# zhang-xuan1314/ABC-Net

Hardware: NVIDIA B200
Metric: images_per_sec_unet_fwd_decode (higher is better)
Workload: dtype bf16

## Files before the change

abcnet_b200/_lib.py:

```python
from __future__ import annotations

import ctypes as C
import os

_HERE = os.path.dirname(os.path.abspath(__file__))
LIB_PATH = os.path.join(_HERE, "libabcnet_b200.so")

EXPORTS = (
    "abc_last_error", "abc_version", "abc_device_ok", "abc_sm_count", "abc_launch_count",
    "abc_conv3x3_c1", "abc_conv3x3_c1_u8", "abc_conv3x3_cn", "abc_conv3x3_cn_wgrad", "abc_conv3x3_stem", "abc_conv_igemm", "abc_conv_wpack_bytes", "abc_decode_peaks",
    "abc_loss_partials", "abc_loss_backward", "abc_loss_partials_p8",
    "abc_bn_stats", "abc_bn_finalize", "abc_bn_act", "abc_bn_act_backward", "abc_nchw_to_p8", "abc_channel_sum",
    "abc_nchw_to_p8_ex", "abc_deinterleave2", "abc_conv_wgrad", "abc_conv3x3_c1_wgrad", "abc_conv3x3_c1_raw",
    "abc_heads_fused", "abc_heads_fused_pack_sizes", "abc_gather_pack", "abc_adam_step", "abc_adam_chunk_elems", "abc_assemble_molblocks", "abc_gather_patches", "abc_rasterise_targets",
    "abc_unet_wpack_bytes", "abc_unet_workspace_bytes", "abc_unet_create", "abc_unet_forward_infer", "abc_unet_destroy", "abc_unet_pack_host",
)


class AbcConvDesc(C.Structure):
    _fields_ = [
        ("in_", C.c_void_p), ("N", C.c_int), ("H", C.c_int), ("W", C.c_int),
        ("in_planes", C.c_int), ("in_plane_off", C.c_int), ("cin", C.c_int),
        ("wpack", C.c_void_p), ("bias", C.c_void_p),
        ("cout", C.c_int), ("n_tile", C.c_int), ("ntaps", C.c_int),
        ("tap_dy", C.c_int * 9), ("tap_dx", C.c_int * 9),
        ("act", C.c_int), ("out_mode", C.c_int),
        ("out", C.c_void_p), ("out_planes", C.c_int), ("out_plane_off", C.c_int),
        ("out_H", C.c_int), ("out_W", C.c_int),
        ("out_sy", C.c_int), ("out_oy", C.c_int), ("out_sx", C.c_int), ("out_ox", C.c_int),
        ("pool_out", C.c_void_p), ("pool_planes", C.c_int), ("pool_plane_off", C.c_int),
        ("k_segments", C.c_int), ("seg_tap0", C.c_int * 4), ("seg_ntaps", C.c_int * 4),
        ("row_fold", C.c_int), ("cta_pair", C.c_int), ("swap_mn", C.c_int),
        ("stat_sum", C.c_void_p), ("stat_sq", C.c_void_p), ("subpixel", C.c_int), ("k_chunk", C.c_int), ("act_fp16", C.c_int),
    ]


class AbcUNetConfig(C.Structure):
    _fields_ = [("in_channels", C.c_int), ("n_heads", C.c_int), ("heads", C.c_int * 16), ("crop_first", C.c_int), ("act_fp16", C.c_int)]


class AbcNamedTensor(C.Structure):
    _fields_ = [("name", C.c_char_p), ("data", C.c_void_p), ("numel", C.c_int64)]


class AbcAtomRec(C.Structure):
    _fields_ = [("x", C.c_uint16), ("y", C.c_uint16), ("type", C.c_uint8), ("charge", C.c_uint8),
                ("hs", C.c_uint8), ("pad", C.c_uint8)]


class AbcBondRec(C.Structure):
    _fields_ = [("x", C.c_uint16), ("y", C.c_uint16), ("omega", C.c_uint8), ("type", C.c_uint8),
                ("pad", C.c_uint16), ("rho", C.c_float)]


class AbcDecodeDesc(C.Structure):
    _fields_ = [
        ("maps", C.c_void_p * 8), ("N", C.c_int), ("H", C.c_int), ("W", C.c_int),
        ("c_type", C.c_int), ("c_charge", C.c_int), ("c_hs", C.c_int), ("n_omega", C.c_int), ("n_btype", C.c_int),
        ("thr", C.c_float), ("omega_mode", C.c_int),
        ("atoms", C.c_void_p), ("atom_cap", C.c_int),
        ("bonds", C.c_void_p), ("bond_cap", C.c_int),
        ("counts", C.c_void_p), ("p8f_mask", C.c_int), ("centre_prob", C.c_int), ("thr_omega", C.c_float),
        ("peak_pix", C.c_void_p), ("peak_cnt", C.c_void_p), ("peak_cap", C.c_int), ("sparse_mode", C.c_int),
    ]


class AbcTargetsDesc(C.Structure):
    _fields_ = [
        ("N", C.c_int), ("H", C.c_int), ("W", C.c_int), ("n_omega", C.c_int), ("n_btype", C.c_int), ("c_type", C.c_int),
        ("c_charge", C.c_int), ("c_hs", C.c_int),
        ("atoms", C.c_void_p), ("atom_off", C.c_void_p), ("bonds", C.c_void_p), ("bond_rho", C.c_void_p), ("bond_off", C.c_void_p),
        ("atom_target", C.c_void_p), ("atom_type", C.c_void_p), ("atom_charge", C.c_void_p), ("atom_hs", C.c_void_p),
        ("bond_target", C.c_void_p), ("bond_type", C.c_void_p), ("bond_rho_map", C.c_void_p), ("bond_omega", C.c_void_p),
        ("f64", C.c_int), ("zero_first", C.c_int),
    ]


class AbcHeadsFusedDesc(C.Structure):
    _fields_ = [
        ("in_", C.c_void_p), ("N", C.c_int), ("H", C.c_int), ("W", C.c_int), ("in_planes", C.c_int), ("in_plane_off", C.c_int),
        ("w1pack", C.c_void_p), ("bias1", C.c_void_p), ("n_heads", C.c_int), ("cout", C.c_int * 16),
        ("w2pack", C.c_void_p), ("w2pack_bytes", C.c_int64), ("bias2", C.c_void_p), ("bias2_len", C.c_int),
        ("out", C.c_void_p * 16), ("out_mode", C.c_int * 16), ("out_planes", C.c_int * 16), ("item_slot", C.c_int * 6),
        ("act_fp16", C.c_int),
    ]


class AbcBnActDesc(C.Structure):
    _fields_ = [
        ("z", C.c_void_p), ("z_planes", C.c_int), ("z_plane_off", C.c_int),
        ("out", C.c_void_p), ("out_planes", C.c_int), ("out_plane_off", C.c_int),
        ("pool", C.c_void_p), ("pool_planes", C.c_int), ("pool_plane_off", C.c_int),
        ("N", C.c_int), ("H", C.c_int), ("W", C.c_int), ("C", C.c_int),
        ("scale", C.c_void_p), ("shift", C.c_void_p),
        ("act", C.c_int), ("drop_p", C.c_float), ("seed", C.c_uint64), ("seed_dev", C.c_void_p), ("drop_mask", C.c_void_p),
    ]


class AbcBnActBwdDesc(C.Structure):
    _fields_ = [
        ("z", C.c_void_p), ("z_planes", C.c_int), ("z_plane_off", C.c_int),
        ("dA", C.c_void_p), ("dA_planes", C.c_int), ("dA_plane_off", C.c_int),
        ("dP", C.c_void_p), ("dP_planes", C.c_int), ("dP_plane_off", C.c_int),
        ("dz", C.c_void_p), ("dz_planes", C.c_int), ("dz_plane_off", C.c_int),
        ("N", C.c_int), ("H", C.c_int), ("W", C.c_int), ("C", C.c_int),
        ("scale", C.c_void_p), ("shift", C.c_void_p), ("mean", C.c_void_p), ("invstd", C.c_void_p),
        ("act", C.c_int), ("drop_p", C.c_float), ("seed", C.c_uint64),
        ("s1", C.c_void_p), ("s2", C.c_void_p), ("seed_dev", C.c_void_p), ("gscale", C.c_void_p), ("drop_mask", C.c_void_p),
    ]


class AbcWgradDesc(C.Structure):
    _fields_ = [
        ("dz", C.c_void_p), ("dz_planes", C.c_int), ("dz_plane_off", C.c_int), ("cout", C.c_int),
        ("in_", C.c_void_p), ("in_planes", C.c_int), ("in_plane_off", C.c_int), ("cin", C.c_int),
        ("N", C.c_int), ("H", C.c_int), ("W", C.c_int),
        ("ntaps", C.c_int), ("tap_dy", C.c_int * 9), ("tap_dx", C.c_int * 9),
        ("dw", C.c_void_p), ("row_boxes", C.c_int),
    ]


class AbcLossDesc(C.Structure):
    _fields_ = [
        ("logits", C.c_void_p * 8), ("targets", C.c_void_p * 8), ("tgt_f64", C.c_int),
        ("N", C.c_int), ("H", C.c_int), ("W", C.c_int),
        ("c_type", C.c_int), ("c_charge", C.c_int), ("c_hs", C.c_int), ("n_omega", C.c_int), ("n_btype", C.c_int),
        ("type_weights", C.c_void_p), ("sums", C.c_void_p), ("scale", C.c_void_p),
        ("dlogits", C.c_void_p * 8),
    ]


class AbcLossP8Out(C.Structure):
    _fields_ = [("dz", C.c_void_p * 8), ("planes", C.c_int * 8), ("dbias", C.c_void_p * 8)]


assert C.sizeof(AbcAtomRec) == 8 and C.sizeof(AbcBondRec) == 12


def _load():
    if not os.path.exists(LIB_PATH):
        raise ImportError(
            f"{LIB_PATH} not found: the abcnet_b200 CUDA library has not been built "
            "(run __graft_entry__.build() or `make -C abcnet_b200/csrc`). There is no CPU fallback.")
    lib = C.CDLL(LIB_PATH)
    lib.abc_last_error.restype = C.c_char_p
    lib.abc_launch_count.restype = C.c_int64
    lib.abc_conv_wpack_bytes.restype = C.c_int64
    lib.abc_conv_wpack_bytes.argtypes = [C.c_int] * 4
    lib.abc_conv3x3_c1.argtypes = [C.c_void_p, C.c_void_p, C.c_void_p, C.c_void_p, C.c_int, C.c_int, C.c_int,
                                   C.c_int, C.c_int, C.c_void_p]
    lib.abc_conv3x3_c1_u8.argtypes = lib.abc_conv3x3_c1.argtypes
    lib.abc_conv3x3_cn.argtypes = [C.c_void_p, C.c_int, C.c_void_p, C.c_void_p, C.c_void_p, C.c_int, C.c_int, C.c_int,
                                   C.c_int, C.c_int, C.c_int, C.c_void_p]
    lib.abc_conv3x3_stem.argtypes = [C.c_void_p, C.c_int, C.c_int, C.c_void_p, C.c_void_p, C.c_void_p, C.c_int, C.c_int, C.c_int,
                                     C.c_int, C.c_int, C.c_int, C.c_void_p]
    lib.abc_conv3x3_cn_wgrad.argtypes = [C.c_void_p, C.c_int, C.c_void_p, C.c_int, C.c_int, C.c_int, C.c_int, C.c_int,
                                         C.c_void_p, C.c_void_p]
    lib.abc_conv_igemm.argtypes = [C.POINTER(AbcConvDesc), C.c_void_p]
    lib.abc_decode_peaks.argtypes = [C.POINTER(AbcDecodeDesc), C.c_void_p]
    lib.abc_loss_partials.argtypes = [C.POINTER(AbcLossDesc), C.c_void_p]
    lib.abc_loss_backward.argtypes = [C.POINTER(AbcLossDesc), C.c_void_p]
    lib.abc_loss_partials_p8.argtypes = [C.POINTER(AbcLossDesc), C.POINTER(AbcLossP8Out), C.c_void_p]
    vp, ci = C.c_void_p, C.c_int
    lib.abc_bn_stats.argtypes = [vp, ci, ci, ci, ci, ci, ci, vp, vp, vp]
    lib.abc_channel_sum.argtypes = lib.abc_bn_stats.argtypes
    lib.abc_bn_finalize.argtypes = [vp, vp, ci, C.c_double, vp, vp, C.c_float, C.c_float, vp, vp, vp, vp, vp, vp, vp]
    lib.abc_bn_act.argtypes = [C.POINTER(AbcBnActDesc), vp]
    lib.abc_bn_act_backward.argtypes = [C.POINTER(AbcBnActBwdDesc), vp]
    lib.abc_nchw_to_p8.argtypes = [vp, vp, ci, ci, ci, ci, vp]
    lib.abc_nchw_to_p8_ex.argtypes = [vp, vp, ci, ci, ci, ci, ci, vp, vp, vp]
    lib.abc_deinterleave2.argtypes = [vp, ci, ci, ci, vp, ci, ci, ci, vp]
    lib.abc_conv_wgrad.argtypes = [C.POINTER(AbcWgradDesc), vp]
    lib.abc_conv3x3_c1_wgrad.argtypes = [vp, ci, vp, ci, ci, ci, ci, ci, vp, vp]
    lib.abc_conv3x3_c1_raw.argtypes = [vp, ci, vp, vp, vp, ci, ci, ci, ci, ci, vp]
    lib.abc_heads_fused.argtypes = [C.POINTER(AbcHeadsFusedDesc), vp]
    lib.abc_heads_fused_pack_sizes.argtypes = [ci, C.POINTER(C.c_int), C.POINTER(C.c_int64), C.POINTER(C.c_int)]
    lib.abc_gather_pack.argtypes = [vp, vp, vp, C.c_int64, ci, vp]
    lib.abc_adam_step.argtypes = [vp, vp, vp, vp, vp, vp, ci, vp, vp, vp]
    lib.abc_rasterise_targets.argtypes = [C.POINTER(AbcTargetsDesc), vp]
    lib.abc_gather_patches.argtypes = [vp, ci, ci, ci, ci, vp, vp, ci, vp, vp]
    lib.abc_unet_wpack_bytes.restype = C.c_int64
    lib.abc_unet_wpack_bytes.argtypes = [C.POINTER(AbcUNetConfig)]
    lib.abc_unet_workspace_bytes.restype = C.c_int64
    lib.abc_unet_workspace_bytes.argtypes = [C.POINTER(AbcUNetConfig), ci, ci, ci]
    lib.abc_unet_create.argtypes = [C.POINTER(AbcUNetConfig), C.POINTER(AbcNamedTensor), ci, vp, C.c_int64, vp, C.POINTER(vp)]
    lib.abc_unet_forward_infer.argtypes = [vp, vp, ci, ci, ci, ci, vp, C.c_int64, C.POINTER(vp), ci, vp]
    lib.abc_unet_destroy.argtypes = [vp]
    lib.abc_unet_pack_host.argtypes = [C.POINTER(AbcUNetConfig), C.POINTER(AbcNamedTensor), ci, vp, C.c_int64, C.POINTER(C.c_int64)]
    lib.abc_assemble_molblocks.argtypes = [vp, ci, vp, ci, vp, ci, vp, vp, ci, ci, vp, C.c_int64, vp]
    return lib


lib = _load()


def check(rc: int, what: str = "abcnet_b200") -> None:
    if rc != 0:
        msg = lib.abc_last_error()
        raise RuntimeError(f"{what} failed with status {rc}: {msg.decode() if msg else ''}")


def require_device() -> None:
    if not lib.abc_device_ok():
        msg = lib.abc_last_error()
        raise RuntimeError("abcnet_b200 needs an sm_100 (B200) CUDA device and has no CPU fallback: "
                           + (msg.decode() if msg else ""))


def current_stream_ptr() -> int:
    import torch
    return torch.cuda.current_stream().cuda_stream


def launch_count() -> int:
    return int(lib.abc_launch_count())
```

abcnet_b200/csrc/conv_first.cu:

```cuda
#include <cstdlib>
#include <cuda_bf16.h>

#include "common.cuh"
#include "p8_device.cuh"

namespace abc {

template <typename T>
__global__ void __launch_bounds__(256) conv3x3_c1_kernel(const T* __restrict__ img, const float* __restrict__ w,
                                                         const float* __restrict__ b, uint4* __restrict__ out, int H, int W,
                                                         int out_planes, int out_plane_off, int relu) {
  __shared__ float ws[16 * 9 + 16];
  const int tid = threadIdx.y * 32 + threadIdx.x;
  if (tid < 144) ws[tid] = w[tid];
  if (tid < 16) ws[144 + tid] = b[tid];
  __syncthreads();
  const int x = blockIdx.x * 32 + threadIdx.x;
  const int y = blockIdx.y * 8 + threadIdx.y;
  const int n = blockIdx.z;
  if (x >= W || y >= H) return;
  const T* im = img + static_cast<size_t>(n) * H * W;
  float t[9];
#pragma unroll
  for (int dy = 0; dy < 3; ++dy)
#pragma unroll
    for (int dx = 0; dx < 3; ++dx) {
      const int yy = y + dy - 1, xx = x + dx - 1;
      t[dy * 3 + dx] = (yy >= 0 && yy < H && xx >= 0 && xx < W) ? static_cast<float>(__ldg(im + static_cast<size_t>(yy) * W + xx)) : 0.f;
    }
  float v[16];
#pragma unroll
  for (int co = 0; co < 16; ++co) {
    float a = ws[144 + co];
#pragma unroll
    for (int k = 0; k < 9; ++k) a = fmaf(t[k], ws[co * 9 + k], a);
    v[co] = (relu & 1) ? fmaxf(a, 0.f) : a;
  }
#pragma unroll
  for (int pl = 0; pl < 2; ++pl)
    out[((static_cast<size_t>(n) * out_planes + out_plane_off + pl) * H + y) * W + x] = pack8_act16(v + pl * 8, (relu & 2) != 0);
}

constexpr int kC1Rows = 16;

__device__ __forceinline__ uint4 c1_pack8(const float* a, int flags) { return pack8_act16(a, (flags & 2) != 0); }

template <typename T>
__device__ __noinline__ void c1_generic_pixel(const T* __restrict__ im, int y, int x, int H, int W, const float* ws, int relu,
                                              uint4* o0, uint4* o1) {
  float t[9];
#pragma unroll
  for (int k = 0; k < 9; ++k) {
    const int yy = y + k / 3 - 1, xx = x + k % 3 - 1;
    t[k] = (yy >= 0 && yy < H && xx >= 0 && xx < W) ? static_cast<float>(__ldg(im + static_cast<size_t>(yy) * W + xx)) : 0.f;
  }
#pragma unroll
  for (int pl = 0; pl < 2; ++pl) {
    float v[8];
#pragma unroll
    for (int c8 = 0; c8 < 8; ++c8) {
      const int co = pl * 8 + c8;
      float a = ws[144 + co];
#pragma unroll
      for (int k = 0; k < 9; ++k) a = fmaf(t[k], ws[k * 16 + co], a);
      v[c8] = (relu & 1) ? fmaxf(a, 0.f) : a;
    }
    *(pl ? o1 : o0) = c1_pack8(v, relu);
  }
}

template <typename T>
__global__ void __launch_bounds__(256, 4) conv3x3_c1_rows_kernel(const T* __restrict__ img, const float* __restrict__ w,
                                                              const float* __restrict__ b, uint4* __restrict__ out, int N, int H, int W,
                                                              int out_planes, int out_plane_off, int relu) {
  __shared__ __align__(16) float ws[9 * 16 + 16];
  __shared__ __align__(16) uint4 lut[512][2];
  const int tid = threadIdx.x;
  if (tid < 144) ws[(tid % 9) * 16 + tid / 9] = w[tid];
  if (tid < 16) ws[144 + tid] = b[tid];
  __syncthreads();
#pragma unroll 1
  for (int e = tid; e < 512; e += 256) {
#pragma unroll 1
    for (int pl = 0; pl < 2; ++pl) {
      float v[8];
#pragma unroll
      for (int c8 = 0; c8 < 8; ++c8) {
        const int co = pl * 8 + c8;
        float a = ws[144 + co];
#pragma unroll
        for (int k = 0; k < 9; ++k) a = fmaf(((e >> k) & 1) ? 1.f : 0.f, ws[k * 16 + co], a);
        v[c8] = (relu & 1) ? fmaxf(a, 0.f) : a;
      }
      lut[e][pl] = c1_pack8(v, relu);
    }
  }
  __syncthreads();
  const int lane = tid & 31, warp = tid >> 5;
  const int tiles_x = (W + 127) >> 7, strips = (H + kC1Rows - 1) / kC1Rows;
  const long long items = static_cast<long long>(N) * strips * tiles_x;
  const size_t plane = static_cast<size_t>(H) * W;
  for (long long it = static_cast<long long>(blockIdx.x) * 8 + warp; it < items; it += static_cast<long long>(gridDim.x) * 8) {
    const int n = static_cast<int>(it / (strips * tiles_x));
    const int rem = static_cast<int>(it - static_cast<long long>(n) * (strips * tiles_x));
    const int x0 = (rem % tiles_x) << 7, y0 = (rem / tiles_x) * kC1Rows;
    const int y1 = min(y0 + kC1Rows, H);
    const T* im = img + static_cast<size_t>(n) * plane;
    uint4* o_img = out + (static_cast<size_t>(n) * out_planes + out_plane_off) * plane;
    const int xe = lane == 0 ? x0 - 1 : x0 + 128;
    const bool edge_ok = lane < 2 && xe >= 0 && xe < W;
    uint32_t m[3][4], e[3];
    bool nb[3];
    auto load_row = [&](int yy, uint32_t (&mm)[4], uint32_t& ee, bool& nbin) {
      float v[4], ve = 0.f;
      const bool in = yy >= 0 && yy < H;
      const T* row = im + static_cast<size_t>(in ? yy : 0) * W;
#pragma unroll
      for (int k = 0; k < 4; ++k) {
        const int x = x0 + 32 * k + lane;
        v[k] = (in && x < W) ? static_cast<float>(__ldg(row + x)) : 0.f;
      }
      if (in && edge_ok) ve = static_cast<float>(__ldg(row + xe));
      bool bad = (ve != 0.f) && (ve != 1.f);
#pragma unroll
      for (int k = 0; k < 4; ++k) {
        mm[k] = __ballot_sync(0xffffffffu, v[k] != 0.f);
        bad = bad || ((v[k] != 0.f) && (v[k] != 1.f));
      }
      ee = __ballot_sync(0xffffffffu, ve != 0.f);
      nbin = __any_sync(0xffffffffu, bad);
    };
    load_row(y0 - 1, m[0], e[0], nb[0]);
    load_row(y0, m[1], e[1], nb[1]);
    for (int y = y0; y < y1; ++y) {
      load_row(y + 1, m[2], e[2], nb[2]);
      uint4* o0 = o_img + static_cast<size_t>(y) * W;
      uint4* o1 = o0 + plane;
      if (!(nb[0] || nb[1] || nb[2])) {
#pragma unroll
        for (int k = 0; k < 4; ++k) {
          uint32_t pat = 0;
#pragma unroll
          for (int r = 0; r < 3; ++r) {
            const uint32_t lo = k == 0 ? (e[r] & 1u) : (m[r][k - 1] >> 31);
            const uint32_t hi = k == 3 ? ((e[r] >> 1) & 1u) : (m[r][k + 1] & 1u);
            const uint64_t wide = (static_cast<uint64_t>(hi) << 33) | (static_cast<uint64_t>(m[r][k]) << 1) | lo;
            pat |= (static_cast<uint32_t>(wide >> lane) & 7u) << (3 * r);
          }
          const int x = x0 + 32 * k + lane;
          if (x < W) {
            o0[x] = lut[pat][0];
            o1[x] = lut[pat][1];
          }
        }
      } else {
#pragma unroll 1
        for (int k = 0; k < 4; ++k) {
          const int x = x0 + 32 * k + lane;
          if (x < W) c1_generic_pixel<T>(im, y, x, H, W, ws, relu, o0 + x, o1 + x);
        }
      }
#pragma unroll
      for (int k = 0; k < 4; ++k) {
        m[0][k] = m[1][k];
        m[1][k] = m[2][k];
      }
      e[0] = e[1]; e[1] = e[2];
      nb[0] = nb[1]; nb[1] = nb[2];
    }
  }
}

__global__ void __launch_bounds__(256) conv3x3_cn_kernel(const float* __restrict__ img, int cin, const float* __restrict__ w,
                                                         const float* __restrict__ b, uint4* __restrict__ out, int H, int W,
                                                         int out_planes, int out_plane_off, int relu) {
  __shared__ float ws[16 * 8 * 9 + 16];
  const int tid = threadIdx.y * 32 + threadIdx.x;
  for (int i = tid; i < 16 * cin * 9; i += 256) ws[i] = w[i];
  if (tid < 16) ws[16 * 8 * 9 + tid] = b[tid];
  __syncthreads();
  const int x = blockIdx.x * 32 + threadIdx.x;
  const int y = blockIdx.y * 8 + threadIdx.y;
  const int n = blockIdx.z;
  if (x >= W || y >= H) return;
  float v[16];
#pragma unroll
  for (int co = 0; co < 16; ++co) v[co] = ws[16 * 8 * 9 + co];
  for (int ci = 0; ci < cin; ++ci) {
    const float* im = img + (static_cast<size_t>(n) * cin + ci) * H * W;
    float t[9];
#pragma unroll
    for (int dy = 0; dy < 3; ++dy)
#pragma unroll
      for (int dx = 0; dx < 3; ++dx) {
        const int yy = y + dy - 1, xx = x + dx - 1;
        t[dy * 3 + dx] = (yy >= 0 && yy < H && xx >= 0 && xx < W) ? __ldg(im + static_cast<size_t>(yy) * W + xx) : 0.f;
      }
#pragma unroll
    for (int co = 0; co < 16; ++co) {
      float a = v[co];
#pragma unroll
      for (int k = 0; k < 9; ++k) a = fmaf(t[k], ws[(co * cin + ci) * 9 + k], a);
      v[co] = a;
    }
  }
  if (relu & 1) {
#pragma unroll
    for (int co = 0; co < 16; ++co) v[co] = fmaxf(v[co], 0.f);
  }
#pragma unroll
  for (int pl = 0; pl < 2; ++pl)
    out[((static_cast<size_t>(n) * out_planes + out_plane_off + pl) * H + y) * W + x] = pack8_act16(v + pl * 8, (relu & 2) != 0);
}

}

extern "C" int abc_conv3x3_cn(const float* img, int cin, const float* w, const float* b, void* out, int N, int H, int W,
                              int out_planes, int out_plane_off, int relu, void* stream) {
  using namespace abc;
  if (int rc = device_check()) return rc;
  ABC_REQUIRE(img && w && b && out, "abc_conv3x3_cn: null pointer");
  ABC_REQUIRE(cin >= 1 && cin <= 8, "abc_conv3x3_cn: cin=%d must be in 1..8", cin);
  ABC_REQUIRE(N > 0 && H > 0 && W > 0 && N <= 65535, "abc_conv3x3_cn: bad geometry N=%d H=%d W=%d", N, H, W);
  ABC_REQUIRE(out_plane_off >= 0 && out_plane_off + 2 <= out_planes, "abc_conv3x3_cn: output plane range");
  ABC_REQUIRE((reinterpret_cast<uintptr_t>(out) & 15) == 0, "abc_conv3x3_cn: output must be 16-byte aligned");
  dim3 grid((W + 31) / 32, (H + 7) / 8, N);
  conv3x3_cn_kernel<<<grid, dim3(32, 8), 0, static_cast<cudaStream_t>(stream)>>>(img, cin, w, b, static_cast<uint4*>(out), H, W,
                                                                                  out_planes, out_plane_off, relu);
  return launch_check("conv3x3_cn_kernel");
}

template <typename T>
static int conv3x3_c1_launch(const T* img, const float* w, const float* b, void* out, int N, int H, int W, int out_planes,
                             int out_plane_off, void* stream, int relu = 1) {
  using namespace abc;
  if (int rc = device_check()) return rc;
  ABC_REQUIRE(img && w && b && out, "abc_conv3x3_c1: null pointer");
  ABC_REQUIRE(N > 0 && H > 0 && W > 0 && N <= 65535, "abc_conv3x3_c1: bad geometry N=%d H=%d W=%d", N, H, W);
  ABC_REQUIRE(out_plane_off >= 0 && out_plane_off + 2 <= out_planes, "abc_conv3x3_c1: output plane range");
  ABC_REQUIRE((reinterpret_cast<uintptr_t>(out) & 15) == 0, "abc_conv3x3_c1: output must be 16-byte aligned");
  dim3 block(32, 8);
  static const bool simple = getenv("ABCNET_C1_SIMPLE") != nullptr;
  if (!simple) {
    const long long items = static_cast<long long>((W + 127) / 128) * ((H + kC1Rows - 1) / kC1Rows) * N;
    int sms = sm_count();
    if (sms <= 0) sms = 148;
    const long long want = (items + 7) / 8;
    const int gx = static_cast<int>(want < 4LL * sms ? want : 4LL * sms);
    conv3x3_c1_rows_kernel<T><<<gx, 256, 0, static_cast<cudaStream_t>(stream)>>>(img, w, b, static_cast<uint4*>(out), N, H, W,
                                                                                 out_planes, out_plane_off, relu);
    return launch_check("conv3x3_c1_rows_kernel");
  }
  dim3 grid((W + 31) / 32, (H + 7) / 8, N);
  conv3x3_c1_kernel<T><<<grid, block, 0, static_cast<cudaStream_t>(stream)>>>(img, w, b, static_cast<uint4*>(out), H, W,
                                                                               out_planes, out_plane_off, relu);
  return launch_check("conv3x3_c1_kernel");
}

extern "C" int abc_conv3x3_c1(const float* img, const float* w, const float* b, void* out, int N, int H, int W,
                              int out_planes, int out_plane_off, void* stream) {
  return conv3x3_c1_launch<float>(img, w, b, out, N, H, W, out_planes, out_plane_off, stream);
}

extern "C" int abc_conv3x3_c1_u8(const uint8_t* img, const float* w, const float* b, void* out, int N, int H, int W,
                                 int out_planes, int out_plane_off, void* stream) {
  return conv3x3_c1_launch<uint8_t>(img, w, b, out, N, H, W, out_planes, out_plane_off, stream);
}

extern "C" int abc_conv3x3_c1_raw(const void* img, int img_is_u8, const float* w, const float* b, void* out, int N, int H, int W,
                                  int out_planes, int out_plane_off, void* stream) {
  if (img_is_u8)
    return conv3x3_c1_launch<uint8_t>(static_cast<const uint8_t*>(img), w, b, out, N, H, W, out_planes, out_plane_off, stream, 0);
  return conv3x3_c1_launch<float>(static_cast<const float*>(img), w, b, out, N, H, W, out_planes, out_plane_off, stream, 0);
}


extern "C" int abc_conv3x3_stem(const void* img, int img_is_u8, int cin, const float* w, const float* b, void* out, int N, int H, int W,
                                int out_planes, int out_plane_off, int flags, void* stream) {
  ABC_REQUIRE(flags >= 0 && flags <= 3, "abc_conv3x3_stem: flags=%d (bit 0 ReLU, bit 1 fp16 output)", flags);
  if (cin != 1) {
    ABC_REQUIRE(!img_is_u8, "abc_conv3x3_stem: uint8 images are the 1-channel binarised format");
    return abc_conv3x3_cn(static_cast<const float*>(img), cin, w, b, out, N, H, W, out_planes, out_plane_off, flags, stream);
  }
  if (img_is_u8)
    return conv3x3_c1_launch<uint8_t>(static_cast<const uint8_t*>(img), w, b, out, N, H, W, out_planes, out_plane_off, stream, flags);
  return conv3x3_c1_launch<float>(static_cast<const float*>(img), w, b, out, N, H, W, out_planes, out_plane_off, stream, flags);
}
```

abcnet_b200/csrc/conv_igemm_sm100.cu:

```cuda
#include <cstdlib>
#include <cuda.h>
#include <cuda_bf16.h>

#include "common.cuh"
#include "p8_device.cuh"
#include "ptx_sm100.cuh"

namespace abc {

constexpr int kMaxNA = 8;
constexpr int kMaxAcc = 8;
constexpr int kMaxNB = 16;
constexpr uint32_t kHeaderBytes = 2048;
constexpr uint32_t kSmemBudget = 232448;
constexpr int kThreads = 384;
constexpr int kTmemCols = 512;
constexpr uint32_t kSwapRowBytes = 80;
constexpr uint32_t kSwapWarpBytes = 16 * kSwapRowBytes;
constexpr uint32_t kSwapStageBytes = 8 * kSwapWarpBytes;

struct ConvKParams {
  int N, H, W, tiles_x, tiles_y, groups_x, num_groups;
  int in_plane_off, kp, nkc, ntaps, halo, n_tile, resident_b, na, nb, mt, nacc, acc_cols;
  int chunks_per_seg, blocks_per_ntile;
  int seg_tap0[4], seg_ntaps[4];
  uint32_t a_stage_bytes, a_tile_bytes, a_plane_bytes, a_row_bytes, b_block_bytes;
  uint32_t tap_off[18];
  int dbg;
  int fold;
  int tile_rows;
  uint32_t smem_a_off, smem_b_off;
  const uint8_t* wpack;
  const float* bias;
  int cout, act, out_mode;
  void* out;
  int out_planes, out_plane_off, out_H, out_W, out_sy, out_oy, out_sx, out_ox;
  void* pool_out;
  int pool_planes, pool_plane_off;
  int subpixel;
  int fp16;
  double* stat_sum;
  double* stat_sq;
};

__device__ __forceinline__ float apply_act(float v, int act) {
  if (act == 1) return fmaxf(v, 0.f);
  if (act == 2) return v > 0.f ? v : 0.01f * v;
  return v;
}

__device__ __forceinline__ uint4 pack8_bf16(const float* v) {
  __nv_bfloat162 a = __floats2bfloat162_rn(v[0], v[1]);
  __nv_bfloat162 b = __floats2bfloat162_rn(v[2], v[3]);
  __nv_bfloat162 c = __floats2bfloat162_rn(v[4], v[5]);
  __nv_bfloat162 d = __floats2bfloat162_rn(v[6], v[7]);
  uint4 r;
  r.x = *reinterpret_cast<uint32_t*>(&a);
  r.y = *reinterpret_cast<uint32_t*>(&b);
  r.z = *reinterpret_cast<uint32_t*>(&c);
  r.w = *reinterpret_cast<uint32_t*>(&d);
  return r;
}

__device__ __forceinline__ uint32_t pool_max_bf16x2(uint32_t a, bool f16) {
  uint32_t b = __shfl_xor_sync(0xffffffffu, a, 1);
  a = max2_act16(a, b, f16);
  b = __shfl_xor_sync(0xffffffffu, a, 8);
  return max2_act16(a, b, f16);
}

__device__ __forceinline__ uint4 hmax_bf16x8(uint4 a, uint4 b, bool f16) {
  return make_uint4(max2_act16(a.x, b.x, f16), max2_act16(a.y, b.y, f16), max2_act16(a.z, b.z, f16), max2_act16(a.w, b.w, f16));
}

__device__ __forceinline__ uint4 pool_hmax_x(uint4 q, bool f16) {
  uint4 o;
  o.x = __shfl_xor_sync(0xffffffffu, q.x, 1);
  o.y = __shfl_xor_sync(0xffffffffu, q.y, 1);
  o.z = __shfl_xor_sync(0xffffffffu, q.z, 1);
  o.w = __shfl_xor_sync(0xffffffffu, q.w, 1);
  return hmax_bf16x8(q, o, f16);
}

__device__ __forceinline__ uint4 pool_max_bf16x8(uint4 q, bool f16) {
  q.x = pool_max_bf16x2(q.x, f16);
  q.y = pool_max_bf16x2(q.y, f16);
  q.z = pool_max_bf16x2(q.z, f16);
  q.w = pool_max_bf16x2(q.w, f16);
  return q;
}

template <int KSTEPS, bool RESIDENT, bool CG2, bool SWAP = false, bool STATS = false>
__global__ void __launch_bounds__(kThreads, 1)
conv_igemm_kernel(const __grid_constant__ CUtensorMap tmap, const ConvKParams p) {
  static_assert(!(CG2 && RESIDENT), "the CTA-pair variant streams its weights");
  static_assert(!(CG2 && SWAP), "operand swap is a single-CTA mode");
  static_assert(!(STATS && (SWAP || CG2)), "STATS is the non-swap, single-CTA variant");
  extern __shared__ __align__(1024) uint8_t smem[];
  const uint32_t sbase = smem_u32(smem);
  const int warp = static_cast<int>(warp_id_uniform());
  const int lane = threadIdx.x & 31;
  const uint32_t cta_rank = CG2 ? cluster_ctarank() : 0u;
  const bool leader = cta_rank == 0;

  const uint32_t bar_a_full = sbase;
  const uint32_t bar_a_empty = sbase + 8 * kMaxNA;
  const uint32_t bar_b_full = sbase + 8 * (2 * kMaxNA);
  const uint32_t bar_b_empty = bar_b_full + 8 * kMaxNB;
  const uint32_t bar_acc_full = bar_b_empty + 8 * kMaxNB;
  const uint32_t bar_acc_empty = bar_acc_full + 8 * kMaxAcc;
  static_assert(8 * (2 * kMaxNA + 2 * kMaxNB + 2 * kMaxAcc) <= 768, "barrier slots overflow the header");
  uint32_t* tmem_slot = reinterpret_cast<uint32_t*>(smem + 768);
  float* bias_s = reinterpret_cast<float*>(smem + 1024);

  if (threadIdx.x == 0) {
    const uint32_t full_count = (CG2 && leader && !(p.dbg & 1)) ? 2 : 1;
    for (int i = 0; i < kMaxNA; ++i) {
      mbar_init(bar_a_full + 8 * i, full_count);
      mbar_init(bar_a_empty + 8 * i, 1);
    }
    for (int i = 0; i < kMaxNB; ++i) {
      mbar_init(bar_b_full + 8 * i, full_count);
      mbar_init(bar_b_empty + 8 * i, 1);
    }
    for (int i = 0; i < kMaxAcc; ++i) {
      mbar_init(bar_acc_full + 8 * i, 1);
      mbar_init(bar_acc_empty + 8 * i, CG2 ? 16 : 8);
    }
    fence_mbar_init();
    tma_prefetch_desc(&tmap);
  }
  if (CG2) cluster_sync_all();
  if (warp == 2) {
    if (CG2) tmem_alloc_pair<kTmemCols>(smem_u32(tmem_slot));
    else tmem_alloc<kTmemCols>(smem_u32(tmem_slot));
  }
  for (int i = threadIdx.x; i < p.n_tile; i += kThreads) bias_s[i] = p.bias[blockIdx.y * p.n_tile + i];
  uint32_t* utab = reinterpret_cast<uint32_t*>(smem + 800);
  uint32_t* utab2 = reinterpret_cast<uint32_t*>(smem + 928);
  if (threadIdx.x < ((p.mt * p.n_tile) >> 4)) {
    const int col = threadIdx.x << 4;
    const int ti = col / p.n_tile;
    const int ul = (col - ti * p.n_tile) >> 4;
    const int b16 = ul / p.fold;
    utab[threadIdx.x] = static_cast<uint32_t>(ti) | (ul << 8) | (b16 << 16) | ((ul - b16 * p.fold) << 24);
    if (p.subpixel > 0 && threadIdx.x < 16) {
      const int c0 = blockIdx.y * p.n_tile + (b16 << 4);
      const int ph = c0 / p.subpixel, chn = c0 - ph * p.subpixel;
      utab2[threadIdx.x] = (static_cast<uint32_t>(chn >> 3) << 16) | static_cast<uint32_t>((ph >> 1) * p.out_W + (ph & 1));
    }
  }
  tc_fence_before();
  if (CG2) cluster_sync_all();
  else __syncthreads();
  tc_fence_after();
  const uint32_t tmem_base = *reinterpret_cast<volatile uint32_t*>(tmem_slot);
  const int g_first = CG2 ? static_cast<int>(blockIdx.x & ~1u) : static_cast<int>(blockIdx.x);

  const int groups_per_img = p.groups_x * p.tiles_y;
  const uint32_t a_region = sbase + p.smem_a_off;
  const uint32_t b_region = sbase + p.smem_b_off;
  const int blocks_per_ntile = p.blocks_per_ntile;

  if (warp == 0) {
    int stage = 0;
    uint32_t phase = 0;
    for (int gp = g_first; gp < p.num_groups; gp += gridDim.x) {
      const int g = CG2 ? min(gp + static_cast<int>(cta_rank), p.num_groups - 1) : gp;
      const int n = g / groups_per_img;
      const int rem = g - n * groups_per_img;
      const int ty = rem / p.groups_x;
      const int tx0 = (rem - ty * p.groups_x) * p.mt;
      const int c1 = ty * p.tile_rows - p.halo;
      for (int kc = 0; kc < p.nkc; ++kc) {
        mbar_wait(bar_a_empty + 8 * stage, phase ^ 1);
        if (elect_one()) {
          mbar_arrive_expect_tx(bar_a_full + 8 * stage, p.a_stage_bytes);
          for (int i = 0; i < p.mt; ++i)
            tma_load_4d(a_region + stage * p.a_stage_bytes + i * p.a_tile_bytes, &tmap, bar_a_full + 8 * stage,
                        ((tx0 + i) * 8 - p.halo) * 8, c1, p.in_plane_off + kc * p.kp, n);
        }
        __syncwarp();
        if (++stage == p.na) {
          stage = 0;
          phase ^= 1;
        }
      }
    }
  } else if (warp == 3) {
    const size_t b_src_stride = CG2 ? 2 * static_cast<size_t>(p.b_block_bytes) : p.b_block_bytes;
    const uint8_t* wsrc = p.wpack + static_cast<size_t>(blockIdx.y) * blocks_per_ntile * b_src_stride +
                          (CG2 ? cta_rank * p.b_block_bytes : 0u);
    if (RESIDENT) {
      if (blockIdx.x < p.num_groups && elect_one()) {
        mbar_arrive_expect_tx(bar_b_full, static_cast<uint32_t>(blocks_per_ntile) * p.b_block_bytes);
        for (int blk = 0; blk < blocks_per_ntile; ++blk)
          bulk_load_1d(b_region + blk * p.b_block_bytes, wsrc + static_cast<size_t>(blk) * p.b_block_bytes,
                       p.b_block_bytes, bar_b_full);
      }
      __syncwarp();
    } else {
      int stage = 0;
      uint32_t phase = 0;
      for (int g = g_first; g < p.num_groups; g += gridDim.x) {
        for (int blk = 0; blk < blocks_per_ntile; ++blk) {
          mbar_wait(bar_b_empty + 8 * stage, phase ^ 1);
          if (elect_one()) {
            mbar_arrive_expect_tx(bar_b_full + 8 * stage, p.b_block_bytes);
            bulk_load_1d(b_region + stage * p.b_block_bytes, wsrc + static_cast<size_t>(blk) * b_src_stride,
                         p.b_block_bytes, bar_b_full + 8 * stage);
          }
          __syncwarp();
          if (++stage == p.nb) {
            stage = 0;
            phase ^= 1;
          }
        }
      }
    }
  } else if (warp == 1 && CG2 && !leader) {
    int a_stage = 0, b_stage = 0;
    uint32_t a_phase = 0, b_phase = 0;
    for (int g = g_first; g < p.num_groups; g += gridDim.x) {
      for (int kc = 0; kc < p.nkc; ++kc) {
        mbar_wait(bar_a_full + 8 * a_stage, a_phase);
        if (!(p.dbg & 1) && elect_one()) mbar_arrive_cluster(mapa_cluster(bar_a_full + 8 * a_stage, 0));
        __syncwarp();
        if (++a_stage == p.na) {
          a_stage = 0;
          a_phase ^= 1;
        }
        for (int t = 0; t < p.ntaps; ++t) {
          mbar_wait(bar_b_full + 8 * b_stage, b_phase);
          if (!(p.dbg & 1) && elect_one()) mbar_arrive_cluster(mapa_cluster(bar_b_full + 8 * b_stage, 0));
          __syncwarp();
          if (++b_stage == p.nb) {
            b_stage = 0;
            b_phase ^= 1;
          }
        }
      }
    }
  } else if (warp == 1) {
    const bool f16 = p.fp16 != 0;
    const uint32_t idesc = SWAP ? umma_idesc_16(128, 256, 0, 0, f16) : umma_idesc_16(CG2 ? 256 : 128, p.n_tile, 0, 0, f16);
    const int b_rows = CG2 ? p.n_tile >> 1 : p.n_tile;
    auto mma = [&](uint32_t d, uint32_t a_lo, uint32_t a_hi_, uint32_t b_lo, uint32_t b_hi_, uint32_t acc_) {
      if (CG2) umma_bf16_lohi_pair(d, a_lo, a_hi_, b_lo, b_hi_, idesc, acc_);
      else if (SWAP) umma_bf16_lohi(d, b_lo, b_hi_, a_lo, a_hi_, idesc, acc_);
      else umma_bf16_lohi(d, a_lo, a_hi_, b_lo, b_hi_, idesc, acc_);
    };
    auto commit = [&](uint32_t bar) {
      if (CG2) umma_commit_pair(bar);
      else umma_commit(bar);
    };
    const uint64_t a_hi64 = umma_desc_hi(p.a_plane_bytes, p.a_row_bytes * p.fold);
    const uint64_t b_hi64 = CG2 ? umma_desc_hi_sw128() : umma_desc_hi(b_rows * 16, 128);
    const uint32_t a_hi = static_cast<uint32_t>(a_hi64 >> 32), b_hi = static_cast<uint32_t>(b_hi64 >> 32);
    const uint32_t a_lo0 = static_cast<uint32_t>(a_hi64) | (a_region >> 4);
    const uint32_t b_lo0 = static_cast<uint32_t>(b_hi64) | (b_region >> 4);
    const uint32_t a_kstep = (2 * p.a_plane_bytes) >> 4, b_kstep = CG2 ? 2u : (2 * b_rows * 16) >> 4;
    const uint32_t a_tile16 = p.a_tile_bytes >> 4, a_stage16 = p.a_stage_bytes >> 4, b_block16 = p.b_block_bytes >> 4;
    int a_stage = 0, b_stage = 0, acc = 0;
    uint32_t a_phase = 0, b_phase = 0, acc_phase = 0;
    if (RESIDENT && blockIdx.x < p.num_groups) {
      mbar_wait(bar_b_full, 0);
      tc_fence_after();
    }
    if (p.chunks_per_seg == p.nkc) {
      uint32_t tap16[18];
#pragma unroll
      for (int t = 0; t < 18; ++t) tap16[t] = p.tap_off[t] >> 4;
      const int ntaps = p.ntaps, nkc = p.nkc, mt = p.mt, n_tile = p.n_tile, na = p.na, nb = p.nb, nacc = p.nacc;
      const uint32_t acc_cols = p.acc_cols;
      for (int g = g_first; g < p.num_groups; g += gridDim.x) {
        mbar_wait(bar_acc_empty + 8 * acc, acc_phase ^ 1);
        tc_fence_after();
        const uint32_t tmem_d = tmem_base + acc * acc_cols;
        uint32_t b_res = b_lo0;
        for (int kc = 0; kc < nkc; ++kc) {
          mbar_wait(bar_a_full + 8 * a_stage, a_phase);
          tc_fence_after();
          const uint32_t a_base = a_lo0 + a_stage * a_stage16;
#pragma unroll
          for (int t = 0; t < 18; ++t) {
            if (t < ntaps) {
              uint32_t b_base;
              if (RESIDENT) {
                b_base = b_res;
                b_res += b_block16;
              } else {
                mbar_wait(bar_b_full + 8 * b_stage, b_phase);
                tc_fence_after();
                b_base = b_lo0 + b_stage * b_block16;
              }
              const uint32_t a_tap = a_base + tap16[t];
              const uint32_t acc0 = (kc | t) != 0 ? 1u : 0u;
              if (elect_one()) {
                uint32_t d_col = tmem_d, a_t = a_tap;
                for (int i = 0; i < mt; ++i, d_col += n_tile, a_t += a_tile16) {
#pragma unroll
                  for (int j = 0; j < KSTEPS; ++j)
                    mma(d_col, a_t + j * a_kstep, a_hi, b_base + j * b_kstep, b_hi, j != 0 ? 1u : acc0);
                }
                if (!RESIDENT) commit(bar_b_empty + 8 * b_stage);
              }
              __syncwarp();
              if (!RESIDENT) {
                if (++b_stage == nb) {
                  b_stage = 0;
                  b_phase ^= 1;
                }
              }
            }
          }
          if (elect_one()) commit(bar_a_empty + 8 * a_stage);
          __syncwarp();
          if (++a_stage == na) {
            a_stage = 0;
            a_phase ^= 1;
          }
        }
        if (elect_one()) commit(bar_acc_full + 8 * acc);
        __syncwarp();
        if (++acc == nacc) {
          acc = 0;
          acc_phase ^= 1;
        }
      }
    } else
    for (int g = blockIdx.x; g < p.num_groups; g += gridDim.x) {
      mbar_wait(bar_acc_empty + 8 * acc, acc_phase ^ 1);
      tc_fence_after();
      const uint32_t tmem_d = tmem_base + acc * p.acc_cols;
      int blk = 0;
      for (int kc = 0; kc < p.nkc; ++kc) {
        mbar_wait(bar_a_full + 8 * a_stage, a_phase);
        tc_fence_after();
        const uint32_t a_base = a_lo0 + a_stage * a_stage16;
        const int seg = kc / p.chunks_per_seg;
        const int t_begin = p.seg_tap0[seg], t_end = t_begin + p.seg_ntaps[seg];
        for (int t = t_begin; t < t_end; ++t, ++blk) {
          uint32_t b_base;
          if (RESIDENT) {
            b_base = b_lo0 + blk * b_block16;
          } else {
            mbar_wait(bar_b_full + 8 * b_stage, b_phase);
            tc_fence_after();
            b_base = b_lo0 + b_stage * b_block16;
          }
          const uint32_t a_tap = a_base + (p.tap_off[t] >> 4);
          const uint32_t acc0 = (kc | (t - t_begin)) != 0 ? 1u : 0u;
          if (elect_one()) {
#pragma unroll 2
            for (int i = 0; i < p.mt; ++i) {
#pragma unroll
              for (int j = 0; j < KSTEPS; ++j)
                umma_bf16_lohi(tmem_d + i * p.n_tile, a_tap + i * a_tile16 + j * a_kstep, a_hi, b_base + j * b_kstep, b_hi,
                               idesc, j != 0 ? 1u : acc0);
            }
            if (!RESIDENT) umma_commit(bar_b_empty + 8 * b_stage);
          }
          __syncwarp();
          if (!RESIDENT) {
            if (++b_stage == p.nb) {
              b_stage = 0;
              b_phase ^= 1;
            }
          }
        }
        if (elect_one()) umma_commit(bar_a_empty + 8 * a_stage);
        __syncwarp();
        if (++a_stage == p.na) {
          a_stage = 0;
          a_phase ^= 1;
        }
      }
      if (elect_one()) umma_commit(bar_acc_full + 8 * acc);
      __syncwarp();
      if (++acc == p.nacc) {
        acc = 0;
        acc_phase ^= 1;
      }
    }
  } else if (warp >= 4 && SWAP) {
    const int q = warp & 3;
    const int eh = (warp - 4) >> 2;
    const int n0 = blockIdx.y * p.n_tile;
    const float bias = bias_s[q * 32 + lane];
    const float slope = p.act == 1 ? 0.f : (p.act == 2 ? 0.01f : 1.f);
    const int g8 = lane >> 3, i8 = lane & 7;
    const int J = p.fold, cpj = 128 / J;
    const int m0 = q * 32 + g8 * 8;
    const int fj = m0 / cpj, ch0 = m0 - fj * cpj;
    uint8_t* stage = smem + kHeaderBytes + (warp - 4) * kSwapWarpBytes;
    unsigned short* st_w = reinterpret_cast<unsigned short*>(stage) + lane;
    const bool f16 = p.fp16 != 0;
    const uint4* st_r = reinterpret_cast<const uint4*>(stage + i8 * kSwapRowBytes + g8 * 16);
    const bool plane_ok = (n0 + ch0) < p.cout;
    const size_t out_plane_px = static_cast<size_t>(p.out_H) * p.out_W;
    const bool do_stats = p.stat_sum != nullptr;
    const int m_own = q * 32 + lane;
    const int fj_own = m_own / cpj;
    float st_s = 0.f, st_q = 0.f;
    int acc = 0;
    uint32_t acc_phase = 0;
    for (int g = g_first; g < p.num_groups; g += gridDim.x) {
      const int n = g / groups_per_img;
      const int rem = g - n * groups_per_img;
      const int ty = rem / p.groups_x;
      const int tx = rem - ty * p.groups_x;
      const int x = tx * 8 + i8;
      const int y0 = (ty * 32 + eh * 16) * J + fj;
      uint4* obase = reinterpret_cast<uint4*>(p.out) +
                     (static_cast<size_t>(n) * p.out_planes + p.out_plane_off + ((n0 + ch0) >> 3)) * out_plane_px +
                     static_cast<size_t>(p.out_oy) * p.out_W + (x * p.out_sx + p.out_ox);
      const bool col_ok = plane_ok && x < p.W;
      const uint32_t tbase = tmem_base + acc * p.acc_cols + (static_cast<uint32_t>(q * 32) << 16) + eh * 128;
      const int x_left = p.W - tx * 8;
      const uint32_t xmask8 = x_left >= 8 ? 0xffu : ((1u << (x_left > 0 ? x_left : 0)) - 1u);
      const int yo0 = (ty * 32 + eh * 16) * J + fj_own;
      mbar_wait(bar_acc_full + 8 * acc, acc_phase);
      tc_fence_after();
      auto process = [&](uint32_t (&raw)[16], int it) {
        uint32_t vmask = 0;
        if (do_stats)
          vmask = ((yo0 + (it * 2) * J) < p.H ? xmask8 : 0u) | ((yo0 + (it * 2 + 1) * J) < p.H ? (xmask8 << 8) : 0u);
#pragma unroll
        for (int i = 0; i < 16; ++i) {
          const float t = __uint_as_float(raw[i]) + bias;
          const unsigned short hv = to_act16(fmaxf(t, t * slope), f16);
          st_w[i * (kSwapRowBytes / 2)] = hv;
          if (do_stats && ((vmask >> i) & 1u)) {
            const float r = __uint_as_float(static_cast<uint32_t>(hv) << 16);
            st_s += r;
            st_q = fmaf(r, r, st_q);
          }
        }
        __syncwarp();
#pragma unroll
        for (int rr = 0; rr < 2; ++rr) {
          const uint4 val = st_r[rr * (8 * kSwapRowBytes / 16)];
          const int y = y0 + (it * 2 + rr) * J;
          if (col_ok && y < p.H) obase[static_cast<size_t>(y * p.out_sy) * p.out_W] = val;
        }
        __syncwarp();
      };
      uint32_t raw_a[16], raw_b[16];
      tmem_ld16(tbase, raw_a);
#pragma unroll 1
      for (int it = 0; it < 8; it += 2) {
        tmem_ld_wait();
        tmem_ld16(tbase + (it + 1) * 16, raw_b);
        process(raw_a, it);
        tmem_ld_wait();
        if (it + 2 < 8) tmem_ld16(tbase + (it + 2) * 16, raw_a);
        process(raw_b, it + 1);
      }
      tc_fence_before();
      __syncwarp();
      if (lane == 0) mbar_arrive(bar_acc_empty + 8 * acc);
      if (++acc == p.nacc) {
        acc = 0;
        acc_phase ^= 1;
      }
    }
    if (do_stats) {
      const int ch = n0 + (m_own - fj_own * cpj);
      if (ch < p.cout) {
        atomicAdd(p.stat_sum + ch, static_cast<double>(st_s));
        atomicAdd(p.stat_sq + ch, static_cast<double>(st_q));
      }
    }
  } else if (warp >= 4) {
    const int q = warp & 3;
    const int eh = (warp - 4) >> 2;
    const int m = q * 32 + lane;
    const int r = m >> 3, c = m & 7;
    const int n0 = blockIdx.y * p.n_tile;
    const int units = (p.mt * p.n_tile) >> 4;
    const int nchunks = (units + 1) >> 1;
    const float slope = p.act == 1 ? 0.f : (p.act == 2 ? 0.01f : 1.f);
    const bool f16 = p.fp16 != 0;
    const float4* bias4 = reinterpret_cast<const float4*>(bias_s);
    const size_t out_plane_px = static_cast<size_t>(p.out_H) * p.out_W;
    const int ph = p.H >> 1, pw = p.W >> 1;
    const size_t pool_plane_px = static_cast<size_t>(ph) * pw;
    int acc = 0;
    uint32_t acc_phase = 0;
    float sacc[STATS ? 16 : 1], qacc[STATS ? 16 : 1];
#pragma unroll
    for (int i = 0; i < (STATS ? 16 : 1); ++i) sacc[i] = qacc[i] = 0.f;
    const uint32_t acc_empty_base = CG2 ? mapa_cluster(bar_acc_empty, 0) : bar_acc_empty;
    for (int gp = g_first; gp < p.num_groups; gp += gridDim.x) {
      const int g = CG2 ? min(gp + static_cast<int>(cta_rank), p.num_groups - 1) : gp;
      const bool g_valid = !CG2 || (gp + static_cast<int>(cta_rank) < p.num_groups);
      const int n = g / groups_per_img;
      const int rem = g - n * groups_per_img;
      const int ty = rem / p.groups_x;
      const int tx0 = (rem - ty * p.groups_x) * p.mt;
      const int ybase = (ty * 16 + r) * p.fold;
      const int xbase = tx0 * 8 + c;
      const size_t out_px0 = static_cast<size_t>(ybase * p.out_sy + p.out_oy) * p.out_W + (xbase * p.out_sx + p.out_ox);
      const size_t out_pl0 = static_cast<size_t>(n) * p.out_planes + p.out_plane_off + (n0 >> 3);
      const size_t pool_px0 = static_cast<size_t>(ybase >> 1) * pw + (xbase >> 1);
      const size_t pool_pl0 = static_cast<size_t>(n) * p.pool_planes + p.pool_plane_off + (n0 >> 3);
      const uint32_t tbase = tmem_base + acc * p.acc_cols + (static_cast<uint32_t>(q * 32) << 16);
      mbar_wait(bar_acc_full + 8 * acc, acc_phase);
      tc_fence_after();

      auto load = [&](uint32_t (&raw)[2][16], int ch) {
        tmem_ld16(tbase + ch * 32, raw[0]);
        if (2 * ch + 1 < units) tmem_ld16(tbase + ch * 32 + 16, raw[1]);
      };
      auto process = [&](uint32_t (&raw)[2][16], int ch) {
        uint4 keep0 = make_uint4(0, 0, 0, 0), keep1 = keep0;
#pragma unroll
        for (int half = 0; half < 2; ++half) {
          const int u = 2 * ch + half;
          if (u >= units) break;
          const uint32_t info = utab[u];
          const int ti = info & 0xff, bu = (info >> 8) & 0xff, b16 = (info >> 16) & 0xff, j = info >> 24;
          if (tx0 + ti >= p.tiles_x) continue;
          const int ch0 = n0 + (b16 << 4);
          const int y = ybase + j;
          const int x = xbase + ti * 8;
          const bool valid = (y < p.H) && (x < p.W) && (ch0 < p.cout) && g_valid;
          const bool two = (ch0 + 8) < p.cout;
          float v[16];
#pragma unroll
          for (int i = 0; i < 4; ++i) {
            const float4 bb = bias4[bu * 4 + i];
            float t0 = __uint_as_float(raw[half][4 * i + 0]) + bb.x, t1 = __uint_as_float(raw[half][4 * i + 1]) + bb.y;
            float t2 = __uint_as_float(raw[half][4 * i + 2]) + bb.z, t3 = __uint_as_float(raw[half][4 * i + 3]) + bb.w;
            v[4 * i + 0] = fmaxf(t0, t0 * slope);
            v[4 * i + 1] = fmaxf(t1, t1 * slope);
            v[4 * i + 2] = fmaxf(t2, t2 * slope);
            v[4 * i + 3] = fmaxf(t3, t3 * slope);
          }
          if (p.out_mode == 0) {
            uint4 q0 = pack8_act16(v, f16), q1 = pack8_act16(v + 8, f16);
            if constexpr (STATS) {
              if (valid) {
                float r[16];
                unpack8u(q0, r);
                unpack8u(q1, r + 8);
#pragma unroll
                for (int i = 0; i < 16; ++i) {
                  sacc[i] += r[i];
                  qacc[i] = fmaf(r[i], r[i], qacc[i]);
                }
              }
            }
            if (p.out != nullptr && valid) {
              uint4* o;
              if (p.subpixel > 0) {
                const uint32_t t2 = utab2[u];
                o = reinterpret_cast<uint4*>(p.out) +
                    (static_cast<size_t>(n) * p.out_planes + p.out_plane_off + (t2 >> 16)) * out_plane_px + out_px0 + (t2 & 0xffffu) +
                    ti * 8 * p.out_sx;
              } else {
                o = reinterpret_cast<uint4*>(p.out) + (out_pl0 + 2 * b16) * out_plane_px + out_px0 +
                    static_cast<size_t>(j * p.out_sy) * p.out_W + ti * 8 * p.out_sx;
              }
              o[0] = q0;
              if (two) o[out_plane_px] = q1;
            }
            if (p.pool_out != nullptr) {
              bool write;
              if (p.fold == 1) {
                q0 = pool_max_bf16x8(q0, f16);
                q1 = pool_max_bf16x8(q1, f16);
                write = !(c & 1) && !(r & 1);
              } else {
                if (half == 0) {
                  keep0 = q0;
                  keep1 = q1;
                  continue;
                }
                q0 = pool_hmax_x(hmax_bf16x8(q0, keep0, f16), f16);
                q1 = pool_hmax_x(hmax_bf16x8(q1, keep1, f16), f16);
                write = !(c & 1);
              }
              if (valid && write) {
                uint4* o = reinterpret_cast<uint4*>(p.pool_out) + (pool_pl0 + 2 * b16) * pool_plane_px + pool_px0 +
                           static_cast<size_t>(j >> 1) * pw + ti * 4;
                o[0] = q0;
                if (two) o[pool_plane_px] = q1;
              }
            }
          } else if (p.out_mode == 2) {
            if (valid) {
              float4* o = reinterpret_cast<float4*>(p.out) + 2 * ((out_pl0 + 2 * b16) * out_plane_px + out_px0 + ti * 8 * p.out_sx);
              o[0] = make_float4(v[0], v[1], v[2], v[3]);
              o[1] = make_float4(v[4], v[5], v[6], v[7]);
              if (two) {
                o += 2 * out_plane_px;
                o[0] = make_float4(v[8], v[9], v[10], v[11]);
                o[1] = make_float4(v[12], v[13], v[14], v[15]);
              }
            }
          } else if (valid) {
            float* o = reinterpret_cast<float*>(p.out) + (static_cast<size_t>(n) * p.cout + ch0) * out_plane_px + out_px0 +
                       ti * 8 * p.out_sx;
#pragma unroll
            for (int i = 0; i < 16; ++i)
              if (ch0 + i < p.cout) o[i * out_plane_px] = v[i];
          }
        }
      };

      uint32_t raw_a[2][16], raw_b[2][16];
      int ch = eh;
      if (ch < nchunks) {
        load(raw_a, ch);
        while (true) {
          tmem_ld_wait();
          if (ch + 2 < nchunks) load(raw_b, ch + 2);
          process(raw_a, ch);
          ch += 2;
          if (ch >= nchunks) break;
          tmem_ld_wait();
          if (ch + 2 < nchunks) load(raw_a, ch + 2);
          process(raw_b, ch);
          ch += 2;
          if (ch >= nchunks) break;
        }
      }
      tc_fence_before();
      __syncwarp();
      if (lane == 0) {
        if (CG2) mbar_arrive_cluster(acc_empty_base + 8 * acc);
        else mbar_arrive(bar_acc_empty + 8 * acc);
      }
      if (++acc == p.nacc) {
        acc = 0;
        acc_phase ^= 1;
      }
    }
    if constexpr (STATS) {
#pragma unroll
      for (int i = 0; i < 16; ++i) {
        float a = sacc[i], b = qacc[i];
#pragma unroll
        for (int o = 16; o > 0; o >>= 1) {
          a += __shfl_xor_sync(0xffffffffu, a, o);
          b += __shfl_xor_sync(0xffffffffu, b, o);
        }
        if (lane == 0 && n0 + i < p.cout) {
          atomicAdd(p.stat_sum + n0 + i, static_cast<double>(a));
          atomicAdd(p.stat_sq + n0 + i, static_cast<double>(b));
        }
      }
    }
  }

  tc_fence_before();
  if (CG2) cluster_sync_all();
  else __syncthreads();
  if (warp == 2) {
    tc_fence_after();
    if (CG2) tmem_dealloc_pair<kTmemCols>(tmem_base);
    else tmem_dealloc<kTmemCols>(tmem_base);
  }
}

typedef CUresult (*EncodeTiledFn)(CUtensorMap*, CUtensorMapDataType, cuuint32_t, void*, const cuuint64_t*,
                                  const cuuint64_t*, const cuuint32_t*, const cuuint32_t*, CUtensorMapInterleave,
                                  CUtensorMapSwizzle, CUtensorMapL2promotion, CUtensorMapFloatOOBfill);

static EncodeTiledFn get_encode_fn() { return reinterpret_cast<EncodeTiledFn>(tensor_map_encode_fn()); }

static int conv_kc(int cin) { return cin < 64 ? cin : 64; }

struct ConvEnv {
  int pair_dbg, mt256, mt, nacc;
  ConvEnv() {
    auto num = [](const char* name, int dflt) { const char* e = getenv(name); return e ? atoi(e) : dflt; };
    pair_dbg = num("ABCNET_PAIR_DBG", 0);
    mt256 = num("ABCNET_MT256", 0);
    mt = num("ABCNET_MT", 0);
    nacc = num("ABCNET_NACC", 0);
  }
};
static const ConvEnv& conv_env() {
  static const ConvEnv e;
  return e;
}

}

extern "C" int64_t abc_conv_wpack_bytes(int cin, int cout, int ntaps, int n_tile) {
  if (cin <= 0 || cin % 16 || n_tile < 16 || n_tile > 256 || n_tile % 16 || ntaps < 1 || ntaps > 18 || cout < 1) return -1;
  const int n_tiles = (cout + n_tile - 1) / n_tile;
  return static_cast<int64_t>(n_tiles) * n_tile * cin * ntaps * 2;
}

extern "C" int abc_conv_igemm(const AbcConvDesc* d, void* stream_) {
  using namespace abc;
  if (int rc = device_check()) return rc;
  ABC_REQUIRE(d != nullptr, "abc_conv_igemm: null descriptor");
  ABC_REQUIRE(d->in && d->wpack && d->bias, "abc_conv_igemm: null input / weights / bias");
  ABC_REQUIRE(d->out || d->pool_out, "abc_conv_igemm: no output buffer");
  ABC_REQUIRE(d->N > 0 && d->H > 0 && d->W > 0, "abc_conv_igemm: bad geometry N=%d H=%d W=%d", d->N, d->H, d->W);
  ABC_REQUIRE(d->cin >= 16 && d->cin % 16 == 0 && (d->cin <= 64 || d->cin % 64 == 0),
              "abc_conv_igemm: cin=%d must be 16, 32, 48, 64 or a multiple of 64", d->cin);
  ABC_REQUIRE(d->in_plane_off >= 0 && d->in_plane_off + d->cin / 8 <= d->in_planes, "abc_conv_igemm: input plane range");
  ABC_REQUIRE(d->n_tile >= 16 && d->n_tile <= 256 && d->n_tile % 16 == 0, "abc_conv_igemm: n_tile=%d", d->n_tile);
  ABC_REQUIRE(d->ntaps >= 1 && d->ntaps <= 9, "abc_conv_igemm: ntaps=%d", d->ntaps);
  ABC_REQUIRE(d->cout >= 1, "abc_conv_igemm: cout=%d", d->cout);
  ABC_REQUIRE(d->out_mode >= 0 && d->out_mode <= 2, "abc_conv_igemm: out_mode=%d", d->out_mode);
  ABC_REQUIRE((reinterpret_cast<uintptr_t>(d->in) & 15) == 0 && (reinterpret_cast<uintptr_t>(d->wpack) & 15) == 0,
              "abc_conv_igemm: input / weights must be 16-byte aligned");
  const int fold = d->row_fold > 1 ? d->row_fold : 1;
  if (fold > 1) {
    ABC_REQUIRE(fold == 2 || fold == 4, "abc_conv_igemm: row_fold=%d must be 1, 2 or 4", fold);
    ABC_REQUIRE(d->ntaps == 9 && d->k_segments <= 1, "abc_conv_igemm: row_fold needs the plain 3x3 tap set");
    ABC_REQUIRE(d->cout % 16 == 0 && d->n_tile == fold * d->cout, "abc_conv_igemm: row_fold needs n_tile == row_fold * cout (cout %% 16 == 0)");
    ABC_REQUIRE(d->out_mode == 0 && d->out_sy == 1 && d->out_sx == 1 && d->out_oy == 0 && d->out_ox == 0,
                "abc_conv_igemm: row_fold supports plain P8 outputs only");
  }
  const bool swap = d->swap_mn != 0;
  if (swap) {
    ABC_REQUIRE(d->n_tile == 128 && (fold == 1 || fold == 2 || fold == 4) && d->k_segments <= 1 && !d->cta_pair,
                "abc_conv_igemm: swap_mn needs n_tile == 128 and no k_segments / cta_pair");
    ABC_REQUIRE(d->out_mode == 0 && d->out != nullptr && d->pool_out == nullptr,
                "abc_conv_igemm: swap_mn supports plain P8 outputs only (no pool_out)");
  }
  int halo = 0;
  for (int t = 0; t < d->ntaps; ++t) {
    ABC_REQUIRE(d->tap_dy[t] >= -1 && d->tap_dy[t] <= 1 && d->tap_dx[t] >= -1 && d->tap_dx[t] <= 1,
                "abc_conv_igemm: tap %d offset out of [-1,1]", t);
    if (d->tap_dy[t] || d->tap_dx[t]) halo = 1;
  }
  if (d->out_mode == 0) {
    ABC_REQUIRE(d->cout % 8 == 0, "abc_conv_igemm: P8 output needs cout %% 8 == 0 (got %d)", d->cout);
    const int out_ch = d->subpixel > 0 ? d->subpixel : d->cout;
    if (d->out) ABC_REQUIRE(d->out_plane_off >= 0 && d->out_plane_off + out_ch / 8 <= d->out_planes, "abc_conv_igemm: output plane range");
  } else {
    ABC_REQUIRE(d->out != nullptr && d->pool_out == nullptr, "abc_conv_igemm: fp32 output modes need out and no pool_out");
    if (d->out_mode == 2)
      ABC_REQUIRE(d->out_plane_off >= 0 && d->out_plane_off + (d->cout + 7) / 8 <= d->out_planes,
                  "abc_conv_igemm: planar fp32 output plane range");
  }
  const int subpixel = d->subpixel > 0 ? d->subpixel : 0;
  if (subpixel) {
    ABC_REQUIRE(d->out_mode == 0 && d->out != nullptr && d->pool_out == nullptr && !swap && fold == 1 && !d->cta_pair,
                "abc_conv_igemm: subpixel needs a plain P8 output without pool / swap / fold / pair");
    ABC_REQUIRE(subpixel % 16 == 0 && d->cout == 4 * subpixel && d->out_sy == 2 && d->out_sx == 2,
                "abc_conv_igemm: subpixel needs cout == 4 * subpixel (multiple of 16) and out_sy == out_sx == 2");
    ABC_REQUIRE(d->n_tile / 16 <= 16 && d->out_W < 32768 && d->out_plane_off + subpixel / 8 <= d->out_planes,
                "abc_conv_igemm: subpixel: n_tile <= 256, out_W < 32768, plane range");
    ABC_REQUIRE((d->H - 1) * 2 + d->out_oy + 1 < d->out_H && (d->W - 1) * 2 + d->out_ox + 1 < d->out_W,
                "abc_conv_igemm: subpixel output mapping exceeds out_H x out_W");
  }
  if (d->out) {
    ABC_REQUIRE(d->out_sy >= 1 && d->out_sx >= 1 && d->out_oy >= 0 && d->out_ox >= 0 &&
                    (d->H - 1) * d->out_sy + d->out_oy < d->out_H && (d->W - 1) * d->out_sx + d->out_ox < d->out_W,
                "abc_conv_igemm: output mapping exceeds out_H x out_W");
  }
  if (d->pool_out) {
    ABC_REQUIRE(d->H % 2 == 0 && d->W % 2 == 0, "abc_conv_igemm: fused max-pool needs even H, W");
    ABC_REQUIRE(d->pool_plane_off >= 0 && d->pool_plane_off + d->cout / 8 <= d->pool_planes, "abc_conv_igemm: pool plane range");
  }

  ConvKParams p{};
  p.N = d->N; p.H = d->H; p.W = d->W;
  p.tiles_x = (d->W + 7) / 8;
  p.fold = fold;
  const ConvEnv& env = conv_env();
  p.dbg = env.pair_dbg;
  p.tile_rows = swap ? 32 * fold : 16 * fold;
  p.tiles_y = (d->H + p.tile_rows - 1) / p.tile_rows;
  p.in_plane_off = d->in_plane_off;
  const int kc = d->k_chunk > 0 ? d->k_chunk : conv_kc(d->cin);
  ABC_REQUIRE((kc == 16 || kc == 32 || kc == 48 || kc == 64) && kc <= d->cin && d->cin % kc == 0 && !(d->cta_pair && kc != 64),
              "abc_conv_igemm: k_chunk=%d must be 16, 32 or 64 and divide cin=%d", kc, d->cin);
  p.kp = kc / 8;
  p.nkc = d->cin / kc;
  p.ntaps = fold > 1 ? 3 * (fold + 2) : d->ntaps;
  p.halo = halo;
  p.n_tile = d->n_tile;
  const int rows = p.tile_rows + 2 * halo, cols = 8 + 2 * halo;
  p.a_row_bytes = cols * 16;
  p.a_plane_bytes = rows * p.a_row_bytes;
  p.a_tile_bytes = p.kp * p.a_plane_bytes;
  p.b_block_bytes = static_cast<uint32_t>(d->n_tile) * kc * 2;
  if (fold > 1) {
    for (int t = 0; t < p.ntaps; ++t) p.tap_off[t] = static_cast<uint32_t>(((t / 3) * cols + (t % 3)) * 16);
  } else {
    for (int t = 0; t < d->ntaps; ++t)
      p.tap_off[t] = static_cast<uint32_t>(((d->tap_dy[t] + halo) * cols + (d->tap_dx[t] + halo)) * 16);
  }
  ABC_REQUIRE((p.a_tile_bytes & 127u) == 0, "abc_conv_igemm: internal: A tile not a 128-byte multiple");
  const int nseg = d->k_segments > 1 ? d->k_segments : 1;
  ABC_REQUIRE(nseg <= 4 && p.nkc % nseg == 0, "abc_conv_igemm: k_segments=%d must divide the %d K chunks (<= 4)", nseg, p.nkc);
  p.chunks_per_seg = p.nkc / nseg;
  p.blocks_per_ntile = 0;
  for (int sgi = 0; sgi < nseg; ++sgi) {
    p.seg_tap0[sgi] = nseg > 1 ? d->seg_tap0[sgi] : 0;
    p.seg_ntaps[sgi] = nseg > 1 ? d->seg_ntaps[sgi] : p.ntaps;
    ABC_REQUIRE(p.seg_tap0[sgi] >= 0 && p.seg_ntaps[sgi] >= 1 && p.seg_tap0[sgi] + p.seg_ntaps[sgi] <= p.ntaps,
                "abc_conv_igemm: segment %d tap range", sgi);
    p.blocks_per_ntile += p.chunks_per_seg * p.seg_ntaps[sgi];
  }
  const bool want_pair = d->cta_pair != 0;
  if (want_pair) {
    ABC_REQUIRE(fold == 1 && nseg == 1 && kc == 64 && d->n_tile % 32 == 0,
                "abc_conv_igemm: cta_pair needs cin %% 64 == 0, n_tile %% 32 == 0, no row folding / K segments");
    p.b_block_bytes /= 2;
  }
  const uint32_t total_b = want_pair ? (1u << 30) : static_cast<uint32_t>(p.blocks_per_ntile) * p.b_block_bytes;
  p.smem_a_off = kHeaderBytes + (swap ? kSwapStageBytes : 0u);
  const uint32_t hdr = p.smem_a_off;
  int mt_max = swap ? 1 : 256 / d->n_tile;
  if (d->n_tile == 256 && env.mt256 > 0) mt_max = env.mt256 >= 2 ? 2 : 1;
  if (mt_max > 8) mt_max = 8;
  if (mt_max > p.tiles_x) mt_max = p.tiles_x;
  if (env.mt >= 1 && env.mt < mt_max) mt_max = env.mt;
  uint32_t smem_bytes = 0;
  p.mt = 0;
  for (int mt = mt_max; mt >= 1 && !p.mt; --mt) {
    const uint32_t a_stage = mt * p.a_tile_bytes;
    if (total_b < (1u << 20) && hdr + 2 * a_stage + total_b <= kSmemBudget) {
      p.mt = mt; p.resident_b = 1; p.nb = 1;
      int na = static_cast<int>((kSmemBudget - hdr - total_b) / a_stage);
      p.na = na > kMaxNA ? kMaxNA : na;
      p.a_stage_bytes = a_stage;
      p.smem_b_off = hdr + p.na * a_stage;
      smem_bytes = p.smem_b_off + total_b;
    }
  }
  for (int mt = mt_max; mt >= 1 && !p.mt; --mt) {
    const uint32_t a_stage = mt * p.a_tile_bytes;
    if (hdr + 2 * a_stage + (swap && fold > 1 ? 3 : 4) * p.b_block_bytes <= kSmemBudget) {
      p.mt = mt; p.resident_b = 0; p.na = 2;
      if (hdr + 3 * a_stage + 6 * p.b_block_bytes <= kSmemBudget) p.na = 3;
      p.a_stage_bytes = a_stage;
      p.smem_b_off = hdr + p.na * a_stage;
      if (want_pair) p.smem_b_off = (p.smem_b_off + 1023u) & ~1023u;
      int nb = static_cast<int>((kSmemBudget - p.smem_b_off) / p.b_block_bytes);
      p.nb = nb > kMaxNB ? kMaxNB : nb;
      smem_bytes = p.smem_b_off + p.nb * p.b_block_bytes;
    }
  }
  ABC_REQUIRE(p.mt >= 1, "abc_conv_igemm: cin=%d n_tile=%d does not fit in shared memory", d->cin, d->n_tile);
  p.acc_cols = swap ? 256 : p.mt * d->n_tile;
  p.nacc = kTmemCols / p.acc_cols;
  if (p.nacc > kMaxAcc) p.nacc = kMaxAcc;
  if (env.nacc >= 2 && env.nacc < p.nacc) p.nacc = env.nacc;
  p.groups_x = (p.tiles_x + p.mt - 1) / p.mt;
  const int64_t groups = static_cast<int64_t>(d->N) * p.groups_x * p.tiles_y;
  ABC_REQUIRE(groups < (1ll << 31), "abc_conv_igemm: too many tiles");
  p.num_groups = static_cast<int>(groups);
  if (smem_bytes < 120 * 1024) smem_bytes = 120 * 1024;
  p.wpack = static_cast<const uint8_t*>(d->wpack);
  p.bias = d->bias;
  p.cout = d->cout; p.act = d->act; p.out_mode = d->out_mode;
  p.out = d->out;
  p.out_planes = d->out_planes; p.out_plane_off = d->out_plane_off;
  p.out_H = d->out_H; p.out_W = d->out_W;
  p.out_sy = d->out_sy; p.out_oy = d->out_oy; p.out_sx = d->out_sx; p.out_ox = d->out_ox;
  p.pool_out = d->pool_out; p.pool_planes = d->pool_planes; p.pool_plane_off = d->pool_plane_off;
  p.subpixel = subpixel;
  p.fp16 = d->act_fp16 ? 1 : 0;
  ABC_REQUIRE(!(p.fp16 && (want_pair || d->stat_sum)), "abc_conv_igemm: act_fp16 is an inference mode (no cta_pair, no fused statistics)");
  cudaStream_t st_ = static_cast<cudaStream_t>(stream_);
  const bool stats = d->stat_sum != nullptr || d->stat_sq != nullptr;
  if (stats) {
    ABC_REQUIRE(d->stat_sum && d->stat_sq, "abc_conv_igemm: stat_sum and stat_sq go together");
    ABC_REQUIRE(d->out_mode == 0 && d->out != nullptr && d->pool_out == nullptr && !want_pair,
                "abc_conv_igemm: fused statistics need a plain P8 output");
    ABC_REQUIRE(swap || (fold == 4 && d->cout == 16 && d->n_tile == 64 && d->cin == 16),
                "abc_conv_igemm: fused statistics are built for operand-swap launches and the row-folded 16 -> 16 layers "
                "(use abc_bn_stats otherwise)");
    ABC_CUDA(cudaMemsetAsync(d->stat_sum, 0, d->cout * sizeof(double), st_));
    ABC_CUDA(cudaMemsetAsync(d->stat_sq, 0, d->cout * sizeof(double), st_));
    p.stat_sum = d->stat_sum;
    p.stat_sq = d->stat_sq;
  }

  EncodeTiledFn encode = get_encode_fn();
  if (!encode) {
    set_error("cuTensorMapEncodeTiled driver entry point not available");
    return ABC_ERR_NO_DEVICE;
  }
  CUtensorMap tmap;
  const cuuint64_t gdim[4] = {static_cast<cuuint64_t>(d->W) * 8, static_cast<cuuint64_t>(d->H),
                              static_cast<cuuint64_t>(d->in_planes), static_cast<cuuint64_t>(d->N)};
  const cuuint64_t gstride[3] = {static_cast<cuuint64_t>(d->W) * 16, static_cast<cuuint64_t>(d->W) * d->H * 16,
                                 static_cast<cuuint64_t>(d->W) * d->H * 16 * d->in_planes};
  const cuuint32_t box[4] = {static_cast<cuuint32_t>(cols * 8), static_cast<cuuint32_t>(rows),
                             static_cast<cuuint32_t>(p.kp), 1};
  const cuuint32_t estr[4] = {1, 1, 1, 1};
  CUresult cr = encode(&tmap, CU_TENSOR_MAP_DATA_TYPE_BFLOAT16, 4, const_cast<void*>(d->in), gdim, gstride, box, estr,
                       CU_TENSOR_MAP_INTERLEAVE_NONE, CU_TENSOR_MAP_SWIZZLE_NONE, CU_TENSOR_MAP_L2_PROMOTION_L2_256B,
                       CU_TENSOR_MAP_FLOAT_OOB_FILL_NONE);
  if (cr != CUDA_SUCCESS) {
    set_error("cuTensorMapEncodeTiled failed with CUresult %d (W=%d H=%d planes=%d N=%d box=%ux%ux%u)", static_cast<int>(cr),
              d->W, d->H, d->in_planes, d->N, box[0], box[1], box[2]);
    return ABC_ERR_CUDA;
  }

  typedef void (*KernelFn)(const CUtensorMap, const ConvKParams);
  KernelFn kernels[2][5] = {{nullptr, conv_igemm_kernel<1, false, false>, conv_igemm_kernel<2, false, false>,
                             conv_igemm_kernel<3, false, false>, conv_igemm_kernel<4, false, false>},
                            {nullptr, conv_igemm_kernel<1, true, false>, conv_igemm_kernel<2, true, false>,
                             conv_igemm_kernel<3, true, false>, conv_igemm_kernel<4, true, false>}};
  KernelFn swap_kernels[2][5] = {{nullptr, conv_igemm_kernel<1, false, false, true>, conv_igemm_kernel<2, false, false, true>,
                                  conv_igemm_kernel<3, false, false, true>, conv_igemm_kernel<4, false, false, true>},
                                 {nullptr, conv_igemm_kernel<1, true, false, true>, conv_igemm_kernel<2, true, false, true>,
                                  conv_igemm_kernel<3, true, false, true>, conv_igemm_kernel<4, true, false, true>}};
  KernelFn pair_kernel = conv_igemm_kernel<4, false, true>;
  KernelFn stats_kernel = conv_igemm_kernel<1, true, false, false, true>;
  static PerDeviceOnce attr_once;
  ABC_CUDA(attr_once.run([&]() -> cudaError_t {
    for (int r = 0; r < 2; ++r)
      for (int k = 1; k <= 4; ++k) {
        if (cudaError_t e = cudaFuncSetAttribute(kernels[r][k], cudaFuncAttributeMaxDynamicSharedMemorySize, kSmemBudget)) return e;
        if (cudaError_t e = cudaFuncSetAttribute(swap_kernels[r][k], cudaFuncAttributeMaxDynamicSharedMemorySize, kSmemBudget)) return e;
      }
    if (cudaError_t e = cudaFuncSetAttribute(stats_kernel, cudaFuncAttributeMaxDynamicSharedMemorySize, kSmemBudget)) return e;
    return cudaFuncSetAttribute(pair_kernel, cudaFuncAttributeMaxDynamicSharedMemorySize, kSmemBudget);
  }));
  const int ksteps = p.kp / 2;
  ABC_REQUIRE(ksteps >= 1 && ksteps <= 4, "abc_conv_igemm: internal: ksteps=%d", ksteps);
  const int n_tiles = (d->cout + d->n_tile - 1) / d->n_tile;
  int sms = sm_count();
  if (sms <= 0) sms = 148;
  int gx = sms / n_tiles;
  if (gx < 1) gx = 1;
  if (want_pair) {
    ABC_REQUIRE(!p.resident_b && ksteps == 4, "abc_conv_igemm: internal: cta_pair with resident weights");
    const int need = (p.num_groups + 1) & ~1;
    gx &= ~1;
    if (gx > need) gx = need;
    if (gx < 2) gx = 2;
    cudaLaunchConfig_t cfg = {};
    cfg.gridDim = dim3(gx, n_tiles, 1);
    cfg.blockDim = dim3(kThreads, 1, 1);
    cfg.dynamicSmemBytes = smem_bytes;
    cfg.stream = static_cast<cudaStream_t>(stream_);
    cudaLaunchAttribute attr[1];
    attr[0].id = cudaLaunchAttributeClusterDimension;
    attr[0].val.clusterDim.x = 2;
    attr[0].val.clusterDim.y = 1;
    attr[0].val.clusterDim.z = 1;
    cfg.attrs = attr;
    cfg.numAttrs = 1;
    ABC_CUDA(cudaLaunchKernelEx(&cfg, pair_kernel, tmap, p));
    return launch_check("conv_igemm_kernel<pair>");
  }
  if (gx > p.num_groups) gx = p.num_groups;
  dim3 grid(gx, n_tiles, 1);
  KernelFn fn = (swap ? swap_kernels : kernels)[p.resident_b ? 1 : 0][ksteps];
  if (stats && !swap) {
    ABC_REQUIRE(p.resident_b && ksteps == 1, "abc_conv_igemm: internal: fused statistics variant");
    fn = stats_kernel;
  }
  fn<<<grid, kThreads, smem_bytes, st_>>>(tmap, p);
  return launch_check(swap ? "conv_igemm_kernel<swap>" : "conv_igemm_kernel");
}
```

abcnet_b200/csrc/ptx_sm100.cuh:

```cuda
#pragma once
#include <cstdint>
#include <cuda_runtime.h>

namespace abc {

__device__ __forceinline__ uint32_t smem_u32(const void* p) {
  return static_cast<uint32_t>(__cvta_generic_to_shared(p));
}

__device__ __forceinline__ uint32_t warp_id_uniform() { return __shfl_sync(0xffffffffu, threadIdx.x >> 5, 0); }
__device__ __forceinline__ bool elect_one() {
  uint32_t pred;
  asm volatile(
      "{\n\t.reg .b32 rx;\n\t.reg .pred px;\n\t"
      "elect.sync rx|px, 0xffffffff;\n\t"
      "selp.u32 %0, 1, 0, px;\n\t}"
      : "=r"(pred));
  return pred != 0;
}

__device__ __forceinline__ void mbar_init(uint32_t bar, uint32_t count) {
  asm volatile("mbarrier.init.shared::cta.b64 [%0], %1;" ::"r"(bar), "r"(count) : "memory");
}
__device__ __forceinline__ void fence_mbar_init() {
  asm volatile("fence.mbarrier_init.release.cluster;" ::: "memory");
}
__device__ __forceinline__ void fence_proxy_async() {
  asm volatile("fence.proxy.async.shared::cta;" ::: "memory");
}
__device__ __forceinline__ void mbar_arrive(uint32_t bar) {
  asm volatile("{\n\t.reg .b64 st;\n\tmbarrier.arrive.shared::cta.b64 st, [%0];\n\t}" ::"r"(bar) : "memory");
}
__device__ __forceinline__ void mbar_arrive_expect_tx(uint32_t bar, uint32_t bytes) {
  asm volatile("{\n\t.reg .b64 st;\n\tmbarrier.arrive.expect_tx.shared::cta.b64 st, [%0], %1;\n\t}" ::"r"(bar),
               "r"(bytes)
               : "memory");
}
__device__ __forceinline__ bool mbar_try_wait(uint32_t bar, uint32_t parity) {
  uint32_t ok;
  asm volatile(
      "{\n\t.reg .pred p;\n\t"
      "mbarrier.try_wait.parity.shared::cta.b64 p, [%1], %2;\n\t"
      "selp.u32 %0, 1, 0, p;\n\t}"
      : "=r"(ok)
      : "r"(bar), "r"(parity)
      : "memory");
  return ok != 0;
}
__device__ __forceinline__ void mbar_wait(uint32_t bar, uint32_t parity) {
  uint32_t spins = 0;
  while (!mbar_try_wait(bar, parity)) {
    if (++spins > (1u << 24)) {
      printf("abcnet: mbarrier timeout (block %d,%d thread %d bar 0x%x parity %u)\n", blockIdx.x, blockIdx.y,
             threadIdx.x, bar, parity);
      __trap();
    }
  }
}

__device__ __forceinline__ void tma_prefetch_desc(const void* desc) {
  asm volatile("prefetch.tensormap [%0];" ::"l"(reinterpret_cast<uint64_t>(desc)) : "memory");
}
__device__ __forceinline__ void tma_load_4d(uint32_t dst, const void* desc, uint32_t bar, int c0, int c1, int c2,
                                            int c3) {
  asm volatile(
      "cp.async.bulk.tensor.4d.shared::cluster.global.mbarrier::complete_tx::bytes [%0], [%1, {%3, %4, %5, %6}], [%2];"
      ::"r"(dst), "l"(reinterpret_cast<uint64_t>(desc)), "r"(bar), "r"(c0), "r"(c1), "r"(c2), "r"(c3)
      : "memory");
}
__device__ __forceinline__ void bulk_load_1d(uint32_t dst, const void* src, uint32_t bytes, uint32_t bar) {
  asm volatile("cp.async.bulk.shared::cluster.global.mbarrier::complete_tx::bytes [%0], [%1], %2, [%3];" ::"r"(dst),
               "l"(reinterpret_cast<uint64_t>(src)), "r"(bytes), "r"(bar)
               : "memory");
}

template <int kCols>
__device__ __forceinline__ void tmem_alloc(uint32_t smem_dst) {
  const uint32_t ncols = kCols;
  asm volatile("tcgen05.alloc.cta_group::1.sync.aligned.shared::cta.b32 [%0], %1;" ::"r"(smem_dst), "r"(ncols)
               : "memory");
  asm volatile("tcgen05.relinquish_alloc_permit.cta_group::1.sync.aligned;" ::: "memory");
}
template <int kCols>
__device__ __forceinline__ void tmem_dealloc(uint32_t taddr) {
  const uint32_t ncols = kCols;
  asm volatile("tcgen05.dealloc.cta_group::1.sync.aligned.b32 %0, %1;" ::"r"(taddr), "r"(ncols) : "memory");
}
__device__ __forceinline__ void tc_fence_before() { asm volatile("tcgen05.fence::before_thread_sync;" ::: "memory"); }
__device__ __forceinline__ void tc_fence_after() { asm volatile("tcgen05.fence::after_thread_sync;" ::: "memory"); }

__device__ __forceinline__ void umma_bf16(uint32_t tmem_d, uint64_t adesc, uint64_t bdesc, uint32_t idesc,
                                          uint32_t accumulate) {
  asm volatile(
      "{\n\t.reg .pred p;\n\tsetp.ne.b32 p, %4, 0;\n\t"
      "tcgen05.mma.cta_group::1.kind::f16 [%0], %1, %2, %3, p;\n\t}"
      ::"r"(tmem_d), "l"(adesc), "l"(bdesc), "r"(idesc), "r"(accumulate)
      : "memory");
}
__device__ __forceinline__ void umma_bf16_lohi(uint32_t tmem_d, uint32_t a_lo, uint32_t a_hi, uint32_t b_lo, uint32_t b_hi,
                                               uint32_t idesc, uint32_t accumulate) {
  asm volatile(
      "{\n\t.reg .pred p;\n\t.reg .b64 da, db;\n\t"
      "mov.b64 da, {%1, %2};\n\tmov.b64 db, {%3, %4};\n\t"
      "setp.ne.b32 p, %6, 0;\n\t"
      "tcgen05.mma.cta_group::1.kind::f16 [%0], da, db, %5, p;\n\t}"
      ::"r"(tmem_d), "r"(a_lo), "r"(a_hi), "r"(b_lo), "r"(b_hi), "r"(idesc), "r"(accumulate)
      : "memory");
}
__device__ __forceinline__ void umma_16_ts(uint32_t tmem_d, uint32_t tmem_a, uint32_t b_lo, uint32_t b_hi, uint32_t idesc,
                                           uint32_t accumulate) {
  asm volatile(
      "{\n\t.reg .pred p;\n\t.reg .b64 db;\n\t"
      "mov.b64 db, {%2, %3};\n\t"
      "setp.ne.b32 p, %5, 0;\n\t"
      "tcgen05.mma.cta_group::1.kind::f16 [%0], [%1], db, %4, p;\n\t}"
      ::"r"(tmem_d), "r"(tmem_a), "r"(b_lo), "r"(b_hi), "r"(idesc), "r"(accumulate)
      : "memory");
}
__device__ __forceinline__ void umma_commit(uint32_t bar) {
  asm volatile("tcgen05.commit.cta_group::1.mbarrier::arrive::one.shared::cluster.b64 [%0];" ::"r"(bar) : "memory");
}
__device__ __forceinline__ void tmem_ld_wait() { asm volatile("tcgen05.wait::ld.sync.aligned;" ::: "memory"); }

__device__ __forceinline__ void tmem_ld16(uint32_t taddr, uint32_t (&r)[16]) {
  asm volatile(
      "tcgen05.ld.sync.aligned.32x32b.x16.b32 {%0,%1,%2,%3,%4,%5,%6,%7,%8,%9,%10,%11,%12,%13,%14,%15}, [%16];"
      : "=r"(r[0]), "=r"(r[1]), "=r"(r[2]), "=r"(r[3]), "=r"(r[4]), "=r"(r[5]), "=r"(r[6]), "=r"(r[7]), "=r"(r[8]),
        "=r"(r[9]), "=r"(r[10]), "=r"(r[11]), "=r"(r[12]), "=r"(r[13]), "=r"(r[14]), "=r"(r[15])
      : "r"(taddr)
      : "memory");
}
__device__ __forceinline__ void tmem_st16(uint32_t taddr, const uint32_t* r) {
  asm volatile(
      "tcgen05.st.sync.aligned.32x32b.x16.b32 [%0], {%1,%2,%3,%4,%5,%6,%7,%8,%9,%10,%11,%12,%13,%14,%15,%16};"
      ::"r"(taddr), "r"(r[0]), "r"(r[1]), "r"(r[2]), "r"(r[3]), "r"(r[4]), "r"(r[5]), "r"(r[6]), "r"(r[7]), "r"(r[8]),
        "r"(r[9]), "r"(r[10]), "r"(r[11]), "r"(r[12]), "r"(r[13]), "r"(r[14]), "r"(r[15])
      : "memory");
}
__device__ __forceinline__ void tmem_st_wait() { asm volatile("tcgen05.wait::st.sync.aligned;" ::: "memory"); }
__device__ __forceinline__ void named_bar_sync(uint32_t id, uint32_t threads) {
  asm volatile("bar.sync %0, %1;" ::"r"(id), "r"(threads) : "memory");
}

__device__ __forceinline__ uint32_t cluster_ctarank() {
  uint32_t r;
  asm volatile("mov.u32 %0, %%cluster_ctarank;" : "=r"(r));
  return r;
}
__device__ __forceinline__ void cluster_sync_all() {
  asm volatile("barrier.cluster.arrive.release.aligned;\n\tbarrier.cluster.wait.acquire.aligned;" ::: "memory");
}
__device__ __forceinline__ uint32_t mapa_cluster(uint32_t addr, uint32_t rank) {
  uint32_t r;
  asm volatile("mapa.shared::cluster.u32 %0, %1, %2;" : "=r"(r) : "r"(addr), "r"(rank));
  return r;
}
__device__ __forceinline__ void mbar_arrive_cluster(uint32_t cluster_addr) {
  asm volatile("mbarrier.arrive.release.cluster.shared::cluster.b64 _, [%0];" ::"r"(cluster_addr) : "memory");
}
template <int kCols>
__device__ __forceinline__ void tmem_alloc_pair(uint32_t smem_dst) {
  const uint32_t ncols = kCols;
  asm volatile("tcgen05.alloc.cta_group::2.sync.aligned.shared::cta.b32 [%0], %1;" ::"r"(smem_dst), "r"(ncols) : "memory");
  asm volatile("tcgen05.relinquish_alloc_permit.cta_group::2.sync.aligned;" ::: "memory");
}
template <int kCols>
__device__ __forceinline__ void tmem_dealloc_pair(uint32_t taddr) {
  const uint32_t ncols = kCols;
  asm volatile("tcgen05.dealloc.cta_group::2.sync.aligned.b32 %0, %1;" ::"r"(taddr), "r"(ncols) : "memory");
}
__device__ __forceinline__ void umma_bf16_lohi_pair(uint32_t tmem_d, uint32_t a_lo, uint32_t a_hi, uint32_t b_lo, uint32_t b_hi,
                                                    uint32_t idesc, uint32_t accumulate) {
  asm volatile(
      "{\n\t.reg .pred p;\n\t.reg .b64 da, db;\n\t"
      "mov.b64 da, {%1, %2};\n\tmov.b64 db, {%3, %4};\n\t"
      "setp.ne.b32 p, %6, 0;\n\t"
      "tcgen05.mma.cta_group::2.kind::f16 [%0], da, db, %5, p;\n\t}"
      ::"r"(tmem_d), "r"(a_lo), "r"(a_hi), "r"(b_lo), "r"(b_hi), "r"(idesc), "r"(accumulate)
      : "memory");
}
__device__ __forceinline__ void umma_commit_pair(uint32_t bar) {
  const uint16_t mask = 3;
  asm volatile("tcgen05.commit.cta_group::2.mbarrier::arrive::one.shared::cluster.multicast::cluster.b64 [%0], %1;" ::"r"(bar),
               "h"(mask)
               : "memory");
}

__device__ __forceinline__ uint64_t umma_desc_hi(uint32_t lbo_bytes, uint32_t sbo_bytes) {
  return (static_cast<uint64_t>((lbo_bytes >> 4) & 0x3FFF) << 16) | (static_cast<uint64_t>((sbo_bytes >> 4) & 0x3FFF) << 32) |
         (1ull << 46);
}
__device__ __forceinline__ uint64_t umma_desc(uint64_t hi, uint32_t smem_addr) {
  return hi | static_cast<uint64_t>((smem_addr >> 4) & 0x3FFF);
}
__device__ __forceinline__ uint64_t umma_desc_hi_sw128() {
  return (static_cast<uint64_t>(1024 >> 4) << 32) | (1ull << 46) | (2ull << 61);
}
__host__ __device__ constexpr uint32_t umma_idesc_bf16(int M, int N, int a_mn_major, int b_mn_major) {
  return (1u << 4) | (1u << 7) | (1u << 10) | (static_cast<uint32_t>(a_mn_major) << 15) |
         (static_cast<uint32_t>(b_mn_major) << 16) | (static_cast<uint32_t>(N >> 3) << 17) |
         (static_cast<uint32_t>(M >> 4) << 24);
}
__host__ __device__ constexpr uint32_t umma_idesc_16(int M, int N, int a_mn_major, int b_mn_major, bool fp16) {
  return umma_idesc_bf16(M, N, a_mn_major, b_mn_major) & ~(fp16 ? ((1u << 7) | (1u << 10)) : 0u);
}

}
```

abcnet_b200/csrc/unet_plan.cu:

```cuda
#include <cmath>
#include <cstring>
#include <map>
#include <string>
#include <vector>

#include <cuda_bf16.h>
#include <cuda_fp16.h>

#include "common.cuh"

namespace abc {

struct PackedConv {
  int64_t w_off = 0, b_off = 0;
  int cin = 0, cout = 0, n_tile = 0, ntaps = 0, fold = 1, fold_swap = 0, subpixel = 0;
  int tap_dy[9] = {0}, tap_dx[9] = {0};
};

struct UNetHandle {
  AbcUNetConfig cfg;
  const uint8_t* arena = nullptr;
  int64_t arena_bytes = 0;
  std::map<std::string, PackedConv> convs;
  int64_t stem_w_off = 0, stem_b_off = 0;
};

static const char* kDoubleConvs[] = {"inc1", "inc2", "down1.maxpool_conv.1", "down2.maxpool_conv.1", "inc3", "down3.maxpool_conv.1",
                                     "down4.maxpool_conv.1", "down5.maxpool_conv.1", "up1.conv", "up2.conv", "up3.conv", "dconv1", "dconv2"};
static const char* kShort[] = {"inc1", "inc2", "down1", "down2", "inc3", "down3", "down4", "down5", "up1.conv", "up2.conv", "up3.conv",
                               "dconv1", "dconv2"};
static const int kDcIn[] = {0, 16, 16, 32, 64, 64, 128, 256, 512, 256, 128, 128, 128};
static const int kDcOut[] = {16, 16, 32, 64, 64, 128, 256, 512, 256, 128, 128, 128, 128};

static bool is_pooled(const std::string& n) {
  return n == "inc2.3" || n == "down1.3" || n == "inc3.3" || n == "down3.3" || n == "down4.3";
}
static int default_n_tile(int cin, int cout) {
  const int c16 = (cout + 15) / 16 * 16;
  if (c16 <= 128) return c16;
  return (cout % 256 == 0 && cin >= 128) ? 256 : 128;
}
static int row_fold_for(int cin, int cout) {
  if (cout == 16 && cin <= 32) return 4;
  if (cout == 32 && cin <= 32) return 2;
  return 1;
}
static int swap_fold_for(int cin, int cout, bool plain) {
  if (!plain) return 0;
  const int J = cout == 64 ? 2 : (cout == 32 ? 4 : 0);
  if (J == 4 && cin > 32) return 0;
  return J;
}
static int head_conv2_n_tile(int h) {
  if (h <= 16) return 16;
  if (h <= 64) return 64;
  if (h <= 128) return 128;
  return ((h + 191) / 192 * 192 <= (h + 127) / 128 * 128) ? 192 : 128;
}
static void phase_taps(int parity, bool crop_first, int (&k)[2], int (&d)[2], int& n) {
  if (crop_first) {
    if (parity == 0) { n = 1; k[0] = 1; d[0] = 0; }
    else { n = 2; k[0] = 0; d[0] = 1; k[1] = 2; d[1] = 0; }
  } else {
    if (parity == 0) { n = 2; k[0] = 0; d[0] = 0; k[1] = 2; d[1] = -1; }
    else { n = 1; k[0] = 1; d[0] = 0; }
  }
}

struct Logical {
  int ntaps, rows, cin;
  std::vector<float> w;
  std::vector<float> bias;
  float& at(int t, int r, int c) { return w[(static_cast<size_t>(t) * rows + r) * cin + c]; }
};

static void append_pack(std::vector<uint8_t>& arena, PackedConv& pc, Logical& L, int n_tile, bool fp16) {
  const int kc = L.cin < 64 ? L.cin : 64;
  const int n_tiles = (L.rows + n_tile - 1) / n_tile;
  pc.n_tile = n_tile;
  pc.ntaps = L.ntaps;
  pc.cin = L.cin;
  while (arena.size() % 256) arena.push_back(0);
  pc.w_off = static_cast<int64_t>(arena.size());
  const size_t n_el = static_cast<size_t>(n_tiles) * n_tile * L.cin * L.ntaps;
  arena.resize(arena.size() + n_el * 2);
  uint16_t* dst = reinterpret_cast<uint16_t*>(arena.data() + pc.w_off);
  size_t o = 0;
  for (int nt = 0; nt < n_tiles; ++nt)
    for (int c = 0; c < L.cin / kc; ++c)
      for (int t = 0; t < L.ntaps; ++t)
        for (int p = 0; p < kc / 8; ++p)
          for (int r = 0; r < n_tile; ++r)
            for (int e = 0; e < 8; ++e) {
              const int row = nt * n_tile + r;
              const float v = row < L.rows ? L.at(t, row, c * kc + p * 8 + e) : 0.f;
              if (fp16) {
                const __half hv = __float2half_rn(v > 65504.f ? 65504.f : (v < -65504.f ? -65504.f : v));
                memcpy(&dst[o++], &hv, 2);
              } else {
                const __nv_bfloat16 bv = __float2bfloat16_rn(v);
                memcpy(&dst[o++], &bv, 2);
              }
            }
  while (arena.size() % 256) arena.push_back(0);
  pc.b_off = static_cast<int64_t>(arena.size());
  arena.resize(arena.size() + static_cast<size_t>(n_tiles) * n_tile * 4);
  float* b = reinterpret_cast<float*>(arena.data() + pc.b_off);
  for (int i = 0; i < n_tiles * n_tile; ++i) b[i] = i < L.rows ? L.bias[i] : 0.f;
}

struct Tensors {
  std::map<std::string, const AbcNamedTensor*> by_name;
  const float* get(const std::string& name, int64_t numel) const {
    auto it = by_name.find(name);
    if (it == by_name.end()) {
      set_error("abc_unet_create: tensor '%s' missing from the state_dict", name.c_str());
      return nullptr;
    }
    if (it->second->numel != numel || it->second->data == nullptr) {
      set_error("abc_unet_create: tensor '%s' has %lld elements, expected %lld", name.c_str(), static_cast<long long>(it->second->numel),
                static_cast<long long>(numel));
      return nullptr;
    }
    return it->second->data;
  }
};

static bool folded_conv(const Tensors& T, const std::string& conv, const std::string& bn, int cout, int cin, int k,
                        std::vector<float>& w, std::vector<float>& b) {
  const int64_t per = static_cast<int64_t>(cin) * k * k;
  const float* cw = T.get(conv + ".weight", cout * per);
  const float* cb = T.get(conv + ".bias", cout);
  const float* g = T.get(bn + ".weight", cout);
  const float* be = T.get(bn + ".bias", cout);
  const float* rm = T.get(bn + ".running_mean", cout);
  const float* rv = T.get(bn + ".running_var", cout);
  if (!cw || !cb || !g || !be || !rm || !rv) return false;
  w.resize(static_cast<size_t>(cout) * per);
  b.resize(cout);
  for (int co = 0; co < cout; ++co) {
    const float scale = g[co] / sqrtf(rv[co] + 1e-5f);
    for (int64_t i = 0; i < per; ++i) w[co * per + i] = cw[co * per + i] * scale;
    const float t = cb[co] - rm[co];
    b[co] = t * scale + be[co];
  }
  return true;
}

static void pack3x3(std::vector<uint8_t>& arena, PackedConv& pc, const std::vector<float>& w, const std::vector<float>& b, int cout, int cin,
                    bool plain_output, bool fp16) {
  const int js = swap_fold_for(cin, cout, plain_output);
  const int J = js ? js : row_fold_for(cin, cout);
  pc.cout = cout;
  pc.fold = J;
  pc.fold_swap = js ? 1 : 0;
  auto W = [&](int co, int ci, int dy, int dx) { return w[((static_cast<size_t>(co) * cin + ci) * 3 + (dy + 1)) * 3 + (dx + 1)]; };
  Logical L;
  L.cin = cin;
  if (J == 1) {
    L.ntaps = 9;
    L.rows = cout;
    L.w.assign(static_cast<size_t>(9) * cout * cin, 0.f);
    L.bias = b;
    for (int t = 0; t < 9; ++t) {
      pc.tap_dy[t] = t / 3 - 1;
      pc.tap_dx[t] = t % 3 - 1;
      for (int co = 0; co < cout; ++co)
        for (int ci = 0; ci < cin; ++ci) L.at(t, co, ci) = W(co, ci, t / 3 - 1, t % 3 - 1);
    }
    append_pack(arena, pc, L, default_n_tile(cin, cout), fp16);
    return;
  }
  L.ntaps = 3 * (J + 2);
  L.rows = J * cout;
  L.w.assign(static_cast<size_t>(L.ntaps) * L.rows * cin, 0.f);
  L.bias.resize(L.rows);
  for (int t = 0; t < 9; ++t) {
    pc.tap_dy[t] = t / 3 - 1;
    pc.tap_dx[t] = t % 3 - 1;
  }
  for (int r = 0; r < J + 2; ++r)
    for (int c = 0; c < 3; ++c)
      for (int j = 0; j < J; ++j) {
        const int dy = r - 1 - j;
        if (dy < -1 || dy > 1) continue;
        for (int co = 0; co < cout; ++co) {
          const int row = js ? j * cout + co : ((co / 16) * J + j) * 16 + (co % 16);
          for (int ci = 0; ci < cin; ++ci) L.at(r * 3 + c, row, ci) = W(co, ci, dy, c - 1);
        }
      }
  for (int j = 0; j < J; ++j)
    for (int co = 0; co < cout; ++co) L.bias[js ? j * cout + co : ((co / 16) * J + j) * 16 + (co % 16)] = b[co];
  append_pack(arena, pc, L, J * cout, fp16);
  pc.ntaps = 9;
}

static int64_t align256(int64_t v) { return (v + 255) & ~static_cast<int64_t>(255); }

struct Workspace {
  uint8_t* base;
  int64_t used = 0, cap;
  void* take(int64_t bytes) {
    void* p = base ? base + used : nullptr;
    used += align256(bytes);
    return p;
  }
};

static int64_t p8_bytes(int N, int C, int H, int W) { return static_cast<int64_t>(N) * (C / 8) * H * W * 16; }

}

using namespace abc;

static int check_cfg(const AbcUNetConfig* c) {
  ABC_REQUIRE(c != nullptr, "abc_unet: null configuration");
  ABC_REQUIRE(c->in_channels >= 1 && c->in_channels <= 8, "abc_unet: in_channels=%d must be in 1..8", c->in_channels);
  ABC_REQUIRE(c->n_heads >= 1 && c->n_heads <= 16, "abc_unet: n_heads=%d must be in 1..16", c->n_heads);
  for (int i = 0; i < c->n_heads; ++i) ABC_REQUIRE(c->heads[i] >= 1 && c->heads[i] <= 4096, "abc_unet: heads[%d]=%d", i, c->heads[i]);
  return ABC_OK;
}

static int64_t pack_bytes(int rows, int cin, int ntaps, int n_tile) {
  const int64_t n_tiles = (rows + n_tile - 1) / n_tile;
  return align256(n_tiles * n_tile * cin * ntaps * 2) + align256(n_tiles * n_tile * 4);
}

extern "C" int64_t abc_unet_wpack_bytes(const AbcUNetConfig* cfg) {
  if (check_cfg(cfg)) return -1;
  int64_t b = 0;
  for (int i = 0; i < 13; ++i) {
    const int cin0 = kDcIn[i] ? kDcIn[i] : cfg->in_channels, cout = kDcOut[i];
    for (int half = 0; half < 2; ++half) {
      const int cin = half ? cout : cin0;
      if (i == 0 && half == 0) {
        b += align256(static_cast<int64_t>(16) * cin * 9 * 4) + align256(64);
        continue;
      }
      const std::string name = std::string(kShort[i]) + (half ? ".3" : ".0");
      const int js = swap_fold_for(cin, cout, !is_pooled(name));
      const int J = js ? js : row_fold_for(cin, cout);
      b += J == 1 ? pack_bytes(cout, cin, 9, default_n_tile(cin, cout)) : pack_bytes(J * cout, cin, 3 * (J + 2), J * cout);
    }
  }
  const int up_cin[] = {512, 256, 128};
  for (int u = 0; u < 3; ++u) b += pack_bytes(4 * (up_cin[u] / 2), up_cin[u], 4, (up_cin[u] / 2) % 64 == 0 ? 256 : 128);
  b += pack_bytes(128 * cfg->n_heads, 128, 9, 256);
  for (int i = 0; i < cfg->n_heads; ++i) b += pack_bytes(cfg->heads[i], 128, 1, head_conv2_n_tile(cfg->heads[i]));
  return b + 256;
}

extern "C" int64_t abc_unet_workspace_bytes(const AbcUNetConfig* cfg, int N, int H, int W) {
  if (check_cfg(cfg)) return -1;
  if (N <= 0 || H <= 0 || W <= 0 || H % 32 || W % 32) {
    set_error("abc_unet_workspace_bytes: N=%d H=%d W=%d (H, W multiples of 32)", N, H, W);
    return -1;
  }
  int64_t b = 0;
  auto add = [&](int C, int s) { b += align256(p8_bytes(N, C, H / s, W / s)); };
  add(16, 1); add(16, 1); add(16, 2); add(32, 2); add(32, 4); add(64, 4); add(64, 4); add(128, 4); add(64, 8); add(128, 8); add(256, 8);
  add(128, 16); add(256, 16); add(512, 16); add(256, 32); add(512, 32); add(512, 32); add(256, 16); add(256, 16); add(128, 8); add(128, 8);
  add(128, 4); add(128, 4); add(128 * cfg->n_heads, 4);
  return b + 4096;
}

static int pack_all(const AbcUNetConfig* cfg, const AbcNamedTensor* tensors, int n_tensors, UNetHandle* h, std::vector<uint8_t>& arena) {
  Tensors T;
  for (int i = 0; i < n_tensors; ++i) {
    ABC_REQUIRE(tensors[i].name != nullptr, "abc_unet_create: tensor %d has no name", i);
    std::string nm = tensors[i].name;
    if (nm.rfind("module.", 0) == 0) nm = nm.substr(7);
    T.by_name[nm] = &tensors[i];
  }
  h->cfg = *cfg;
  const bool fp16 = cfg->act_fp16 != 0;
  arena.reserve(64 << 20);
  std::vector<float> w, b;
  auto fail = [&]() { return ABC_ERR_INVALID; };
  for (int i = 0; i < 13; ++i) {
    const int cin0 = kDcIn[i] ? kDcIn[i] : cfg->in_channels, cout = kDcOut[i];
    const std::string pre = std::string(kDoubleConvs[i]) + ".double_conv";
    for (int half = 0; half < 2; ++half) {
      const int cin = half ? cout : cin0;
      const std::string name = std::string(kShort[i]) + (half ? ".3" : ".0");
      if (!folded_conv(T, pre + (half ? ".3" : ".0"), pre + (half ? ".4" : ".1"), cout, cin, 3, w, b)) return fail();
      if (i == 0 && half == 0) {
        while (arena.size() % 256) arena.push_back(0);
        h->stem_w_off = static_cast<int64_t>(arena.size());
        arena.resize(arena.size() + w.size() * 4);
        memcpy(arena.data() + h->stem_w_off, w.data(), w.size() * 4);
        while (arena.size() % 256) arena.push_back(0);
        h->stem_b_off = static_cast<int64_t>(arena.size());
        arena.resize(arena.size() + 64);
        memcpy(arena.data() + h->stem_b_off, b.data(), 64);
        continue;
      }
      pack3x3(arena, h->convs[name], w, b, cout, cin, !is_pooled(name), fp16);
    }
  }
  const char* ups[] = {"up1", "up2", "up3"};
  const int up_cin[] = {512, 256, 128};
  for (int u = 0; u < 3; ++u) {
    const int cin = up_cin[u], cout = cin / 2;
    const float* uw = T.get(std::string(ups[u]) + ".up.weight", static_cast<int64_t>(cin) * cout * 9);
    const float* ub = T.get(std::string(ups[u]) + ".up.bias", cout);
    if (!uw || !ub) return fail();
    PackedConv& pc = h->convs[std::string(ups[u]) + ".up"];
    std::vector<std::pair<int, int>> offs;
    for (int dy = -1; dy <= 1; ++dy)
      for (int dx = -1; dx <= 1; ++dx) {
        bool used = false;
        for (int py = 0; py < 2 && !used; ++py)
          for (int px = 0; px < 2 && !used; ++px) {
            int ky[2], dyv[2], ny, kx[2], dxv[2], nx;
            phase_taps(py, cfg->crop_first != 0, ky, dyv, ny);
            phase_taps(px, cfg->crop_first != 0, kx, dxv, nx);
            for (int a = 0; a < ny; ++a)
              for (int c = 0; c < nx; ++c) used = used || (dyv[a] == dy && dxv[c] == dx);
          }
        if (used) offs.push_back({dy, dx});
      }
    Logical L;
    L.ntaps = static_cast<int>(offs.size());
    L.rows = 4 * cout;
    L.cin = cin;
    L.w.assign(static_cast<size_t>(L.ntaps) * L.rows * cin, 0.f);
    L.bias.resize(L.rows);
    for (int ph = 0; ph < 4; ++ph)
      for (int co = 0; co < cout; ++co) L.bias[ph * cout + co] = ub[co];
    for (int py = 0; py < 2; ++py)
      for (int px = 0; px < 2; ++px) {
        int ky[2], dyv[2], ny, kx[2], dxv[2], nx;
        phase_taps(py, cfg->crop_first != 0, ky, dyv, ny);
        phase_taps(px, cfg->crop_first != 0, kx, dxv, nx);
        for (int a = 0; a < ny; ++a)
          for (int c = 0; c < nx; ++c) {
            int t = 0;
            while (offs[t].first != dyv[a] || offs[t].second != dxv[c]) ++t;
            for (int co = 0; co < cout; ++co)
              for (int ci = 0; ci < cin; ++ci)
                L.at(t, (2 * py + px) * cout + co, ci) = uw[((static_cast<size_t>(ci) * cout + co) * 3 + ky[a]) * 3 + kx[c]];
          }
      }
    for (int t = 0; t < L.ntaps; ++t) {
      pc.tap_dy[t] = offs[t].first;
      pc.tap_dx[t] = offs[t].second;
    }
    pc.cout = 4 * cout;
    pc.subpixel = cout;
    append_pack(arena, pc, L, cout % 64 == 0 ? 256 : 128, fp16);
  }
  {
    const int nh = cfg->n_heads;
    Logical L;
    L.ntaps = 9;
    L.rows = 128 * nh;
    L.cin = 128;
    L.w.assign(static_cast<size_t>(9) * L.rows * 128, 0.f);
    L.bias.resize(L.rows);
    PackedConv& pc = h->convs["heads.conv1"];
    for (int i = 0; i < nh; ++i) {
      const std::string om = "out_modules." + std::to_string(i);
      if (!folded_conv(T, om + ".conv1", om + ".bn", 128, 128, 3, w, b)) return fail();
      for (int co = 0; co < 128; ++co) {
        L.bias[128 * i + co] = b[co];
        for (int ci = 0; ci < 128; ++ci)
          for (int t = 0; t < 9; ++t) L.at(t, 128 * i + co, ci) = w[(static_cast<size_t>(co) * 128 + ci) * 9 + t];
      }
    }
    for (int t = 0; t < 9; ++t) {
      pc.tap_dy[t] = t / 3 - 1;
      pc.tap_dx[t] = t % 3 - 1;
    }
    pc.cout = 128 * nh;
    append_pack(arena, pc, L, 256, fp16);
    for (int i = 0; i < nh; ++i) {
      const int hc = cfg->heads[i];
      const std::string om = "out_modules." + std::to_string(i);
      const float* w2 = T.get(om + ".conv2.weight", static_cast<int64_t>(hc) * 128);
      const float* b2 = T.get(om + ".conv2.bias", hc);
      if (!w2 || !b2) return fail();
      Logical L2;
      L2.ntaps = 1;
      L2.rows = hc;
      L2.cin = 128;
      L2.w.assign(w2, w2 + static_cast<size_t>(hc) * 128);
      L2.bias.assign(b2, b2 + hc);
      PackedConv& p2 = h->convs["heads." + std::to_string(i) + ".conv2"];
      p2.cout = hc;
      append_pack(arena, p2, L2, head_conv2_n_tile(hc), fp16);
    }
  }
  return ABC_OK;
}

extern "C" int abc_unet_create(const AbcUNetConfig* cfg, const AbcNamedTensor* tensors, int n_tensors, void* wpack_dev, int64_t wpack_bytes,
                               void* stream, AbcUNet** out) {
  if (int rc = check_cfg(cfg)) return rc;
  if (int rc = device_check()) return rc;
  ABC_REQUIRE(tensors && n_tensors > 0 && wpack_dev && out, "abc_unet_create: null argument");
  auto* h = new UNetHandle();
  std::vector<uint8_t> arena;
  if (int rc = pack_all(cfg, tensors, n_tensors, h, arena)) {
    delete h;
    return rc;
  }
  if (static_cast<int64_t>(arena.size()) > wpack_bytes) {
    set_error("abc_unet_create: packed weights need %lld bytes, wpack_bytes = %lld", static_cast<long long>(arena.size()),
              static_cast<long long>(wpack_bytes));
    delete h;
    return ABC_ERR_INVALID;
  }
  cudaStream_t st = static_cast<cudaStream_t>(stream);
  cudaError_t e = cudaMemcpyAsync(wpack_dev, arena.data(), arena.size(), cudaMemcpyHostToDevice, st);
  if (e == cudaSuccess) e = cudaStreamSynchronize(st);
  if (e != cudaSuccess) {
    set_error("abc_unet_create: weight upload failed: %s", cudaGetErrorString(e));
    delete h;
    return ABC_ERR_CUDA;
  }
  h->arena = static_cast<const uint8_t*>(wpack_dev);
  h->arena_bytes = static_cast<int64_t>(arena.size());
  *out = reinterpret_cast<AbcUNet*>(h);
  return ABC_OK;
}

extern "C" int abc_unet_pack_host(const AbcUNetConfig* cfg, const AbcNamedTensor* tensors, int n_tensors, void* out, int64_t out_bytes,
                                  int64_t* used) {
  if (int rc = check_cfg(cfg)) return rc;
  ABC_REQUIRE(tensors && n_tensors > 0 && out && used, "abc_unet_pack_host: null argument");
  UNetHandle h;
  std::vector<uint8_t> arena;
  if (int rc = pack_all(cfg, tensors, n_tensors, &h, arena)) return rc;
  *used = static_cast<int64_t>(arena.size());
  ABC_REQUIRE(*used <= out_bytes, "abc_unet_pack_host: %lld bytes needed, %lld given", static_cast<long long>(*used),
              static_cast<long long>(out_bytes));
  memcpy(out, arena.data(), arena.size());
  return ABC_OK;
}

extern "C" int abc_unet_destroy(AbcUNet* net) {
  delete reinterpret_cast<UNetHandle*>(net);
  return ABC_OK;
}

extern "C" int abc_unet_forward_infer(AbcUNet* net, const void* img, int img_is_u8, int N, int H, int W, void* workspace,
                                      int64_t workspace_bytes, void* const* out_ptrs, int logits_layout, void* stream) {
  if (int rc = device_check()) return rc;
  ABC_REQUIRE(net && img && workspace && out_ptrs, "abc_unet_forward_infer: null argument");
  auto* h = reinterpret_cast<UNetHandle*>(net);
  const AbcUNetConfig& cfg = h->cfg;
  ABC_REQUIRE(N > 0 && H > 0 && W > 0 && H % 32 == 0 && W % 32 == 0, "abc_unet_forward_infer: N=%d H=%d W=%d (H, W multiples of 32)", N, H, W);
  ABC_REQUIRE(logits_layout == 1 || logits_layout == 2, "abc_unet_forward_infer: logits_layout 1 (NCHW fp32) or 2 (planar-8 fp32)");
  ABC_REQUIRE(!(img_is_u8 && cfg.in_channels != 1), "abc_unet_forward_infer: uint8 images are the 1-channel binarised format");
  const int64_t need = abc_unet_workspace_bytes(&cfg, N, H, W);
  ABC_REQUIRE(workspace_bytes >= need, "abc_unet_forward_infer: workspace of %lld bytes, %lld needed", static_cast<long long>(workspace_bytes),
              static_cast<long long>(need));
  ABC_REQUIRE((reinterpret_cast<uintptr_t>(workspace) & 255) == 0, "abc_unet_forward_infer: workspace must be 256-byte aligned");
  Workspace ws{static_cast<uint8_t*>(workspace), 0, workspace_bytes};
  auto buf = [&](int C, int s) { return ws.take(p8_bytes(N, C, H / s, W / s)); };
  void *a = buf(16, 1), *b = buf(16, 1), *p1 = buf(16, 2), *d1 = buf(32, 2), *p2 = buf(32, 4), *e1 = buf(64, 4), *e2 = buf(64, 4);
  void *cat3 = buf(128, 4), *p3 = buf(64, 8), *f1 = buf(128, 8), *cat2 = buf(256, 8), *p4 = buf(128, 16), *g1 = buf(256, 16);
  void *cat1 = buf(512, 16), *p5 = buf(256, 32), *h1 = buf(512, 32), *h2 = buf(512, 32), *i1 = buf(256, 16), *i2 = buf(256, 16);
  void *j1 = buf(128, 8), *j2 = buf(128, 8), *k1 = buf(128, 4), *k2 = buf(128, 4), *hid = buf(128 * cfg.n_heads, 4);

  auto conv = [&](const char* name, const void* src, int in_planes, int hh, int ww, void* dst, int out_planes, int out_plane_off, int act,
                  void* pool, int pool_planes) -> int {
    auto it = h->convs.find(name);
    ABC_REQUIRE(it != h->convs.end(), "abc_unet_forward_infer: internal: no pack '%s'", name);
    const PackedConv& pc = it->second;
    AbcConvDesc d;
    memset(&d, 0, sizeof(d));
    d.in = src; d.N = N; d.H = hh; d.W = ww; d.in_planes = in_planes; d.in_plane_off = 0; d.cin = pc.cin;
    d.wpack = h->arena + pc.w_off;
    d.bias = reinterpret_cast<const float*>(h->arena + pc.b_off);
    d.cout = pc.cout; d.n_tile = pc.n_tile; d.ntaps = pc.ntaps;
    for (int t = 0; t < 9; ++t) { d.tap_dy[t] = pc.tap_dy[t]; d.tap_dx[t] = pc.tap_dx[t]; }
    d.act = act; d.out_mode = 0;
    d.out = dst; d.out_planes = out_planes; d.out_plane_off = out_plane_off;
    d.out_sy = d.out_sx = pc.subpixel ? 2 : 1;
    d.out_H = hh * d.out_sy; d.out_W = ww * d.out_sx;
    d.pool_out = pool; d.pool_planes = pool_planes;
    d.row_fold = pc.fold; d.subpixel = pc.subpixel;
    d.act_fp16 = cfg.act_fp16 ? 1 : 0;
    d.swap_mn = (!pc.subpixel && pc.n_tile == 128 && (pc.fold == 1 || pc.fold_swap) && dst != nullptr && pool == nullptr) ? 1 : 0;
    return abc_conv_igemm(&d, stream);
  };
#define RUN(call)               \
  do {                          \
    if (int rc_ = (call)) return rc_; \
  } while (0)

  const float* sw = reinterpret_cast<const float*>(h->arena + h->stem_w_off);
  const float* sb = reinterpret_cast<const float*>(h->arena + h->stem_b_off);
  RUN(abc_conv3x3_stem(img, img_is_u8 ? 1 : 0, cfg.in_channels, sw, sb, a, N, H, W, 2, 0, 1 | (cfg.act_fp16 ? 2 : 0), stream));
  RUN(conv("inc1.3", a, 2, H, W, b, 2, 0, 1, nullptr, 0));
  RUN(conv("inc2.0", b, 2, H, W, a, 2, 0, 1, nullptr, 0));
  RUN(conv("inc2.3", a, 2, H, W, nullptr, 0, 0, 1, p1, 2));
  RUN(conv("down1.0", p1, 2, H / 2, W / 2, d1, 4, 0, 1, nullptr, 0));
  RUN(conv("down1.3", d1, 4, H / 2, W / 2, nullptr, 0, 0, 1, p2, 4));
  RUN(conv("down2.0", p2, 4, H / 4, W / 4, e1, 8, 0, 1, nullptr, 0));
  RUN(conv("down2.3", e1, 8, H / 4, W / 4, e2, 8, 0, 1, nullptr, 0));
  RUN(conv("inc3.0", e2, 8, H / 4, W / 4, e1, 8, 0, 1, nullptr, 0));
  RUN(conv("inc3.3", e1, 8, H / 4, W / 4, cat3, 16, 0, 1, p3, 8));
  RUN(conv("down3.0", p3, 8, H / 8, W / 8, f1, 16, 0, 1, nullptr, 0));
  RUN(conv("down3.3", f1, 16, H / 8, W / 8, cat2, 32, 0, 1, p4, 16));
  RUN(conv("down4.0", p4, 16, H / 16, W / 16, g1, 32, 0, 1, nullptr, 0));
  RUN(conv("down4.3", g1, 32, H / 16, W / 16, cat1, 64, 0, 1, p5, 32));
  RUN(conv("down5.0", p5, 32, H / 32, W / 32, h1, 64, 0, 1, nullptr, 0));
  RUN(conv("down5.3", h1, 64, H / 32, W / 32, h2, 64, 0, 1, nullptr, 0));
  RUN(conv("up1.up", h2, 64, H / 32, W / 32, cat1, 64, 32, 0, nullptr, 0));
  RUN(conv("up1.conv.0", cat1, 64, H / 16, W / 16, i1, 32, 0, 1, nullptr, 0));
  RUN(conv("up1.conv.3", i1, 32, H / 16, W / 16, i2, 32, 0, 1, nullptr, 0));
  RUN(conv("up2.up", i2, 32, H / 16, W / 16, cat2, 32, 16, 0, nullptr, 0));
  RUN(conv("up2.conv.0", cat2, 32, H / 8, W / 8, j1, 16, 0, 1, nullptr, 0));
  RUN(conv("up2.conv.3", j1, 16, H / 8, W / 8, j2, 16, 0, 1, nullptr, 0));
  RUN(conv("up3.up", j2, 16, H / 8, W / 8, cat3, 16, 8, 0, nullptr, 0));
  RUN(conv("up3.conv.0", cat3, 16, H / 4, W / 4, k1, 16, 0, 1, nullptr, 0));
  RUN(conv("up3.conv.3", k1, 16, H / 4, W / 4, k2, 16, 0, 1, nullptr, 0));
  RUN(conv("dconv1.0", k2, 16, H / 4, W / 4, k1, 16, 0, 1, nullptr, 0));
  RUN(conv("dconv1.3", k1, 16, H / 4, W / 4, k2, 16, 0, 1, nullptr, 0));
  RUN(conv("dconv2.0", k2, 16, H / 4, W / 4, k1, 16, 0, 1, nullptr, 0));
  RUN(conv("dconv2.3", k1, 16, H / 4, W / 4, k2, 16, 0, 1, nullptr, 0));
  RUN(conv("heads.conv1", k2, 16, H / 4, W / 4, hid, 16 * cfg.n_heads, 0, 2, nullptr, 0));
  for (int i = 0; i < cfg.n_heads; ++i) {
    const PackedConv& pc = h->convs["heads." + std::to_string(i) + ".conv2"];
    ABC_REQUIRE(out_ptrs[i] != nullptr, "abc_unet_forward_infer: out_ptrs[%d] is null", i);
    AbcConvDesc d;
    memset(&d, 0, sizeof(d));
    d.in = hid; d.N = N; d.H = H / 4; d.W = W / 4; d.in_planes = 16 * cfg.n_heads; d.in_plane_off = 16 * i; d.cin = 128;
    d.wpack = h->arena + pc.w_off;
    d.bias = reinterpret_cast<const float*>(h->arena + pc.b_off);
    d.cout = pc.cout; d.n_tile = pc.n_tile; d.ntaps = 1;
    d.act = 0;
    d.out_mode = (logits_layout == 2 && pc.cout > 1) ? 2 : 1;
    d.out = out_ptrs[i]; d.out_planes = d.out_mode == 2 ? (pc.cout + 7) / 8 : 0; d.out_plane_off = 0;
    d.out_H = H / 4; d.out_W = W / 4; d.out_sy = d.out_sx = 1;
    d.row_fold = 1;
    d.act_fp16 = cfg.act_fp16 ? 1 : 0;
    RUN(abc_conv_igemm(&d, stream));
  }
#undef RUN
  return ABC_OK;
}
```

abcnet_b200/unet.py:

```python
from __future__ import annotations

import ctypes as C
import os
from collections import OrderedDict

import torch
import torch.nn as nn

from . import _lib
from ._lib import AbcConvDesc, AbcHeadsFusedDesc, check, lib

BN_EPS = 1e-5
_TAPS3 = [(ky - 1, kx - 1, ky, kx) for ky in range(3) for kx in range(3)]


def _bn(c):
    return nn.BatchNorm2d(c)


def _conv_bn_pair(cin, cout):
    holder = nn.Module()
    holder.double_conv = nn.Sequential(nn.Conv2d(cin, cout, 3, padding=1), _bn(cout), nn.ReLU(inplace=True),
                                       nn.Conv2d(cout, cout, 3, padding=1), _bn(cout), nn.ReLU(inplace=True))
    return holder


def _down(cin, cout):
    holder = nn.Module()
    holder.maxpool_conv = nn.Sequential(nn.MaxPool2d(2), _conv_bn_pair(cin, cout))
    return holder


def _up(cin, cout):
    holder = nn.Module()
    holder.up = nn.ConvTranspose2d(cin, cin // 2, kernel_size=3, stride=2)
    holder.conv = _conv_bn_pair(cin, cout)
    return holder


def _head(cin, cout):
    holder = nn.Module()
    holder.conv1 = nn.Conv2d(cin, cin, 3, padding=1)
    holder.bn = _bn(cin)
    holder.conv2 = nn.Conv2d(cin, cout, 1)
    return holder


def row_fold_for(cin, cout):
    if os.environ.get("ABCNET_NO_FOLD"):
        return 1
    if cout == 16 and cin <= 32:
        return 4
    if cout == 32 and cin <= 32:
        return 2
    return 1


def k_chunk_for(cin):
    if cin == 64 and os.environ.get("ABCNET_KC64"):
        return int(os.environ["ABCNET_KC64"])
    return min(cin, 64)


def use_cta_pair(cin, ntaps, n_tile):
    if os.environ.get("ABCNET_PAIR", "0") != "1":
        return False
    return cin % 64 == 0 and n_tile % 32 == 0 and cin * ntaps * n_tile * 2 > 160 * 1024


def swap_fold_for(cin, cout, plain_output=True):
    if os.environ.get("ABCNET_NO_SWAP") or os.environ.get("ABCNET_NO_FOLD") or os.environ.get("ABCNET_NO_SWAPFOLD") or not plain_output:
        return 0
    J = {64: 2, 32: 4}.get(cout, 0)
    if J == 4 and cin > 32:
        return 0
    return J


def use_swap(pk, out_mode, dst, pool):
    if os.environ.get("ABCNET_NO_SWAP"):
        return False
    return (pk.n_tile == 128 and (pk.fold == 1 or getattr(pk, "fold_swap", False)) and not pk.pair
            and not getattr(pk, "segments", None) and out_mode == 0 and dst is not None and pool is None)


def pair_pack(w_taps, n_tiles, n_tile):
    ntaps, _, cin = w_taps.shape
    w = w_taps.view(ntaps, n_tiles, 2, n_tile // 16, 8, cin // 64, 8, 8)
    r8 = torch.arange(8, device=w_taps.device).view(8, 1)
    pos = torch.arange(8, device=w_taps.device).view(1, 8)
    src = (pos ^ r8).view(1, 1, 1, 1, 8, 1, 8, 1).expand(ntaps, n_tiles, 2, n_tile // 16, 8, cin // 64, 8, 8)
    w = torch.gather(w, 6, src)
    return w.permute(1, 5, 0, 2, 3, 4, 6, 7)


def fold_rows_swap(w_taps, bias, taps, J):
    ntaps, cout, cin = w_taps.shape
    assert ntaps == 9 and J * cout == 128 and sorted(taps) == sorted((dy, dx) for dy in (-1, 0, 1) for dx in (-1, 0, 1))
    by_off = {t: w_taps[i] for i, t in enumerate(taps)}
    out = w_taps.new_zeros(3 * (J + 2), J, cout, cin)
    for r in range(J + 2):
        for c in range(3):
            for j in range(J):
                dy = r - 1 - j
                if -1 <= dy <= 1:
                    out[r * 3 + c, j] = by_off[(dy, c - 1)]
    return out.view(3 * (J + 2), J * cout, cin), bias.view(1, cout).expand(J, cout).reshape(-1)


def fold_rows(w_taps, bias, taps, J):
    ntaps, cout, cin = w_taps.shape
    assert ntaps == 9 and cout % 16 == 0 and sorted(taps) == sorted((dy, dx) for dy in (-1, 0, 1) for dx in (-1, 0, 1))
    by_off = {t: w_taps[i] for i, t in enumerate(taps)}
    out = w_taps.new_zeros(3 * (J + 2), cout // 16, J, 16, cin)
    for r in range(J + 2):
        for c in range(3):
            for j in range(J):
                dy = r - 1 - j
                if -1 <= dy <= 1:
                    out[r * 3 + c, :, j] = by_off[(dy, c - 1)].view(cout // 16, 16, cin)
    b = bias.view(cout // 16, 1, 16).expand(cout // 16, J, 16).reshape(-1)
    return out.view(3 * (J + 2), J * cout, cin), b


class _Packed:

    def __init__(self, w_taps, bias, taps, n_tile, cout, fold=1, pair=None, fold_swap=False, kc=None, dtype=torch.bfloat16):
        self.fold, self.fold_swap = fold, bool(fold_swap) and fold > 1
        if fold > 1:
            w_taps, bias = (fold_rows_swap if fold_swap else fold_rows)(w_taps, bias, taps, fold)
            n_tile = fold * cout
        ntaps, co, cin = w_taps.shape
        kc = kc or k_chunk_for(cin)
        self.kc = kc
        n_tiles = (cout + n_tile - 1) // n_tile
        pad = n_tiles * n_tile - co
        if pad:
            w_taps = torch.cat([w_taps, w_taps.new_zeros(ntaps, pad, cin)], 1)
            bias = torch.cat([bias, bias.new_zeros(pad)])
        if pair is None:
            pair = use_cta_pair(cin, ntaps, n_tile) and fold == 1
        self.pair = bool(pair)
        if self.pair:
            w = pair_pack(w_taps, n_tiles, n_tile)
        else:
            w = w_taps.view(ntaps, n_tiles, n_tile, cin // kc, kc // 8, 8).permute(1, 3, 0, 4, 2, 5)
        self.fp16 = dtype == torch.float16
        self.w = (w.contiguous().clamp(-65504.0, 65504.0) if self.fp16 else w.contiguous()).to(dtype)
        assert self.w.numel() * 2 == lib.abc_conv_wpack_bytes(cin, co, ntaps, n_tile)
        self.bias = bias.contiguous().float()
        self.taps, self.n_tile, self.cout, self.cin = taps, n_tile, cout, cin


def _fold(conv_w, conv_b, bn):
    scale = bn.weight.detach().float() / torch.sqrt((bn.running_var.detach().float() + bn.eps).double()).float()
    w = conv_w.detach().float() * scale.view(-1, 1, 1, 1)
    b = (conv_b.detach().float() - bn.running_mean.detach().float()) * scale + bn.bias.detach().float()
    return w, b


def _default_n_tile(cin, cout):
    env = os.environ.get(f"ABCNET_NTILE_{cin}x{cout}")
    if env:
        return int(env)
    c16 = (cout + 15) // 16 * 16
    if c16 <= 128:
        return c16
    return 256 if (cout % 256 == 0 and cin >= 128) else 128


class HeadMaps(list):

    def __init__(self, heads):
        super().__init__()
        self.heads = list(heads)

    def to_nchw(self):
        out = []
        for t, h in zip(self, self.heads):
            if t.dim() == 5:
                N, P_, H, W, _ = t.shape
                t = t.permute(0, 1, 4, 2, 3).reshape(N, P_ * 8, H, W)[:, :h].contiguous()
            out.append(t)
        return out


class _LaunchTimer:

    def __init__(self, sink, name):
        self.sink, self.name = sink, name

    def __enter__(self):
        if self.sink is not None:
            self.a = torch.cuda.Event(enable_timing=True)
            self.b = torch.cuda.Event(enable_timing=True)
            self.a.record()

    def __exit__(self, *exc):
        if self.sink is not None:
            self.b.record()
            self.sink.append((self.name, self.a, self.b))
        return False


class UNet(nn.Module):
    def __init__(self, in_channels, heads=[1, 21, 5, 1, 4, 2], crop_first=True, act_dtype="bf16"):
        super().__init__()
        if act_dtype not in ("bf16", "fp16"):
            raise ValueError("act_dtype must be 'bf16' or 'fp16'")
        self.act_dtype = act_dtype
        if not (1 <= int(in_channels) <= 8):
            raise ValueError("abcnet_b200.UNet: in_channels must be in 1..8")
        self.n_channels = int(in_channels)
        self.heads = list(heads)
        self.crop_first = bool(crop_first)
        self.s = nn.Parameter(torch.randn(10) / 100)
        self.inc1 = _conv_bn_pair(in_channels, 16)
        self.inc2 = _conv_bn_pair(16, 16)
        self.down1 = _down(16, 32)
        self.down2 = _down(32, 64)
        self.inc3 = _conv_bn_pair(64, 64)
        self.down3 = _down(64, 128)
        self.down4 = _down(128, 256)
        self.down5 = _down(256, 512)
        self.up1 = _up(512, 256)
        self.up2 = _up(256, 128)
        self.up3 = _up(128, 128)
        self.dconv1 = _conv_bn_pair(128, 128)
        self.dconv2 = _conv_bn_pair(128, 128)
        self.out_modules = nn.ModuleList([_head(128, h) for h in self.heads])
        self._packed = None
        self._packed_key = None
        self._pack_gen = 0
        self._bufs = {}
        self.timing = None
        self.dropout_p = 0.2
        self.grad_buckets = None
        self.fuse_bn = True
        self._engine = None

    def load_state_dict(self, state_dict, strict=True, **kw):
        if any(k.startswith("module.") for k in state_dict):
            state_dict = OrderedDict((k[7:] if k.startswith("module.") else k, v) for k, v in state_dict.items())
        self._packed = None
        return super().load_state_dict(state_dict, strict=strict, **kw)

    def _param_key(self):
        return tuple((p.data_ptr(), p._version) for p in list(self.parameters()) + list(self.buffers()))

    def invalidate_packed(self):
        self._packed = None
        self._packed_key = None

    def train(self, mode=True):
        self.invalidate_packed()
        return super().train(mode)

    def _dc_layers(self, holder):
        seq = holder.double_conv
        return [(seq[0], seq[1]), (seq[3], seq[4])]

    @property
    def _act_torch_dtype(self):
        return torch.float16 if self.act_dtype == "fp16" else torch.bfloat16

    @torch.no_grad()
    def prepare(self, _inspect_on_cpu=False):
        dev = self.s.device
        adt = self._act_torch_dtype
        if dev.type != "cuda" and not _inspect_on_cpu:
            raise RuntimeError("abcnet_b200.UNet runs on a CUDA (sm_100) device only; call .cuda() first -- there is no CPU path")
        P = {}

        pooled = {"inc2.3", "down1.3", "inc3.3", "down3.3", "down4.3"}

        def pack3(name, conv, bn):
            w, b = _fold(conv.weight, conv.bias, bn)
            cout, cin = w.shape[:2]
            wt = torch.stack([w[:, :, ky, kx] for (_, _, ky, kx) in _TAPS3])
            js = swap_fold_for(cin, cout, name not in pooled)
            P[name] = _Packed(wt, b, [(dy, dx) for (dy, dx, _, _) in _TAPS3], _default_n_tile(cin, cout), cout,
                              fold=js or row_fold_for(cin, cout), fold_swap=bool(js), dtype=adt)

        c0, b0 = self.inc1.double_conv[0], self.inc1.double_conv[1]
        w, b = _fold(c0.weight, c0.bias, b0)
        P["inc1.0"] = (w.reshape(16, self.n_channels * 9).contiguous(), b.contiguous())
        pack3("inc1.3", self.inc1.double_conv[3], self.inc1.double_conv[4])
        for name, holder in (("inc2", self.inc2), ("down1", self.down1.maxpool_conv[1]), ("down2", self.down2.maxpool_conv[1]),
                             ("inc3", self.inc3), ("down3", self.down3.maxpool_conv[1]), ("down4", self.down4.maxpool_conv[1]),
                             ("down5", self.down5.maxpool_conv[1]), ("up1.conv", self.up1.conv), ("up2.conv", self.up2.conv),
                             ("up3.conv", self.up3.conv), ("dconv1", self.dconv1), ("dconv2", self.dconv2)):
            (ca, ba), (cb, bb) = self._dc_layers(holder)
            pack3(name + ".0", ca, ba)
            pack3(name + ".3", cb, bb)
        for name, holder in (("up1", self.up1), ("up2", self.up2), ("up3", self.up3)):
            w = holder.up.weight.detach().float()
            b = holder.up.bias.detach().float()
            cin, cout = w.shape[:2]
            P[f"{name}.up"] = self._pack_subpixel(w, b)
            for py in (0, 1):
                for px in (0, 1):
                    ys = self._phase_taps(py)
                    xs = self._phase_taps(px)
                    taps = [(dy, dx) for (ky, dy) in ys for (kx, dx) in xs]
                    wt = torch.stack([w[:, :, ky, kx].t() for (ky, dy) in ys for (kx, dx) in xs])
                    P[f"{name}.up.{py}{px}"] = _Packed(wt.contiguous(), b, taps, _default_n_tile(cin, cout), cout, dtype=adt)
        ws, bs = [], []
        for om in self.out_modules:
            w, b = _fold(om.conv1.weight, om.conv1.bias, om.bn)
            ws.append(w)
            bs.append(b)
        w = torch.cat(ws, 0)
        wt = torch.stack([w[:, :, ky, kx] for (_, _, ky, kx) in _TAPS3])
        nt = int(os.environ.get("ABCNET_NTILE_HEADS", "256"))
        P["heads.conv1"] = _Packed(wt, torch.cat(bs), [(dy, dx) for (dy, dx, _, _) in _TAPS3], nt, w.shape[0], dtype=adt)
        P["heads.conv1.plain"] = P["heads.conv1"] if not P["heads.conv1"].pair else None
        self._heads_w1 = (wt, torch.cat(bs), w.shape[0])
        self._packed_heads_ntile = nt
        for i, om in enumerate(self.out_modules):
            w2 = om.conv2.weight.detach().float().reshape(om.conv2.weight.shape[0], -1)
            h = w2.shape[0]
            n_tile = 16 if h <= 16 else (64 if h <= 64 else (128 if h <= 128 else (192 if (h + 191) // 192 * 192 <= (h + 127) // 128 * 128 else 128)))
            P[f"heads.{i}.conv2"] = _Packed(w2.unsqueeze(0).contiguous(), om.conv2.bias.detach().float(), [(0, 0)], n_tile, h, dtype=adt)
        P["heads.fused"] = self._pack_fused_heads(dev)
        self._packed = P
        self._packed_key = self._param_key()
        self._pack_gen += 1
        return self

    def _pack_fused_heads(self, dev):
        heads = self.heads
        if len(heads) > 16 or self._packed_heads_ntile != 256:
            return None
        for i in range(0, len(heads), 2):
            pair = heads[i:i + 2]
            chunks = sum((h + 127) // 128 for h in pair)
            cols = sum(sum(((min(h - c0, 128) + 15) // 16) * 16 for c0 in range(0, h, 128)) for h in pair)
            if chunks > 6 or cols > 512:
                return None
        adt = self._act_torch_dtype
        blocks, biases = [], []
        for om, h in zip(self.out_modules, heads):
            w2 = om.conv2.weight.detach().float().reshape(h, -1)
            b2 = om.conv2.bias.detach().float()
            for c0 in range(0, h, 128):
                cnt = min(h - c0, 128)
                nc = (cnt + 15) // 16 * 16
                wb = w2.new_zeros(nc, 128)
                wb[:cnt] = w2[c0:c0 + cnt]
                wb = wb.view(nc, 16, 8).permute(1, 0, 2).contiguous()
                blocks.append((wb.clamp(-65504.0, 65504.0) if adt == torch.float16 else wb).to(adt).reshape(-1))
                bb = b2.new_zeros(nc)
                bb[:cnt] = b2[c0:c0 + cnt]
                biases.append(bb)
        w2pack = torch.cat(blocks).contiguous()
        bias2 = torch.cat(biases).contiguous()
        nb, nl = C.c_int64(0), C.c_int(0)
        check(lib.abc_heads_fused_pack_sizes(len(heads), (C.c_int * len(heads))(*heads), C.byref(nb), C.byref(nl)), "abc_heads_fused_pack_sizes")
        assert w2pack.numel() * 2 == nb.value and bias2.numel() == nl.value
        return w2pack, bias2

    def _pack_subpixel(self, w, b):
        cin, cout = w.shape[:2]
        offs = sorted({(dy, dx) for py in (0, 1) for px in (0, 1) for (_, dy) in self._phase_taps(py) for (_, dx) in self._phase_taps(px)})
        wt = w.new_zeros(len(offs), 4 * cout, cin)
        for py in (0, 1):
            for px in (0, 1):
                ph = 2 * py + px
                for (ky, dy) in self._phase_taps(py):
                    for (kx, dx) in self._phase_taps(px):
                        wt[offs.index((dy, dx)), ph * cout:(ph + 1) * cout] = w[:, :, ky, kx].t()
        pk = _Packed(wt, b.repeat(4), offs, 256 if cout % 64 == 0 else 128, 4 * cout, pair=False, dtype=self._act_torch_dtype)
        pk.subpixel = cout
        return pk

    def _phase_taps(self, parity):
        if self.crop_first:
            return [(1, 0)] if parity == 0 else [(0, 1), (2, 0)]
        return [(0, 0), (2, -1)] if parity == 0 else [(1, 0)]

    def _buf(self, key, shape):
        t = self._bufs.get(key)
        dt = self._act_torch_dtype
        if t is None or tuple(t.shape) != tuple(shape) or t.device != self.s.device or t.dtype != dt:
            t = torch.empty(shape, dtype=dt, device=self.s.device)
            self._bufs[key] = t
        return t

    @staticmethod
    def _conv(pk, src, in_plane_off, dst, out_plane_off=0, act=1, pool=None, pool_plane_off=0, out_mode=0,
              out_scale=(1, 0, 1, 0), stream=0):
        d = AbcConvDesc()
        N, in_planes, H, W, _ = src.shape
        d.in_, d.N, d.H, d.W = src.data_ptr(), N, H, W
        d.in_planes, d.in_plane_off, d.cin = in_planes, in_plane_off, pk.cin
        d.wpack, d.bias = pk.w.data_ptr(), pk.bias.data_ptr()
        d.cout, d.n_tile, d.ntaps = pk.cout, pk.n_tile, len(pk.taps)
        for i, (dy, dx) in enumerate(pk.taps):
            d.tap_dy[i], d.tap_dx[i] = dy, dx
        d.row_fold, d.cta_pair = pk.fold, int(pk.pair)
        d.k_chunk = getattr(pk, "kc", 0) if getattr(pk, "kc", 0) != min(pk.cin, 64) else 0
        d.act_fp16 = int(getattr(pk, "fp16", False))
        d.subpixel = getattr(pk, "subpixel", 0)
        d.swap_mn = int(use_swap(pk, out_mode, dst, pool)) if not d.subpixel else 0
        d.act, d.out_mode = act, out_mode
        sy, oy, sx, ox = out_scale
        d.out_sy, d.out_oy, d.out_sx, d.out_ox = sy, oy, sx, ox
        if dst is not None:
            d.out = dst.data_ptr()
            if out_mode in (0, 2):
                d.out_planes, d.out_H, d.out_W = dst.shape[1], dst.shape[2], dst.shape[3]
            else:
                d.out_planes, d.out_H, d.out_W = 0, dst.shape[2], dst.shape[3]
            d.out_plane_off = out_plane_off
        else:
            d.out, d.out_H, d.out_W = None, H, W
        if pool is not None:
            d.pool_out, d.pool_planes, d.pool_plane_off = pool.data_ptr(), pool.shape[1], pool_plane_off
        check(lib.abc_conv_igemm(C.byref(d), stream), "abc_conv_igemm")

    def _timed(self, name):
        return _LaunchTimer(self.timing, name)

    def forward(self, x):
        if self.training:
            from .train import _UNetTrainFn
            return list(_UNetTrainFn.apply(self, x, *self.parameters()))
        return self.infer(x)

    def _train_engine(self):
        if self._engine is None:
            from .train import TrainEngine
            self._engine = TrainEngine(self)
        return self._engine

    @torch.no_grad()
    def trunk_and_hidden(self, x):
        k2 = self.trunk(x)
        B, _, H4, W4, _ = k2.shape
        hid = self._buf("hid", (B, 16 * len(self.heads), H4, W4, 8))
        with self._timed("heads.conv1"):
            self._conv(self._packed["heads.conv1"], k2, 0, hid, act=2, stream=_lib.current_stream_ptr())
        return k2, hid

    @torch.no_grad()
    def trunk(self, x):
        if not x.is_cuda:
            raise RuntimeError("abcnet_b200.UNet.forward needs a CUDA tensor (no CPU fallback)")
        _lib.require_device()
        if x.dim() != 4 or x.shape[1] != self.n_channels or x.shape[2] % 32 or x.shape[3] % 32:
            raise ValueError(f"expected [B,{self.n_channels},H,W] with H, W multiples of 32, got {tuple(x.shape)}")
        if self._packed is None or self._packed_key != self._param_key():
            self.prepare()
        P = self._packed
        u8 = self.n_channels == 1 and x.dtype in (torch.uint8, torch.bool)
        x = x.contiguous().view(torch.uint8) if u8 else x.contiguous().float()
        stem_flags = 1 | (2 if self.act_dtype == "fp16" else 0)

        def first(xp, wp, bp, op, B_, H_, W_, planes, off, st_):
            return lib.abc_conv3x3_stem(xp, int(u8), self.n_channels, wp, bp, op, B_, H_, W_, planes, off, stem_flags, st_)
        B, _, H, W = x.shape
        st = _lib.current_stream_ptr()

        def cv(name, *a, **k):
            with self._timed(name):
                self._conv(P[name], *a, stream=st, **k)

        a = self._buf("a", (B, 2, H, W, 8))
        b = self._buf("b", (B, 2, H, W, 8))
        w0, b0 = P["inc1.0"]
        with self._timed("inc1.0"):
            check(first(x.data_ptr(), w0.data_ptr(), b0.data_ptr(), a.data_ptr(), B, H, W, 2, 0, st), "abc_conv3x3_stem")
        cv("inc1.3", a, 0, b)
        cv("inc2.0", b, 0, a)
        p1 = self._buf("p1", (B, 2, H // 2, W // 2, 8))
        cv("inc2.3", a, 0, None, pool=p1)
        d1 = self._buf("d1", (B, 4, H // 2, W // 2, 8))
        cv("down1.0", p1, 0, d1)
        p2 = self._buf("p2", (B, 4, H // 4, W // 4, 8))
        cv("down1.3", d1, 0, None, pool=p2)
        e1 = self._buf("e1", (B, 8, H // 4, W // 4, 8))
        e2 = self._buf("e2", (B, 8, H // 4, W // 4, 8))
        cat3 = self._buf("cat3", (B, 16, H // 4, W // 4, 8))
        cv("down2.0", p2, 0, e1)
        cv("down2.3", e1, 0, e2)
        cv("inc3.0", e2, 0, e1)
        p3 = self._buf("p3", (B, 8, H // 8, W // 8, 8))
        cv("inc3.3", e1, 0, cat3, out_plane_off=0, pool=p3)
        f1 = self._buf("f1", (B, 16, H // 8, W // 8, 8))
        cat2 = self._buf("cat2", (B, 32, H // 8, W // 8, 8))
        p4 = self._buf("p4", (B, 16, H // 16, W // 16, 8))
        cv("down3.0", p3, 0, f1)
        cv("down3.3", f1, 0, cat2, out_plane_off=0, pool=p4)
        g1 = self._buf("g1", (B, 32, H // 16, W // 16, 8))
        cat1 = self._buf("cat1", (B, 64, H // 16, W // 16, 8))
        p5 = self._buf("p5", (B, 32, H // 32, W // 32, 8))
        cv("down4.0", p4, 0, g1)
        cv("down4.3", g1, 0, cat1, out_plane_off=0, pool=p5)
        h1 = self._buf("h1", (B, 64, H // 32, W // 32, 8))
        h2 = self._buf("h2", (B, 64, H // 32, W // 32, 8))
        cv("down5.0", p5, 0, h1)
        cv("down5.3", h1, 0, h2)

        merged_up = not os.environ.get("ABCNET_UP_PHASES")

        def up(name, src, cat, half_planes):
            with self._timed(name + ".up"):
                if merged_up:
                    self._conv(P[f"{name}.up"], src, 0, cat, out_plane_off=half_planes, act=0, out_scale=(2, 0, 2, 0), stream=st)
                    return
                for py in (0, 1):
                    for px in (0, 1):
                        self._conv(P[f"{name}.up.{py}{px}"], src, 0, cat, out_plane_off=half_planes, act=0,
                                   out_scale=(2, py, 2, px), stream=st)

        up("up1", h2, cat1, 32)
        i1 = self._buf("i1", (B, 32, H // 16, W // 16, 8))
        i2 = self._buf("i2", (B, 32, H // 16, W // 16, 8))
        cv("up1.conv.0", cat1, 0, i1)
        cv("up1.conv.3", i1, 0, i2)
        up("up2", i2, cat2, 16)
        j1 = self._buf("j1", (B, 16, H // 8, W // 8, 8))
        j2 = self._buf("j2", (B, 16, H // 8, W // 8, 8))
        cv("up2.conv.0", cat2, 0, j1)
        cv("up2.conv.3", j1, 0, j2)
        up("up3", j2, cat3, 8)
        k1 = self._buf("k1", (B, 16, H // 4, W // 4, 8))
        k2 = self._buf("k2", (B, 16, H // 4, W // 4, 8))
        cv("up3.conv.0", cat3, 0, k1)
        cv("up3.conv.3", k1, 0, k2)
        cv("dconv1.0", k2, 0, k1)
        cv("dconv1.3", k1, 0, k2)
        cv("dconv2.0", k2, 0, k1)
        cv("dconv2.3", k1, 0, k2)
        return k2

    @torch.no_grad()
    def infer(self, x, outs=None, layout="nchw", fused=None):
        if layout not in ("nchw", "p8f"):
            raise ValueError("layout must be 'nchw' or 'p8f'")
        p8f = layout == "p8f"
        k2 = self.trunk(x)
        B, _, H4, W4, _ = k2.shape
        st = _lib.current_stream_ptr()
        if outs is None:
            outs = HeadMaps(self.heads)
            for h in self.heads:
                shape = (B, (h + 7) // 8, H4, W4, 8) if (p8f and h > 1) else (B, h, H4, W4)
                outs.append(torch.empty(shape, dtype=torch.float32, device=k2.device))
        fpack = self._packed.get("heads.fused")
        if fused is None:
            fused = fpack is not None and os.environ.get("ABCNET_FUSED_HEADS", "1") != "0"
        if fused:
            if fpack is None:
                raise ValueError("abc_heads_fused is not available for this head list (see include/abcnet_b200.h); use fused=False")
            w2pack, bias2 = fpack
            pk1 = self._packed["heads.conv1.plain"]
            if pk1 is None:
                wt1, b1, c1 = self._heads_w1
                pk1 = self._packed["heads.conv1.plain"] = _Packed(wt1, b1, [(dy, dx) for (dy, dx, _, _) in _TAPS3], 256, c1, pair=False,
                                                                  dtype=self._act_torch_dtype)
            d = AbcHeadsFusedDesc()
            d.in_, d.N, d.H, d.W, d.in_planes, d.in_plane_off = k2.data_ptr(), B, H4, W4, k2.shape[1], 0
            d.w1pack, d.bias1, d.n_heads = pk1.w.data_ptr(), pk1.bias.data_ptr(), len(self.heads)
            d.w2pack, d.w2pack_bytes, d.bias2, d.bias2_len = w2pack.data_ptr(), w2pack.numel() * 2, bias2.data_ptr(), bias2.numel()
            slots = [int(v) for v in os.environ.get("ABCNET_HF_SLOTS", "").split(",") if v.strip()]
            for i in range(6):
                d.item_slot[i] = slots[i] if i < len(slots) else -1
            d.act_fp16 = int(pk1.fp16)
            for i, h in enumerate(self.heads):
                d.cout[i], d.out[i] = h, outs[i].data_ptr()
                d.out_mode[i] = 2 if outs[i].dim() == 5 else 1
                d.out_planes[i] = outs[i].shape[1] if outs[i].dim() == 5 else 0
            with self._timed("heads.fused"):
                check(lib.abc_heads_fused(C.byref(d), st), "abc_heads_fused")
            return outs
        hid = self._buf("hid", (B, 16 * len(self.heads), H4, W4, 8))
        with self._timed("heads.conv1"):
            self._conv(self._packed["heads.conv1"], k2, 0, hid, act=2, stream=st)
        with self._timed("heads.conv2"):
            for i, h in enumerate(self.heads):
                self._conv(self._packed[f"heads.{i}.conv2"], hid, 16 * i, outs[i], act=0,
                           out_mode=2 if outs[i].dim() == 5 else 1, stream=st)
        return outs

    def activation(self, name):
        t = self._bufs[name]
        N, P_, H, W, _ = t.shape
        return t.float().permute(0, 1, 4, 2, 3).reshape(N, P_ * 8, H, W)
```

include/abcnet_b200.h:

```cpp
#ifndef ABCNET_B200_H_
#define ABCNET_B200_H_

#include <stdint.h>

#ifdef __cplusplus
extern "C" {
#endif

#define ABC_API __attribute__((visibility("default")))

typedef enum AbcStatus {
  ABC_OK = 0,
  ABC_ERR_INVALID = -1,
  ABC_ERR_NO_DEVICE = -2,
  ABC_ERR_CUDA = -3,
  ABC_ERR_CAPACITY = -4
} AbcStatus;

ABC_API const char* abc_last_error(void);
ABC_API int abc_version(void);
ABC_API int abc_device_ok(void);
ABC_API int abc_sm_count(void);
ABC_API int64_t abc_launch_count(void);

ABC_API int abc_conv3x3_c1(const float* img, const float* w, const float* b, void* out, int N, int H, int W,
                           int out_planes, int out_plane_off, void* stream);
ABC_API int abc_conv3x3_c1_u8(const uint8_t* img, const float* w, const float* b, void* out, int N, int H, int W,
                              int out_planes, int out_plane_off, void* stream);
ABC_API int abc_conv3x3_stem(const void* img, int img_is_u8, int cin, const float* w, const float* b, void* out, int N, int H, int W,
                             int out_planes, int out_plane_off, int flags, void* stream);
ABC_API int abc_conv3x3_cn(const float* img, int cin, const float* w, const float* b, void* out, int N, int H, int W,
                           int out_planes, int out_plane_off, int relu, void* stream);

typedef struct AbcConvDesc {
  const void* in;
  int N, H, W;
  int in_planes;
  int in_plane_off;
  int cin;
  const void* wpack;
  const float* bias;
  int cout;
  int n_tile;
  int ntaps;
  int tap_dy[9];
  int tap_dx[9];
  int act;
  int out_mode;
  void* out;
  int out_planes;
  int out_plane_off;
  int out_H, out_W;
  int out_sy, out_oy, out_sx, out_ox;
  void* pool_out;
  int pool_planes, pool_plane_off;
  int k_segments;
  int seg_tap0[4];
  int seg_ntaps[4];
  int row_fold;
  int cta_pair;
  int swap_mn;
  double* stat_sum;
  double* stat_sq;
  int subpixel;
  int k_chunk;
  int act_fp16;
} AbcConvDesc;

ABC_API int abc_conv_igemm(const AbcConvDesc* desc, void* stream);
ABC_API int64_t abc_conv_wpack_bytes(int cin, int cout, int ntaps, int n_tile);

typedef struct AbcHeadsFusedDesc {
  const void* in;
  int N, H, W;
  int in_planes, in_plane_off;
  const void* w1pack;
  const float* bias1;
  int n_heads;
  int cout[16];
  const void* w2pack;
  int64_t w2pack_bytes;
  const float* bias2;
  int bias2_len;
  void* out[16];
  int out_mode[16];
  int out_planes[16];
  int item_slot[6];
  int act_fp16;
} AbcHeadsFusedDesc;
ABC_API int abc_heads_fused(const AbcHeadsFusedDesc* desc, void* stream);
ABC_API int abc_heads_fused_pack_sizes(int n_heads, const int* cout, int64_t* w2pack_bytes, int* bias2_len);

typedef struct AbcAtomRec {
  uint16_t x, y;
  uint8_t type, charge, hs, pad;
} AbcAtomRec;
typedef struct AbcBondRec {
  uint16_t x, y;
  uint8_t omega, type;
  uint16_t pad;
  float rho;
} AbcBondRec;
typedef struct AbcDecodeDesc {
  const float* maps[8];
  int N, H, W;
  int c_type, c_charge, c_hs, n_omega, n_btype;
  float thr;
  int omega_mode;
  AbcAtomRec* atoms;
  int atom_cap;
  AbcBondRec* bonds;
  int bond_cap;
  int32_t* counts;
  int p8f_mask;
  int centre_prob;
  float thr_omega;
  int32_t* peak_pix;
  int32_t* peak_cnt;
  int peak_cap;
  int sparse_mode;
} AbcDecodeDesc;
ABC_API int abc_decode_peaks(const AbcDecodeDesc* desc, void* stream);
ABC_API int abc_gather_patches(const void* trunk, int N, int H, int W, int planes, const int32_t* peak_pix, const int32_t* peak_cnt,
                               int peak_cap, void* out, void* stream);

ABC_API int abc_assemble_molblocks(const AbcAtomRec* atoms, int atom_cap, const AbcBondRec* bonds, int bond_cap,
                                   const int32_t* counts, int N, const double* cos_tab, const double* sin_tab, int n_omega,
                                   int n_threads, char* text, int64_t text_stride, int32_t* text_len);

typedef struct AbcLossDesc {
  const float* logits[8];
  const void* targets[8];
  int tgt_f64;
  int N, H, W;
  int c_type, c_charge, c_hs, n_omega, n_btype;
  const float* type_weights;
  double* sums;
  const float* scale;
  float* dlogits[8];
} AbcLossDesc;
enum AbcLossIndex { ABC_L_ATOM = 0, ABC_L_BOND, ABC_L_TYPE, ABC_L_CHARGE, ABC_L_BTYPE, ABC_L_RHO, ABC_L_OMEGA, ABC_L_HS };
ABC_API int abc_loss_partials(const AbcLossDesc* desc, void* stream);
ABC_API int abc_loss_backward(const AbcLossDesc* desc, void* stream);
typedef struct AbcLossP8Out {
  void* dz[8];
  int planes[8];
  double* dbias[8];
} AbcLossP8Out;
ABC_API int abc_loss_partials_p8(const AbcLossDesc* desc, const AbcLossP8Out* out, void* stream);

ABC_API int abc_bn_stats(const void* z, int N, int H, int W, int planes, int plane_off, int C, double* sum, double* sumsq, void* stream);
ABC_API int abc_bn_finalize(const double* sum, const double* sumsq, int C, double count, const float* gamma, const float* beta,
                            float eps, float momentum, float* running_mean, float* running_var, float* scale, float* shift,
                            float* mean, float* invstd, void* stream);
typedef struct AbcBnActDesc {
  const void* z; int z_planes, z_plane_off;
  void* out; int out_planes, out_plane_off;
  void* pool; int pool_planes, pool_plane_off;
  int N, H, W, C;
  const float* scale; const float* shift;
  int act;
  float drop_p; uint64_t seed;
  const uint64_t* seed_dev;
  void* drop_mask;
} AbcBnActDesc;
ABC_API int abc_bn_act(const AbcBnActDesc* desc, void* stream);
typedef struct AbcBnActBwdDesc {
  const void* z; int z_planes, z_plane_off;
  const void* dA; int dA_planes, dA_plane_off;
  const void* dP; int dP_planes, dP_plane_off;
  void* dz; int dz_planes, dz_plane_off;
  int N, H, W, C;
  const float* scale; const float* shift; const float* mean; const float* invstd;
  int act; float drop_p; uint64_t seed;
  double* s1; double* s2;
  const uint64_t* seed_dev;
  const float* gscale;
  const void* drop_mask;
} AbcBnActBwdDesc;
ABC_API int abc_bn_act_backward(const AbcBnActBwdDesc* desc, void* stream);
ABC_API int abc_nchw_to_p8(const float* src, void* dst, int N, int C, int H, int W, void* stream);
ABC_API int abc_nchw_to_p8_ex(const float* src, void* dst, int N, int C, int H, int W, int dst_planes, const float* scale,
                              double* dbias, void* stream);
ABC_API int abc_channel_sum(const void* x, int N, int H, int W, int planes, int plane_off, int C, double* sum, double* scratch, void* stream);
ABC_API int abc_deinterleave2(const void* src, int src_planes, int src_plane_off, int C, void* dst, int N, int H, int W, void* stream);
typedef struct AbcTargetsDesc {
  int N, H, W, n_omega, n_btype, c_type, c_charge, c_hs;
  const int32_t* atoms; const int32_t* atom_off;
  const int32_t* bonds; const double* bond_rho; const int32_t* bond_off;
  float* atom_target; float* atom_type; float* atom_charge; float* atom_hs; float* bond_target; float* bond_type;
  void* bond_rho_map; void* bond_omega;
  int f64;
  int zero_first;
} AbcTargetsDesc;
ABC_API int abc_rasterise_targets(const AbcTargetsDesc* desc, void* stream);

ABC_API int abc_gather_pack(const void* src_ptrs, const void* codes, void* out, int64_t n, int out_is_bf16, void* stream);
ABC_API int abc_adam_chunk_elems(void);
ABC_API int abc_adam_step(const void* p_ptrs, const void* g_ptrs, const void* m_ptrs, const void* v_ptrs, const int64_t* sizes,
                          const int32_t* chunks, int n_chunks, const float* hyper, float* step_dev, void* stream);
typedef struct AbcWgradDesc {
  const void* dz; int dz_planes, dz_plane_off; int cout;
  const void* in; int in_planes, in_plane_off; int cin;
  int N, H, W;
  int ntaps; int tap_dy[9]; int tap_dx[9];
  float* dw;
  int row_boxes;
} AbcWgradDesc;
ABC_API int abc_conv_wgrad(const AbcWgradDesc* desc, void* stream);
ABC_API int abc_conv3x3_c1_raw(const void* img, int img_is_u8, const float* w, const float* b, void* out, int N, int H, int W,
                               int out_planes, int out_plane_off, void* stream);
ABC_API int abc_conv3x3_c1_wgrad(const void* img, int img_is_u8, const void* dz, int dz_planes, int dz_plane_off, int N, int H, int W,
                                 float* dw, void* stream);
ABC_API int abc_conv3x3_cn_wgrad(const float* img, int cin, const void* dz, int dz_planes, int dz_plane_off, int N, int H, int W,
                                 float* dw, void* stream);

typedef struct AbcUNetConfig {
  int in_channels;
  int n_heads;
  int heads[16];
  int crop_first;
  int act_fp16;
} AbcUNetConfig;
typedef struct AbcNamedTensor {
  const char* name;
  const float* data;
  int64_t numel;
} AbcNamedTensor;
typedef struct AbcUNet AbcUNet;
ABC_API int64_t abc_unet_wpack_bytes(const AbcUNetConfig* cfg);
ABC_API int64_t abc_unet_workspace_bytes(const AbcUNetConfig* cfg, int N, int H, int W);
ABC_API int abc_unet_create(const AbcUNetConfig* cfg, const AbcNamedTensor* tensors, int n_tensors, void* wpack_dev, int64_t wpack_bytes,
                            void* stream, AbcUNet** out);
ABC_API int abc_unet_forward_infer(AbcUNet* net, const void* img, int img_is_u8, int N, int H, int W, void* workspace,
                                   int64_t workspace_bytes, void* const* out_ptrs, int logits_layout, void* stream);
ABC_API int abc_unet_destroy(AbcUNet* net);
ABC_API int abc_unet_pack_host(const AbcUNetConfig* cfg, const AbcNamedTensor* tensors, int n_tensors, void* out, int64_t out_bytes,
                               int64_t* used);

#ifdef __cplusplus
}
#endif
#endif
```

Baseline: 10040.

## Fuse single-channel stem conv into first igemm conv's A-operand producer

The first 1->16 3x3 stem convolution is computed on the fly inside the producer warps of the following 16->16 implicit-GEMM conv. The image window is read, binarised into row bitmasks and turned into A tiles through a 512-entry lookup table in shared memory, with a generic fallback path for non-binary pixels. This removes one kernel launch and the full-resolution write and read of the intermediate activation. In exchange it costs extra shared memory, adds per-group table-building and ballot work, and recomputes halo pixels for each tile.

```diff
diff --git a/abcnet_b200/_lib.py b/abcnet_b200/_lib.py
--- a/abcnet_b200/_lib.py
+++ b/abcnet_b200/_lib.py
@@ -32,6 +32,7 @@
         ("k_segments", C.c_int), ("seg_tap0", C.c_int * 4), ("seg_ntaps", C.c_int * 4),
         ("row_fold", C.c_int), ("cta_pair", C.c_int), ("swap_mn", C.c_int),
         ("stat_sum", C.c_void_p), ("stat_sq", C.c_void_p), ("subpixel", C.c_int), ("k_chunk", C.c_int), ("act_fp16", C.c_int),
+        ("stem_img", C.c_void_p), ("stem_img_u8", C.c_int), ("stem_w", C.c_void_p), ("stem_b", C.c_void_p),
     ]
 
 
diff --git a/abcnet_b200/csrc/conv_first.cu b/abcnet_b200/csrc/conv_first.cu
--- a/abcnet_b200/csrc/conv_first.cu
+++ b/abcnet_b200/csrc/conv_first.cu
@@ -3,6 +3,7 @@
 
 #include "common.cuh"
 #include "p8_device.cuh"
+#include "stem_c1.cuh"
 
 namespace abc {
 
@@ -43,31 +44,6 @@
 
 constexpr int kC1Rows = 16;
 
-__device__ __forceinline__ uint4 c1_pack8(const float* a, int flags) { return pack8_act16(a, (flags & 2) != 0); }
-
-template <typename T>
-__device__ __noinline__ void c1_generic_pixel(const T* __restrict__ im, int y, int x, int H, int W, const float* ws, int relu,
-                                              uint4* o0, uint4* o1) {
-  float t[9];
-#pragma unroll
-  for (int k = 0; k < 9; ++k) {
-    const int yy = y + k / 3 - 1, xx = x + k % 3 - 1;
-    t[k] = (yy >= 0 && yy < H && xx >= 0 && xx < W) ? static_cast<float>(__ldg(im + static_cast<size_t>(yy) * W + xx)) : 0.f;
-  }
-#pragma unroll
-  for (int pl = 0; pl < 2; ++pl) {
-    float v[8];
-#pragma unroll
-    for (int c8 = 0; c8 < 8; ++c8) {
-      const int co = pl * 8 + c8;
-      float a = ws[144 + co];
-#pragma unroll
-      for (int k = 0; k < 9; ++k) a = fmaf(t[k], ws[k * 16 + co], a);
-      v[c8] = (relu & 1) ? fmaxf(a, 0.f) : a;
-    }
-    *(pl ? o1 : o0) = c1_pack8(v, relu);
-  }
-}
 
 template <typename T>
 __global__ void __launch_bounds__(256, 4) conv3x3_c1_rows_kernel(const T* __restrict__ img, const float* __restrict__ w,
@@ -82,18 +58,7 @@
 #pragma unroll 1
   for (int e = tid; e < 512; e += 256) {
 #pragma unroll 1
-    for (int pl = 0; pl < 2; ++pl) {
-      float v[8];
-#pragma unroll
-      for (int c8 = 0; c8 < 8; ++c8) {
-        const int co = pl * 8 + c8;
-        float a = ws[144 + co];
-#pragma unroll
-        for (int k = 0; k < 9; ++k) a = fmaf(((e >> k) & 1) ? 1.f : 0.f, ws[k * 16 + co], a);
-        v[c8] = (relu & 1) ? fmaxf(a, 0.f) : a;
-      }
-      lut[e][pl] = c1_pack8(v, relu);
-    }
+    for (int pl = 0; pl < 2; ++pl) lut[e][pl] = c1_table_entry(e, pl, ws, relu);
   }
   __syncthreads();
   const int lane = tid & 31, warp = tid >> 5;
@@ -121,11 +86,11 @@
         v[k] = (in && x < W) ? static_cast<float>(__ldg(row + x)) : 0.f;
       }
       if (in && edge_ok) ve = static_cast<float>(__ldg(row + xe));
-      bool bad = (ve != 0.f) && (ve != 1.f);
+      bool bad = c1_non_binary(ve);
 #pragma unroll
       for (int k = 0; k < 4; ++k) {
         mm[k] = __ballot_sync(0xffffffffu, v[k] != 0.f);
-        bad = bad || ((v[k] != 0.f) && (v[k] != 1.f));
+        bad = bad || c1_non_binary(v[k]);
       }
       ee = __ballot_sync(0xffffffffu, ve != 0.f);
       nbin = __any_sync(0xffffffffu, bad);
diff --git a/abcnet_b200/csrc/conv_igemm_sm100.cu b/abcnet_b200/csrc/conv_igemm_sm100.cu
--- a/abcnet_b200/csrc/conv_igemm_sm100.cu
+++ b/abcnet_b200/csrc/conv_igemm_sm100.cu
@@ -1,10 +1,12 @@
 #include <cstdlib>
+#include <type_traits>
 #include <cuda.h>
 #include <cuda_bf16.h>
 
 #include "common.cuh"
 #include "p8_device.cuh"
 #include "ptx_sm100.cuh"
+#include "stem_c1.cuh"
 
 namespace abc {
 
@@ -18,6 +20,12 @@
 constexpr uint32_t kSwapRowBytes = 80;
 constexpr uint32_t kSwapWarpBytes = 16 * kSwapRowBytes;
 constexpr uint32_t kSwapStageBytes = 8 * kSwapWarpBytes;
+constexpr uint32_t kStemLutBytes = 512 * 32;
+constexpr uint32_t kStemWsOff = kStemLutBytes;
+constexpr uint32_t kStemMaskOff = kStemWsOff + 160 * 4;
+constexpr int kStemWinRows = 68;
+constexpr uint32_t kStemBytes = 18432;
+static_assert(kStemMaskOff + 2 * kStemWinRows * 4 <= kStemBytes, "fused-stem scratch overflow");
 
 struct ConvKParams {
   int N, H, W, tiles_x, tiles_y, groups_x, num_groups;
@@ -41,6 +49,10 @@
   int fp16;
   double* stat_sum;
   double* stat_sq;
+  const void* stem_img;
+  const float* stem_w;
+  const float* stem_b;
+  int stem_flags;
 };
 
 __device__ __forceinline__ float apply_act(float v, int act) {
@@ -90,12 +102,13 @@
   return q;
 }
 
-template <int KSTEPS, bool RESIDENT, bool CG2, bool SWAP = false, bool STATS = false>
+template <int KSTEPS, bool RESIDENT, bool CG2, bool SWAP = false, bool STATS = false, int STEM = 0>
 __global__ void __launch_bounds__(kThreads, 1)
 conv_igemm_kernel(const __grid_constant__ CUtensorMap tmap, const ConvKParams p) {
   static_assert(!(CG2 && RESIDENT), "the CTA-pair variant streams its weights");
   static_assert(!(CG2 && SWAP), "operand swap is a single-CTA mode");
   static_assert(!(STATS && (SWAP || CG2)), "STATS is the non-swap, single-CTA variant");
+  static_assert(STEM == 0 || (KSTEPS == 1 && RESIDENT && !CG2 && !SWAP && !STATS), "STEM is the row-folded 16 -> 16 variant");
   extern __shared__ __align__(1024) uint8_t smem[];
   const uint32_t sbase = smem_u32(smem);
   const int warp = static_cast<int>(warp_id_uniform());
@@ -116,7 +129,7 @@
   if (threadIdx.x == 0) {
     const uint32_t full_count = (CG2 && leader && !(p.dbg & 1)) ? 2 : 1;
     for (int i = 0; i < kMaxNA; ++i) {
-      mbar_init(bar_a_full + 8 * i, full_count);
+      mbar_init(bar_a_full + 8 * i, STEM != 0 ? 2 : full_count);
       mbar_init(bar_a_empty + 8 * i, 1);
     }
     for (int i = 0; i < kMaxNB; ++i) {
@@ -128,7 +141,7 @@
       mbar_init(bar_acc_empty + 8 * i, CG2 ? 16 : 8);
     }
     fence_mbar_init();
-    tma_prefetch_desc(&tmap);
+    if (STEM == 0) tma_prefetch_desc(&tmap);
   }
   if (CG2) cluster_sync_all();
   if (warp == 2) {
@@ -150,6 +163,14 @@
       utab2[threadIdx.x] = (static_cast<uint32_t>(chn >> 3) << 16) | static_cast<uint32_t>((ph >> 1) * p.out_W + (ph & 1));
     }
   }
+  if constexpr (STEM != 0) {
+    float* stem_ws = reinterpret_cast<float*>(smem + kHeaderBytes + kStemWsOff);
+    if (threadIdx.x < 144) stem_ws[(threadIdx.x % 9) * 16 + threadIdx.x / 9] = p.stem_w[threadIdx.x];
+    if (threadIdx.x < 16) stem_ws[144 + threadIdx.x] = p.stem_b[threadIdx.x];
+    __syncthreads();
+    uint4* lut = reinterpret_cast<uint4*>(smem + kHeaderBytes);
+    for (int i = threadIdx.x; i < 1024; i += kThreads) lut[i] = c1_table_entry(i >> 1, i & 1, stem_ws, p.stem_flags);
+  }
   tc_fence_before();
   if (CG2) cluster_sync_all();
   else __syncthreads();
@@ -162,7 +183,115 @@
   const uint32_t b_region = sbase + p.smem_b_off;
   const int blocks_per_ntile = p.blocks_per_ntile;
 
-  if (warp == 0) {
+  if (STEM != 0 && (warp == 0 || warp == 2)) {
+    using T = typename std::conditional<STEM == 2, uint8_t, float>::type;
+    constexpr int kHaloRows = 66, kHaloCols = 10, kRowsPerLane = 22;
+    const T* img = static_cast<const T*>(p.stem_img);
+    const uint4* lut = reinterpret_cast<const uint4*>(smem + kHeaderBytes);
+    const float* stem_ws = reinterpret_cast<const float*>(smem + kHeaderBytes + kStemWsOff);
+    const int pw = warp == 0 ? 0 : 1;
+    uint32_t* rmask = reinterpret_cast<uint32_t*>(smem + kHeaderBytes + kStemMaskOff) + pw * kStemWinRows;
+    const size_t img_plane = static_cast<size_t>(p.H) * p.W;
+    const int hc = lane % kHaloCols, rg = lane / kHaloCols;
+    const int i0 = 2 * pw, ntile = min(2, p.mt - i0);
+    auto window = [&](int g, int& n, int& ty, int& tx0) {
+      n = g / groups_per_img;
+      const int rem = g - n * groups_per_img;
+      ty = rem / p.groups_x;
+      tx0 = (rem - ty * p.groups_x) * p.mt;
+    };
+    int stage = 0;
+    uint32_t phase = 0;
+    for (int g = g_first; g < p.num_groups; g += gridDim.x) {
+      int n, ty, tx0;
+      window(g, n, ty, tx0);
+      const T* im = img + n * img_plane;
+      const int wy0 = ty * p.tile_rows - 2, wx0 = (tx0 + i0) * 8 - 2;
+      bool bad = false;
+      if (ntile > 0) {
+        if (g + static_cast<int>(gridDim.x) < p.num_groups) {
+          int n2, ty2, tx2;
+          window(g + gridDim.x, n2, ty2, tx2);
+          const int x2 = min(max((tx2 + i0) * 8 - 2, 0), p.W - 1);
+          for (int r = lane; r < kStemWinRows; r += 32) {
+            const int y = ty2 * p.tile_rows - 2 + r;
+            if (y >= 0 && y < p.H) prefetch_l2(img + n2 * img_plane + static_cast<size_t>(y) * p.W + x2);
+          }
+        }
+        const int x = wx0 + lane;
+        const bool col_ok = lane < 20 && x >= 0 && x < p.W;
+#pragma unroll 1
+        for (int r0 = 0; r0 < kStemWinRows; r0 += 17) {
+          float v[17];
+#pragma unroll
+          for (int k = 0; k < 17; ++k) {
+            const int y = wy0 + r0 + k;
+            v[k] = (col_ok && y >= 0 && y < p.H) ? static_cast<float>(__ldg(im + static_cast<size_t>(y) * p.W + x)) : 0.f;
+          }
+#pragma unroll
+          for (int k = 0; k < 17; ++k) {
+            const uint32_t m = __ballot_sync(0xffffffffu, v[k] != 0.f);
+            if (lane == 0) rmask[r0 + k] = m;
+            bad = bad || c1_non_binary(v[k]);
+          }
+        }
+        bad = __any_sync(0xffffffffu, bad);
+      }
+      __syncwarp();
+      mbar_wait(bar_a_empty + 8 * stage, phase ^ 1);
+      uint8_t* a_st = smem + p.smem_a_off + stage * p.a_stage_bytes;
+      if (lane < 3 * kHaloCols) {
+        for (int ii = 0; ii < ntile; ++ii) {
+          const int i = i0 + ii;
+          uint8_t* dst = a_st + i * p.a_tile_bytes + (rg * kRowsPerLane * kHaloCols + hc) * 16;
+          const int x = (tx0 + i) * 8 - 1 + hc;
+          const int y0 = ty * p.tile_rows - 1 + rg * kRowsPerLane;
+          const bool x_in = x >= 0 && x < p.W;
+          if (!bad) {
+            const int c = ii * 8 + hc;
+            const uint32_t* rm = rmask + rg * kRowsPerLane;
+            uint32_t t0 = (rm[0] >> c) & 7u, t1 = (rm[1] >> c) & 7u;
+#pragma unroll 2
+            for (int k = 0; k < kRowsPerLane; ++k) {
+              const uint32_t t2 = (rm[k + 2] >> c) & 7u;
+              const uint32_t pat = t0 | (t1 << 3) | (t2 << 6);
+              const int y = y0 + k;
+              uint4 q0 = make_uint4(0u, 0u, 0u, 0u), q1 = q0;
+              if (x_in && y >= 0 && y < p.H) {
+                q0 = lut[2 * pat];
+                q1 = lut[2 * pat + 1];
+              }
+              uint4* o = reinterpret_cast<uint4*>(dst + k * (kHaloCols * 16));
+              o[0] = q0;
+              o[p.a_plane_bytes >> 4] = q1;
+              t0 = t1;
+              t1 = t2;
+            }
+          } else {
+#pragma unroll 1
+            for (int k = 0; k < kRowsPerLane; ++k) {
+              const int y = y0 + k;
+              uint4* o = reinterpret_cast<uint4*>(dst + k * (kHaloCols * 16));
+              if (x_in && y >= 0 && y < p.H) {
+                c1_generic_pixel<T>(im, y, x, p.H, p.W, stem_ws, p.stem_flags, o, o + (p.a_plane_bytes >> 4));
+              } else {
+                o[0] = make_uint4(0u, 0u, 0u, 0u);
+                o[p.a_plane_bytes >> 4] = make_uint4(0u, 0u, 0u, 0u);
+              }
+            }
+          }
+        }
+      }
+      static_assert(3 * kRowsPerLane == kHaloRows, "row split");
+      fence_proxy_async();
+      __syncwarp();
+      if (lane == 0) mbar_arrive(bar_a_full + 8 * stage);
+      if (++stage == p.na) {
+        stage = 0;
+        phase ^= 1;
+      }
+    }
+  } else if (warp == 0) {
     int stage = 0;
     uint32_t phase = 0;
     for (int gp = g_first; gp < p.num_groups; gp += gridDim.x) {
@@ -700,18 +829,26 @@
   using namespace abc;
   if (int rc = device_check()) return rc;
   ABC_REQUIRE(d != nullptr, "abc_conv_igemm: null descriptor");
-  ABC_REQUIRE(d->in && d->wpack && d->bias, "abc_conv_igemm: null input / weights / bias");
+  const bool stem = d->stem_img != nullptr;
+  ABC_REQUIRE((d->in || stem) && d->wpack && d->bias, "abc_conv_igemm: null input / weights / bias");
   ABC_REQUIRE(d->out || d->pool_out, "abc_conv_igemm: no output buffer");
   ABC_REQUIRE(d->N > 0 && d->H > 0 && d->W > 0, "abc_conv_igemm: bad geometry N=%d H=%d W=%d", d->N, d->H, d->W);
   ABC_REQUIRE(d->cin >= 16 && d->cin % 16 == 0 && (d->cin <= 64 || d->cin % 64 == 0),
               "abc_conv_igemm: cin=%d must be 16, 32, 48, 64 or a multiple of 64", d->cin);
-  ABC_REQUIRE(d->in_plane_off >= 0 && d->in_plane_off + d->cin / 8 <= d->in_planes, "abc_conv_igemm: input plane range");
+  if (!stem) ABC_REQUIRE(d->in_plane_off >= 0 && d->in_plane_off + d->cin / 8 <= d->in_planes, "abc_conv_igemm: input plane range");
   ABC_REQUIRE(d->n_tile >= 16 && d->n_tile <= 256 && d->n_tile % 16 == 0, "abc_conv_igemm: n_tile=%d", d->n_tile);
   ABC_REQUIRE(d->ntaps >= 1 && d->ntaps <= 9, "abc_conv_igemm: ntaps=%d", d->ntaps);
   ABC_REQUIRE(d->cout >= 1, "abc_conv_igemm: cout=%d", d->cout);
   ABC_REQUIRE(d->out_mode >= 0 && d->out_mode <= 2, "abc_conv_igemm: out_mode=%d", d->out_mode);
   ABC_REQUIRE((reinterpret_cast<uintptr_t>(d->in) & 15) == 0 && (reinterpret_cast<uintptr_t>(d->wpack) & 15) == 0,
               "abc_conv_igemm: input / weights must be 16-byte aligned");
+  if (stem) {
+    ABC_REQUIRE(d->stem_w && d->stem_b && (d->stem_img_u8 == 0 || d->stem_img_u8 == 1), "abc_conv_igemm: stem_w / stem_b / stem_img_u8");
+    ABC_REQUIRE(d->cin == 16 && d->cout == 16 && d->row_fold == 4 && d->n_tile == 64 && d->ntaps == 9 && (d->k_chunk == 0 || d->k_chunk == 16) &&
+                    !d->swap_mn && !d->cta_pair && d->k_segments <= 1 && !d->subpixel && !d->stat_sum && !d->stat_sq && d->out_mode == 0,
+                "abc_conv_igemm: stem_img is built for the row-folded 16 -> 16 layer (cin = cout = 16, row_fold = 4, n_tile = 64, "
+                "plain P8 output, no statistics)");
+  }
   const int fold = d->row_fold > 1 ? d->row_fold : 1;
   if (fold > 1) {
     ABC_REQUIRE(fold == 2 || fold == 4, "abc_conv_igemm: row_fold=%d must be 1, 2 or 4", fold);
@@ -811,7 +948,7 @@
     p.b_block_bytes /= 2;
   }
   const uint32_t total_b = want_pair ? (1u << 30) : static_cast<uint32_t>(p.blocks_per_ntile) * p.b_block_bytes;
-  p.smem_a_off = kHeaderBytes + (swap ? kSwapStageBytes : 0u);
+  p.smem_a_off = kHeaderBytes + (swap ? kSwapStageBytes : 0u) + (stem ? kStemBytes : 0u);
   const uint32_t hdr = p.smem_a_off;
   int mt_max = swap ? 1 : 256 / d->n_tile;
   if (d->n_tile == 256 && env.mt256 > 0) mt_max = env.mt256 >= 2 ? 2 : 1;
@@ -879,13 +1016,19 @@
     p.stat_sum = d->stat_sum;
     p.stat_sq = d->stat_sq;
   }
+  if (stem) {
+    p.stem_img = d->stem_img;
+    p.stem_w = d->stem_w;
+    p.stem_b = d->stem_b;
+    p.stem_flags = 1 | (p.fp16 ? 2 : 0);
+  }
 
   EncodeTiledFn encode = get_encode_fn();
   if (!encode) {
     set_error("cuTensorMapEncodeTiled driver entry point not available");
     return ABC_ERR_NO_DEVICE;
   }
-  CUtensorMap tmap;
+  CUtensorMap tmap{};
   const cuuint64_t gdim[4] = {static_cast<cuuint64_t>(d->W) * 8, static_cast<cuuint64_t>(d->H),
                               static_cast<cuuint64_t>(d->in_planes), static_cast<cuuint64_t>(d->N)};
   const cuuint64_t gstride[3] = {static_cast<cuuint64_t>(d->W) * 16, static_cast<cuuint64_t>(d->W) * d->H * 16,
@@ -893,7 +1036,7 @@
   const cuuint32_t box[4] = {static_cast<cuuint32_t>(cols * 8), static_cast<cuuint32_t>(rows),
                              static_cast<cuuint32_t>(p.kp), 1};
   const cuuint32_t estr[4] = {1, 1, 1, 1};
-  CUresult cr = encode(&tmap, CU_TENSOR_MAP_DATA_TYPE_BFLOAT16, 4, const_cast<void*>(d->in), gdim, gstride, box, estr,
+  CUresult cr = stem ? CUDA_SUCCESS : encode(&tmap, CU_TENSOR_MAP_DATA_TYPE_BFLOAT16, 4, const_cast<void*>(d->in), gdim, gstride, box, estr,
                        CU_TENSOR_MAP_INTERLEAVE_NONE, CU_TENSOR_MAP_SWIZZLE_NONE, CU_TENSOR_MAP_L2_PROMOTION_L2_256B,
                        CU_TENSOR_MAP_FLOAT_OOB_FILL_NONE);
   if (cr != CUDA_SUCCESS) {
@@ -913,6 +1056,8 @@
                                   conv_igemm_kernel<3, true, false, true>, conv_igemm_kernel<4, true, false, true>}};
   KernelFn pair_kernel = conv_igemm_kernel<4, false, true>;
   KernelFn stats_kernel = conv_igemm_kernel<1, true, false, false, true>;
+  KernelFn stem_kernels[2] = {conv_igemm_kernel<1, true, false, false, false, 1>,
+                              conv_igemm_kernel<1, true, false, false, false, 2>};
   static PerDeviceOnce attr_once;
   ABC_CUDA(attr_once.run([&]() -> cudaError_t {
     for (int r = 0; r < 2; ++r)
@@ -921,6 +1066,8 @@
         if (cudaError_t e = cudaFuncSetAttribute(swap_kernels[r][k], cudaFuncAttributeMaxDynamicSharedMemorySize, kSmemBudget)) return e;
       }
     if (cudaError_t e = cudaFuncSetAttribute(stats_kernel, cudaFuncAttributeMaxDynamicSharedMemorySize, kSmemBudget)) return e;
+    for (KernelFn f : stem_kernels)
+      if (cudaError_t e = cudaFuncSetAttribute(f, cudaFuncAttributeMaxDynamicSharedMemorySize, kSmemBudget)) return e;
     return cudaFuncSetAttribute(pair_kernel, cudaFuncAttributeMaxDynamicSharedMemorySize, kSmemBudget);
   }));
   const int ksteps = p.kp / 2;
@@ -958,6 +1105,10 @@
     ABC_REQUIRE(p.resident_b && ksteps == 1, "abc_conv_igemm: internal: fused statistics variant");
     fn = stats_kernel;
   }
+  if (stem) {
+    ABC_REQUIRE(p.resident_b && ksteps == 1 && p.nkc == 1, "abc_conv_igemm: internal: fused-stem variant");
+    fn = stem_kernels[d->stem_img_u8 ? 1 : 0];
+  }
   fn<<<grid, kThreads, smem_bytes, st_>>>(tmap, p);
-  return launch_check(swap ? "conv_igemm_kernel<swap>" : "conv_igemm_kernel");
+  return launch_check(stem ? "conv_igemm_kernel<stem>" : swap ? "conv_igemm_kernel<swap>" : "conv_igemm_kernel");
 }
diff --git a/abcnet_b200/csrc/ptx_sm100.cuh b/abcnet_b200/csrc/ptx_sm100.cuh
--- a/abcnet_b200/csrc/ptx_sm100.cuh
+++ b/abcnet_b200/csrc/ptx_sm100.cuh
@@ -58,6 +58,9 @@
   }
 }
 
+__device__ __forceinline__ void prefetch_l2(const void* p) {
+  asm volatile("prefetch.global.L2 [%0];" ::"l"(reinterpret_cast<uint64_t>(p)));
+}
 __device__ __forceinline__ void tma_prefetch_desc(const void* desc) {
   asm volatile("prefetch.tensormap [%0];" ::"l"(reinterpret_cast<uint64_t>(desc)) : "memory");
 }
diff --git a/abcnet_b200/csrc/stem_c1.cuh b/abcnet_b200/csrc/stem_c1.cuh
--- /dev/null
+++ b/abcnet_b200/csrc/stem_c1.cuh
@@ -0,0 +1,50 @@
+#pragma once
+
+#include <cuda_bf16.h>
+
+#include "p8_device.cuh"
+
+namespace abc {
+
+__device__ __forceinline__ uint4 c1_pack8(const float* a, int flags) { return pack8_act16(a, (flags & 2) != 0); }
+
+__device__ __forceinline__ bool c1_non_binary(float v) { return v != 0.f && v != 1.f; }
+
+__device__ __forceinline__ uint4 c1_table_entry(int e, int pl, const float* ws, int flags) {
+  float v[8];
+#pragma unroll
+  for (int c8 = 0; c8 < 8; ++c8) {
+    const int co = pl * 8 + c8;
+    float a = ws[144 + co];
+#pragma unroll
+    for (int k = 0; k < 9; ++k) a = fmaf(((e >> k) & 1) ? 1.f : 0.f, ws[k * 16 + co], a);
+    v[c8] = (flags & 1) ? fmaxf(a, 0.f) : a;
+  }
+  return c1_pack8(v, flags);
+}
+
+template <typename T>
+__device__ __noinline__ void c1_generic_pixel(const T* __restrict__ im, int y, int x, int H, int W, const float* ws, int flags,
+                                              uint4* o0, uint4* o1) {
+  float t[9];
+#pragma unroll
+  for (int k = 0; k < 9; ++k) {
+    const int yy = y + k / 3 - 1, xx = x + k % 3 - 1;
+    t[k] = (yy >= 0 && yy < H && xx >= 0 && xx < W) ? static_cast<float>(__ldg(im + static_cast<size_t>(yy) * W + xx)) : 0.f;
+  }
+#pragma unroll
+  for (int pl = 0; pl < 2; ++pl) {
+    float v[8];
+#pragma unroll
+    for (int c8 = 0; c8 < 8; ++c8) {
+      const int co = pl * 8 + c8;
+      float a = ws[144 + co];
+#pragma unroll
+      for (int k = 0; k < 9; ++k) a = fmaf(t[k], ws[k * 16 + co], a);
+      v[c8] = (flags & 1) ? fmaxf(a, 0.f) : a;
+    }
+    *(pl ? o1 : o0) = c1_pack8(v, flags);
+  }
+}
+
+}
diff --git a/abcnet_b200/csrc/unet_plan.cu b/abcnet_b200/csrc/unet_plan.cu
--- a/abcnet_b200/csrc/unet_plan.cu
+++ b/abcnet_b200/csrc/unet_plan.cu
@@ -1,4 +1,5 @@
 #include <cmath>
+#include <cstdlib>
 #include <cstring>
 #include <map>
 #include <string>
@@ -464,6 +465,9 @@
   void *cat1 = buf(512, 16), *p5 = buf(256, 32), *h1 = buf(512, 32), *h2 = buf(512, 32), *i1 = buf(256, 16), *i2 = buf(256, 16);
   void *j1 = buf(128, 8), *j2 = buf(128, 8), *k1 = buf(128, 4), *k2 = buf(128, 4), *hid = buf(128 * cfg.n_heads, 4);
 
+  const void* stem_img = nullptr;
+  const float *stem_w = nullptr, *stem_b = nullptr;
+  int stem_u8 = 0;
   auto conv = [&](const char* name, const void* src, int in_planes, int hh, int ww, void* dst, int out_planes, int out_plane_off, int act,
                   void* pool, int pool_planes) -> int {
     auto it = h->convs.find(name);
@@ -484,6 +488,7 @@
     d.row_fold = pc.fold; d.subpixel = pc.subpixel;
     d.act_fp16 = cfg.act_fp16 ? 1 : 0;
     d.swap_mn = (!pc.subpixel && pc.n_tile == 128 && (pc.fold == 1 || pc.fold_swap) && dst != nullptr && pool == nullptr) ? 1 : 0;
+    d.stem_img = stem_img; d.stem_img_u8 = stem_u8; d.stem_w = stem_w; d.stem_b = stem_b;
     return abc_conv_igemm(&d, stream);
   };
 #define RUN(call)               \
@@ -493,8 +498,22 @@
 
   const float* sw = reinterpret_cast<const float*>(h->arena + h->stem_w_off);
   const float* sb = reinterpret_cast<const float*>(h->arena + h->stem_b_off);
-  RUN(abc_conv3x3_stem(img, img_is_u8 ? 1 : 0, cfg.in_channels, sw, sb, a, N, H, W, 2, 0, 1 | (cfg.act_fp16 ? 2 : 0), stream));
-  RUN(conv("inc1.3", a, 2, H, W, b, 2, 0, 1, nullptr, 0));
+  static const bool stem_fused = [] {
+    const char* e = getenv("ABCNET_STEM_FUSED");
+    return !(e && strcmp(e, "0") == 0);
+  }();
+  if (cfg.in_channels == 1 && stem_fused) {
+    stem_img = img;
+    stem_u8 = img_is_u8 ? 1 : 0;
+    stem_w = sw;
+    stem_b = sb;
+    const int rc = conv("inc1.3", nullptr, 2, H, W, b, 2, 0, 1, nullptr, 0);
+    stem_img = nullptr;
+    RUN(rc);
+  } else {
+    RUN(abc_conv3x3_stem(img, img_is_u8 ? 1 : 0, cfg.in_channels, sw, sb, a, N, H, W, 2, 0, 1 | (cfg.act_fp16 ? 2 : 0), stream));
+    RUN(conv("inc1.3", a, 2, H, W, b, 2, 0, 1, nullptr, 0));
+  }
   RUN(conv("inc2.0", b, 2, H, W, a, 2, 0, 1, nullptr, 0));
   RUN(conv("inc2.3", a, 2, H, W, nullptr, 0, 0, 1, p1, 2));
   RUN(conv("down1.0", p1, 2, H / 2, W / 2, d1, 4, 0, 1, nullptr, 0));
diff --git a/abcnet_b200/unet.py b/abcnet_b200/unet.py
--- a/abcnet_b200/unet.py
+++ b/abcnet_b200/unet.py
@@ -389,7 +389,7 @@
 
     @staticmethod
     def _conv(pk, src, in_plane_off, dst, out_plane_off=0, act=1, pool=None, pool_plane_off=0, out_mode=0,
-              out_scale=(1, 0, 1, 0), stream=0):
+              out_scale=(1, 0, 1, 0), stream=0, stem=None):
         d = AbcConvDesc()
         N, in_planes, H, W, _ = src.shape
         d.in_, d.N, d.H, d.W = src.data_ptr(), N, H, W
@@ -417,6 +417,9 @@
             d.out, d.out_H, d.out_W = None, H, W
         if pool is not None:
             d.pool_out, d.pool_planes, d.pool_plane_off = pool.data_ptr(), pool.shape[1], pool_plane_off
+        if stem is not None:
+            img, u8, w0, b0 = stem
+            d.stem_img, d.stem_img_u8, d.stem_w, d.stem_b = img.data_ptr(), int(u8), w0.data_ptr(), b0.data_ptr()
         check(lib.abc_conv_igemm(C.byref(d), stream), "abc_conv_igemm")
 
     def _timed(self, name):
@@ -469,9 +472,12 @@
         a = self._buf("a", (B, 2, H, W, 8))
         b = self._buf("b", (B, 2, H, W, 8))
         w0, b0 = P["inc1.0"]
-        with self._timed("inc1.0"):
-            check(first(x.data_ptr(), w0.data_ptr(), b0.data_ptr(), a.data_ptr(), B, H, W, 2, 0, st), "abc_conv3x3_stem")
-        cv("inc1.3", a, 0, b)
+        if self.n_channels == 1 and os.environ.get("ABCNET_STEM_FUSED", "1") != "0":
+            cv("inc1.3", a, 0, b, stem=(x, u8, w0, b0))
+        else:
+            with self._timed("inc1.0"):
+                check(first(x.data_ptr(), w0.data_ptr(), b0.data_ptr(), a.data_ptr(), B, H, W, 2, 0, st), "abc_conv3x3_stem")
+            cv("inc1.3", a, 0, b)
         cv("inc2.0", b, 0, a)
         p1 = self._buf("p1", (B, 2, H // 2, W // 2, 8))
         cv("inc2.3", a, 0, None, pool=p1)
diff --git a/include/abcnet_b200.h b/include/abcnet_b200.h
--- a/include/abcnet_b200.h
+++ b/include/abcnet_b200.h
@@ -65,6 +65,10 @@
   int subpixel;
   int k_chunk;
   int act_fp16;
+  const void* stem_img;
+  int stem_img_u8;
+  const float* stem_w;
+  const float* stem_b;
 } AbcConvDesc;
 
 ABC_API int abc_conv_igemm(const AbcConvDesc* desc, void* stream);
diff --git a/scratch_front_ab.py b/scratch_front_ab.py
--- /dev/null
+++ b/scratch_front_ab.py
@@ -0,0 +1,37 @@
+import os, sys, json
+import torch
+sys.path.insert(0, os.path.dirname(os.path.abspath(__file__)))
+import abcnet_b200
+from oracle import synth, unet_ref
+
+B = int(sys.argv[1]) if len(sys.argv) > 1 else 256
+m = abcnet_b200.UNet(1, list(unet_ref.V2_HEADS)).cuda().eval()
+m.load_state_dict(unet_ref.make_state_dict(seed=3, heads=tuple(unet_ref.V2_HEADS), variant="W1"))
+pool = torch.from_numpy(synth.binary_images(5, 64, 512, 512, 0.05))
+x = pool.repeat((B + 63) // 64, 1, 1, 1)[:B].contiguous().cuda()
+xu = (x > 0).to(torch.uint8)
+res = {}
+for rep in range(3):
+    for arm in ("0", "1"):
+        for name, inp in (("f32", x), ("u8", xu)):
+            os.environ["ABCNET_STEM_FUSED"] = arm
+            for _ in range(3):
+                m.trunk(inp)
+            torch.cuda.synchronize()
+            m.timing = []
+            for _ in range(20):
+                m.trunk(inp)
+            torch.cuda.synchronize()
+            agg = {}
+            for n, a, b in m.timing:
+                agg.setdefault(n, []).append(a.elapsed_time(b))
+            m.timing = None
+            front = sum(sum(v) / len(v) for k, v in agg.items() if k in ("inc1.0", "inc1.3"))
+            res.setdefault(f"{name}_fused{arm}", []).append(round(front, 4))
+            e0, e1 = torch.cuda.Event(True), torch.cuda.Event(True)
+            e0.record()
+            for _ in range(10):
+                m.infer(inp)
+            e1.record(); torch.cuda.synchronize()
+            res.setdefault(f"{name}_fused{arm}_infer_ms", []).append(round(e0.elapsed_time(e1) / 10, 3))
+print(json.dumps(res))
```

Result: slower. 9896 (median of 6 runs) (-1.4%).
